# libertininick/imagescry

Hardware: AMD Instinct MI355X
Metric: queries/s cosine top-10 over N x D bank (higher is better)
Workload: dtype f16; 1 GPU; cosine top-10: 1024 fp16 queries x 10000000 x 768 fp16 bank (BASELINE config 4 bank; row-sharded 1 way); bank_rows=10000000, dim=768, queries=1024, k=10, rows_per_gpu=10000000, parallelism=row-shard1

## Files before the change

### imagescry_amd/_lib.py

```python

from __future__ import annotations

import ctypes
import math
import os
from ctypes import POINTER, c_char_p, c_float, c_int, c_int32, c_int64, c_size_t, c_void_p
from pathlib import Path

import torch

LIB_NAME = "libimagescry_hip.so"
LIB_PATH = Path(os.environ.get("ISC_LIB") or Path(__file__).resolve().parent / LIB_NAME)

ISC_U8, ISC_F16, ISC_F32 = 0, 1, 2
ISC_ACT_NONE, ISC_ACT_RELU, ISC_ACT_GELU, ISC_ACT_SILU, ISC_ACT_SIGMOID = 0, 1, 2, 3, 4
ISC_ACT_RESIDUAL_AFTER = 0x100
ISC_TOPK_MAX_K = 120
ISC_SEARCH_MAX_D = 8192
ISC_SEARCH_PASS_QUERIES = 1024
ISC_ABI_VERSION = 4
ISC_BUILD_ABLATION = 1
ISC_GEMM_A_PACKED, ISC_GEMM_W_PACKED, ISC_GEMM_OUT_PACKED, ISC_GEMM_TILE_256, ISC_GEMM_TILE_128 = 1, 2, 4, 8, 16
ISC_KERNEL_DOTS_FILTER, ISC_KERNEL_CONV, ISC_KERNEL_GEMM_F16 = 0, 1, 2

ISC_OK = 0
ISC_ERR_INVALID_ARG = -1
ISC_ERR_UNSUPPORTED = -2
ISC_ERR_WORKSPACE = -3
ISC_ERR_LAUNCH = -4
ISC_ERR_NO_DEVICE = -5
ISC_ERR_ALIGNMENT = -6


class HipLibraryError(RuntimeError):
    """The HIP library is missing, failed to load, or a kernel launch failed."""


SIGNATURES: dict[str, tuple[object, list[object]]] = {
    "isc_abi_version": (c_int, []),
    "isc_build_flags": (c_int, []),
    "isc_strerror": (c_char_p, [c_int]),
    "isc_device_info": (c_int, [POINTER(c_int), POINTER(c_int), c_char_p, c_int]),
    "isc_timing_enable": (c_int, [c_int]),
    "isc_timing_read": (c_int, [c_int, POINTER(ctypes.c_double), POINTER(c_int)]),
    "isc_channel_stats_workspace_bytes": (c_int, [c_int, c_int, c_int, c_int, c_int, POINTER(c_size_t)]),
    "isc_channel_stats": (
        c_int,
        [c_void_p, c_int, c_int, c_int, c_int, c_int, c_void_p, c_void_p, c_void_p, c_size_t, c_void_p],
    ),
    "isc_normalize_clip": (
        c_int,
        [c_void_p, c_int, c_int, c_int, c_int, c_int, c_void_p, c_void_p, c_int, c_float, c_float, c_float, c_void_p,
         c_void_p],
    ),
    "isc_normalize_clip_nhwc4": (
        c_int,
        [c_void_p, c_int, c_int, c_int, c_int, c_int, c_void_p, c_void_p, c_int, c_float, c_float, c_float, c_void_p,
         c_void_p],
    ),
    "isc_resize_bilinear": (c_int, [c_void_p, c_int, c_int, c_int, c_int, c_int, c_int, c_void_p, c_void_p]),
    "isc_l2norm_channels": (c_int, [c_void_p, c_int, c_int, c_int, c_float, c_void_p, c_void_p]),
    "isc_bank_packed_bytes": (c_int, [c_int, c_int64, c_int, POINTER(c_size_t)]),
    "isc_bank_permutation": (c_int, [c_int64, POINTER(c_int64), POINTER(c_int64)]),
    "isc_bank_pack": (
        c_int,
        [c_void_p, c_int, c_int64, c_int, c_int64, c_int64, c_int64, c_int, c_float, c_void_p, c_int, c_void_p,
         c_void_p],
    ),
    "isc_bank_unpack": (c_int, [c_void_p, c_int, c_int, c_int64, c_int64, c_int64, c_void_p, c_int64, c_void_p]),
    "isc_bank_append": (
        c_int,
        [c_void_p, c_int, c_int64, c_int, c_int64, c_int64, c_int64, c_int, c_float, c_void_p, c_int, c_void_p,
         c_void_p, c_void_p, c_void_p, c_void_p],
    ),
    "isc_bank_repack": (
        c_int,
        [c_void_p, c_int64, c_void_p, c_int64, c_int, c_int, c_int64, c_int64, c_void_p, c_void_p, c_void_p, c_void_p],
    ),
    "isc_nchw_to_nhwc": (c_int, [c_void_p, c_int, c_int, c_int, c_int, c_int, c_void_p, c_void_p]),
    "isc_conv2d_nhwc": (
        c_int,
        [c_void_p, c_int, c_int, c_int, c_int, c_void_p, c_int, c_int, c_int, c_int, c_int, c_void_p, c_void_p, c_int,
         c_void_p, c_void_p],
    ),
    "isc_conv2d_nhwc_dual": (
        c_int,
        [c_void_p, c_int, c_int, c_int, c_int, c_void_p, c_int, c_int, c_int, c_int, c_void_p, c_int, c_void_p, c_void_p,
         c_int, c_void_p, c_void_p],
    ),
    "isc_conv2d_nhwc_gated": (
        c_int,
        [c_void_p, c_int, c_int, c_int, c_int, c_void_p, c_void_p, c_int, c_int, c_int, c_int, c_int, c_void_p,
         c_void_p, c_int, c_void_p, c_void_p],
    ),
    "isc_dwconv2d_nhwc": (
        c_int,
        [c_void_p, c_int, c_int, c_int, c_int, c_void_p, c_int, c_int, c_int, c_void_p, c_int, c_void_p, c_void_p],
    ),
    "isc_dwconv2d_nhwc_pool": (
        c_int,
        [c_void_p, c_int, c_int, c_int, c_int, c_void_p, c_int, c_int, c_int, c_void_p, c_int, c_void_p, c_void_p,
         c_void_p, c_void_p],
    ),
    "isc_se_gate": (
        c_int,
        [c_void_p, c_int, c_int, c_void_p, c_int, c_void_p, c_int, c_void_p, c_int, c_void_p, c_void_p, c_void_p],
    ),
    "isc_linear_centered": (
        c_int, [c_void_p, c_int64, c_int, c_void_p, c_void_p, c_int, c_void_p, c_void_p, c_void_p]
    ),
    "isc_feature_sums_workspace_bytes": (c_int, [c_int64, c_int, POINTER(c_size_t)]),
    "isc_feature_sums": (c_int, [c_void_p, c_int64, c_int, c_int64, c_void_p, c_void_p, c_size_t, c_void_p]),
    "isc_center_transpose": (c_int, [c_void_p, c_int64, c_int, c_int64, c_void_p, c_void_p, c_int, c_int64, c_void_p]),
    "isc_gram_rows": (c_int, [c_void_p, c_int, c_int64, c_void_p, c_void_p]),
    "isc_im2col_nchw": (
        c_int,
        [c_void_p, c_int, c_int, c_int, c_int, c_int, c_int, c_int, c_int, c_int, c_void_p, c_void_p],
    ),
    "isc_maxpool_nhwc": (c_int, [c_void_p, c_int, c_int, c_int, c_int, c_int, c_int, c_int, c_void_p, c_void_p]),
    "isc_global_avgpool_nhwc": (c_int, [c_void_p, c_int, c_int, c_int, c_int, c_void_p, c_void_p]),
    "isc_pool_linear_l2norm": (
        c_int, [c_void_p, c_int, c_int, c_int, c_int, c_void_p, c_void_p, c_int, c_int, c_float, c_void_p, c_void_p]
    ),
    "isc_gemm_f16": (
        c_int,
        [c_void_p, c_int64, c_int, c_void_p, c_int, c_void_p, c_void_p, c_int, c_void_p, c_int, c_int, c_void_p],
    ),
    "isc_layernorm": (
        c_int,
        [c_void_p, c_int64, c_int, c_int64, c_void_p, c_void_p, c_float, c_void_p, c_int, c_int64, c_int, c_void_p],
    ),
    "isc_attention_f16": (c_int, [c_void_p, c_int, c_int, c_int, c_int, c_void_p, c_int, c_void_p]),
    "isc_patchify_f16": (c_int, [c_void_p, c_int, c_int, c_int, c_int, c_int, c_void_p, c_int, c_void_p]),
    "isc_vit_assemble": (c_int, [c_void_p, c_void_p, c_void_p, c_int, c_int, c_int, c_void_p, c_void_p]),
    "isc_vit_pos_resample": (c_int, [c_void_p, c_int, c_int, c_int, c_int, c_void_p, c_void_p]),
    "isc_vit_tokens_out": (
        c_int, [c_void_p, c_int, c_int, c_int, c_void_p, c_void_p, c_float, c_int, c_float, c_void_p, c_void_p]
    ),
    "isc_cosine_topk_workspace_bytes": (c_int, [c_int, c_int64, c_int, c_int, c_int, POINTER(c_size_t)]),
    "isc_cosine_topk": (
        c_int,
        [c_void_p, c_int, c_int64, c_int, c_void_p, c_int, c_int, c_int64, c_int, c_int64, c_void_p, c_void_p, c_void_p,
         c_void_p, c_void_p, c_size_t, c_void_p],
    ),
    "isc_bank_shadow_bytes": (c_int, [c_int64, c_int, POINTER(c_size_t)]),
    "isc_bank_quantize": (c_int, [c_void_p, c_int64, c_int, c_void_p, c_size_t, c_void_p]),
    "isc_cosine_topk_uses_shadow": (c_int, [c_int, c_int64, c_int, c_int, c_int, POINTER(c_int)]),
    "isc_cosine_topk_shadow": (
        c_int,
        [c_void_p, c_int, c_int64, c_int, c_void_p, c_int, c_int, c_int64, c_int, c_int64, c_void_p, c_void_p, c_void_p,
         c_void_p, c_void_p, c_size_t, c_void_p, c_void_p],
    ),
    "isc_cosine_topk_exhaustive_workspace_bytes": (c_int, [c_int, c_int64, c_int, c_int, c_int, POINTER(c_size_t)]),
    "isc_cosine_topk_exhaustive": (
        c_int,
        [c_void_p, c_int, c_int64, c_int, c_void_p, c_int, c_int, c_int64, c_int, c_int64, c_void_p, c_void_p,
         c_void_p, c_size_t, c_void_p],
    ),
    "isc_cosine_range_workspace_bytes": (c_int, [c_int, c_int64, c_int, c_int, c_int64, POINTER(c_size_t)]),
    "isc_cosine_range": (
        c_int,
        [c_void_p, c_int, c_int64, c_int, c_void_p, c_int, c_int, c_int64, c_void_p, c_int64, c_void_p, c_int64,
         c_void_p, c_void_p, c_void_p, c_void_p, c_void_p, c_void_p, c_size_t, c_void_p],
    ),
    "isc_row_mask_words": (c_int, [c_int64, POINTER(c_size_t)]),
    "isc_row_mask_pack": (c_int, [c_void_p, c_int64, c_void_p, c_void_p, c_void_p]),
    "isc_cosine_topk_masked": (
        c_int,
        [c_void_p, c_int, c_int64, c_int, c_void_p, c_int, c_int, c_int64, c_int, c_int64, c_void_p, c_void_p, c_void_p,
         c_void_p, c_void_p, c_size_t, c_void_p, c_void_p],
    ),
    "isc_cosine_topk_exhaustive_masked": (
        c_int,
        [c_void_p, c_int, c_int64, c_int, c_void_p, c_int, c_int, c_int64, c_int, c_int64, c_void_p, c_void_p,
         c_void_p, c_size_t, c_void_p, c_void_p],
    ),
    "isc_cosine_range_masked": (
        c_int,
        [c_void_p, c_int, c_int64, c_int, c_void_p, c_int, c_int, c_int64, c_void_p, c_int64, c_void_p, c_int64,
         c_void_p, c_void_p, c_void_p, c_void_p, c_void_p, c_void_p, c_size_t, c_void_p, c_void_p],
    ),
    "isc_row_groups_pack": (c_int, [c_void_p, c_int64, c_void_p, c_void_p]),
    "isc_cosine_topk_grouped": (
        c_int,
        [c_void_p, c_int, c_int64, c_int, c_void_p, c_int, c_int, c_int64, c_int, c_int64, c_void_p, c_void_p, c_void_p,
         c_void_p, c_void_p, c_size_t, c_void_p, c_void_p, c_void_p, c_void_p],
    ),
    "isc_cosine_topk_exhaustive_grouped": (
        c_int,
        [c_void_p, c_int, c_int64, c_int, c_void_p, c_int, c_int, c_int64, c_int, c_int64, c_void_p, c_void_p,
         c_void_p, c_size_t, c_void_p, c_void_p, c_void_p, c_void_p],
    ),
    "isc_cosine_range_grouped": (
        c_int,
        [c_void_p, c_int, c_int64, c_int, c_void_p, c_int, c_int, c_int64, c_void_p, c_int64, c_void_p, c_int64,
         c_void_p, c_void_p, c_void_p, c_void_p, c_void_p, c_void_p, c_size_t, c_void_p, c_void_p, c_void_p, c_void_p],
    ),
    "isc_topk_merge": (
        c_int, [c_void_p, c_void_p, c_int, c_int, c_int, c_int, c_int64, c_int64, c_void_p, c_void_p, c_void_p]
    ),
    "isc_cosine_topk_collapse_workspace_bytes": (c_int, [c_int, c_int64, c_int, c_int, c_int, c_int, POINTER(c_size_t)]),
    "isc_cosine_topk_collapse": (
        c_int,
        [c_void_p, c_int, c_int64, c_int, c_void_p, c_int, c_int, c_int64, c_int, c_int64, c_void_p, c_void_p, c_void_p,
         c_void_p, c_void_p, c_size_t, c_void_p, c_void_p, c_void_p, c_int, c_void_p, c_void_p],
    ),
    "isc_cosine_topk_exhaustive_collapse_workspace_bytes": (
        c_int, [c_int, c_int64, c_int, c_int, c_int, POINTER(c_size_t)]
    ),
    "isc_cosine_topk_exhaustive_collapse": (
        c_int,
        [c_void_p, c_int, c_int64, c_int, c_void_p, c_int, c_int, c_int64, c_int, c_int64, c_void_p, c_void_p,
         c_void_p, c_size_t, c_void_p, c_void_p, c_void_p, c_void_p, c_void_p],
    ),
    "isc_topk_merge_groups": (
        c_int,
        [c_void_p, c_void_p, c_void_p, c_int, c_int, c_int, c_int, c_int64, c_int64, c_int64, c_void_p, c_void_p,
         c_void_p, c_void_p],
    ),
}

_lib: ctypes.CDLL | None = None


def load() -> ctypes.CDLL:
    global _lib
    if _lib is not None:
        return _lib
    if not LIB_PATH.exists():
        raise HipLibraryError(
            f"{LIB_PATH} not found: build it with `python -m imagescry_amd.build` (hipcc, gfx950). "
            "imagescry_amd has no CPU fallback."
        )
    try:
        lib = ctypes.CDLL(str(LIB_PATH))
    except OSError as exc:
        raise HipLibraryError(f"could not load {LIB_PATH}: {exc}") from exc
    missing = [name for name in SIGNATURES if not hasattr(lib, name)]
    if missing:
        raise HipLibraryError(f"{LIB_PATH} does not export {missing}; rebuild it with `python -m imagescry_amd.build`")
    for name, (restype, argtypes) in SIGNATURES.items():
        fn = getattr(lib, name)
        fn.restype = restype
        fn.argtypes = argtypes
    if lib.isc_abi_version() != ISC_ABI_VERSION:
        raise HipLibraryError(
            f"ABI version mismatch: library reports {lib.isc_abi_version()}, binding expects {ISC_ABI_VERSION}; "
            "rebuild it with `python -m imagescry_amd.build`"
        )
    if lib.isc_build_flags() & ISC_BUILD_ABLATION and os.environ.get("ISC_ALLOW_ABLATION") != "1":
        raise HipLibraryError(
            f"{LIB_PATH} is an ablation build (-DISC_ABLATION: timing variants that return wrong results); it is only "
            "loaded with ISC_ALLOW_ABLATION=1 (scripts/), never by the product"
        )
    _lib = lib
    return lib


def strerror(status: int) -> str:
    return load().isc_strerror(status).decode()


def check(status: int, what: str) -> None:
    if status == ISC_OK:
        return
    msg = f"{what}: {strerror(status)} (status {status})"
    if status in (ISC_ERR_INVALID_ARG, ISC_ERR_UNSUPPORTED, ISC_ERR_ALIGNMENT):
        raise ValueError(msg)
    raise HipLibraryError(msg)


def require_device(t: torch.Tensor, name: str) -> None:
    if t.device.type != "cuda":
        raise HipLibraryError(
            f"{name} is on {t.device}; imagescry_amd runs on MI355X (HIP) devices only and has no CPU fallback"
        )


def ptr(t: torch.Tensor | None) -> int | None:
    return None if t is None else t.data_ptr()


def stream_handle(device: torch.device) -> int:
    return torch.cuda.current_stream(device).cuda_stream


def dtype_code(dtype: torch.dtype) -> int:
    if dtype == torch.uint8:
        return ISC_U8
    if dtype == torch.float16:
        return ISC_F16
    if dtype == torch.float32:
        return ISC_F32
    raise TypeError(f"unsupported dtype {dtype}")


INF = math.inf


def timing_enable(enable: bool) -> None:
    check(load().isc_timing_enable(int(enable)), "isc_timing_enable")


def timing_read(kernel_id: int) -> tuple[float, int]:
    total = ctypes.c_double()
    n = c_int()
    check(load().isc_timing_read(kernel_id, total, n), "isc_timing_read")
    return total.value, n.value
```

### imagescry_amd/csrc/bank_layout.h

```cpp
#pragma once

#include <hip/hip_runtime.h>
#include <stdint.h>

#define ISC_TILE_ROWS 256
#define ISC_KSTEP_BYTES 128
#define ISC_TILE_KSTEP_BYTES (ISC_TILE_ROWS * ISC_KSTEP_BYTES)

__host__ __device__ inline int isc_ksteps(int d, int esz) { return (d * esz + ISC_KSTEP_BYTES - 1) / ISC_KSTEP_BYTES; }

__host__ __device__ inline int64_t isc_packed_offset(int64_t row, int kstep, int ks) {
    return (((row >> 8) * ks + kstep) * ISC_TILE_ROWS + (row & 255)) * (int64_t)ISC_KSTEP_BYTES;
}

template <typename T>
__device__ __forceinline__ T isc_packed_load(const void* bank, int64_t row, int e, int ks) {
    const int byte = e * (int)sizeof(T);
    const unsigned char* p = static_cast<const unsigned char*>(bank) + isc_packed_offset(row, byte >> 7, ks) + (byte & 127);
    return *reinterpret_cast<const T*>(p);
}

struct IscShadowRec {
    float scale, inv_scale, resid, qnorm;
};
#define ISC_SHADOW_KSTEP_DIMS 128
__host__ __device__ inline int isc_shadow_ksteps(int d) { return (d + ISC_SHADOW_KSTEP_DIMS - 1) / ISC_SHADOW_KSTEP_DIMS; }
__host__ __device__ inline size_t isc_shadow_data_bytes(int64_t n, int d) {
    return (size_t)((n + ISC_TILE_ROWS - 1) / ISC_TILE_ROWS) * isc_shadow_ksteps(d) * ISC_TILE_KSTEP_BYTES;
}
__host__ __device__ inline size_t isc_shadow_bytes(int64_t n, int d) {
    const size_t rec = (size_t)((n + ISC_TILE_ROWS - 1) / ISC_TILE_ROWS) * sizeof(IscShadowRec);
    return isc_shadow_data_bytes(n, d) + (rec + 255) / 256 * 256;
}

struct IscPerm {
    int64_t n;
    int64_t mul;
    int64_t mul_inv;
};
__host__ __device__ inline int64_t isc_perm_orig(const IscPerm& pm, int64_t packed_pos) {
    return (int64_t)(((unsigned long long)pm.mul * (unsigned long long)packed_pos) % (unsigned long long)pm.n);
}
__host__ __device__ inline int64_t isc_perm_pos(const IscPerm& pm, int64_t orig_row) {
    return (int64_t)(((unsigned long long)pm.mul_inv * (unsigned long long)orig_row) % (unsigned long long)pm.n);
}
IscPerm isc_make_perm(int64_t n);
```

### imagescry_amd/csrc/bank_pack.hip

```cpp
#include "bank_layout.h"
#include "isc_common.h"

namespace {

template <typename TIN, typename TOUT>
__device__ __forceinline__ void isc_pack_row(const TIN* __restrict__ p, int d, int64_t row, int normalize, float eps,
                                             unsigned char* __restrict__ packed, int ks,
                                             unsigned* __restrict__ norm_bound, int lane) {
    float denom = 1.f;
    if (normalize) {
        float acc = 0.f;
        for (int i = lane; i < d; i += 64) {
            const float v = (float)p[i];
            acc += v * v;
        }
        denom = fmaxf(sqrtf(isc_wave_sum(acc)), eps);
    }
    constexpr int PER_CHUNK = 16 / (int)sizeof(TOUT);
    constexpr int IN_VECS = PER_CHUNK * (int)sizeof(TIN) / 16;
    const int chunks = ks * 8;
    const bool vec_ok = IN_VECS > 0 && ((reinterpret_cast<uintptr_t>(p) & 15) == 0);
    float stored_sq = 0.f;
    for (int c = lane; c < chunks; c += 64) {
        TOUT v[PER_CHUNK];
        float f[PER_CHUNK];
        const int e0 = c * PER_CHUNK;
        if (vec_ok && e0 + PER_CHUNK <= d) {
            TIN raw[PER_CHUNK];
#pragma unroll
            for (int u = 0; u < (IN_VECS > 0 ? IN_VECS : 1); ++u)
                reinterpret_cast<uint4*>(raw)[u] = reinterpret_cast<const uint4*>(p + e0)[u];
#pragma unroll
            for (int j = 0; j < PER_CHUNK; ++j) f[j] = (float)raw[j];
        } else {
#pragma unroll
            for (int j = 0; j < PER_CHUNK; ++j) f[j] = e0 + j < d ? (float)p[e0 + j] : 0.f;
        }
#pragma unroll
        for (int j = 0; j < PER_CHUNK; ++j) {
            if (normalize && e0 + j < d) f[j] = __fdiv_rn(f[j], denom);
            v[j] = (TOUT)f[j];
            const float s = (float)v[j];
            stored_sq = fmaf(s, s, stored_sq);
        }
        unsigned char* dst = packed + isc_packed_offset(row, c >> 3, ks) + (c & 7) * 16;
        *reinterpret_cast<uint4*>(dst) = *reinterpret_cast<const uint4*>(v);
    }
    if (norm_bound) {
        stored_sq = isc_wave_sum(stored_sq);
        const float nb = sqrtf(stored_sq) * (1.f + 1e-3f);
        if (lane == 0) {
            const unsigned mine = nb == nb ? __float_as_uint(nb) : 0x7f800000u;
            if (mine > __hip_atomic_load(norm_bound, __ATOMIC_RELAXED, __HIP_MEMORY_SCOPE_AGENT)) atomicMax(norm_bound, mine);
        }
    }
}

template <typename TIN, typename TOUT>
__global__ __launch_bounds__(256) void k_bank_pack(const TIN* __restrict__ x, int64_t n_rows, int d, int64_t ldx,
                                                   int64_t first_row, IscPerm pm, int normalize, float eps,
                                                   unsigned char* __restrict__ packed, int ks,
                                                   unsigned* __restrict__ norm_bound) {
    const int64_t r = (int64_t)blockIdx.x * 4 + (threadIdx.x >> 6);
    if (r >= n_rows) return;
    isc_pack_row<TIN, TOUT>(x + r * ldx, d, isc_perm_pos(pm, first_row + r), normalize, eps, packed, ks, norm_bound,
                            threadIdx.x & 63);
}

template <typename TIN, typename TOUT>
__global__ __launch_bounds__(256) void k_bank_append(const TIN* __restrict__ x, int64_t n_rows, int d, int64_t ldx,
                                                     int64_t first_row, IscPerm pm, int normalize, float eps,
                                                     unsigned char* __restrict__ packed, int ks,
                                                     unsigned* __restrict__ norm_bound, uint32_t* __restrict__ fill_mask,
                                                     const int32_t* __restrict__ codes,
                                                     int32_t* __restrict__ packed_codes) {
    const int64_t r = (int64_t)blockIdx.x * 4 + (threadIdx.x >> 6);
    if (r >= n_rows) return;
    const int lane = threadIdx.x & 63;
    const int64_t row = isc_perm_pos(pm, first_row + r);
    isc_pack_row<TIN, TOUT>(x + r * ldx, d, row, normalize, eps, packed, ks, norm_bound, lane);
    if (lane == 0) {
        atomicOr(fill_mask + (row >> 5), 1u << (row & 31));
        if (packed_codes) {
            const int32_t c = codes[r];
            packed_codes[row] = c < 0 ? -2 : c;
        }
    }
}

__global__ __launch_bounds__(256) void k_bank_repack(const unsigned char* __restrict__ src, IscPerm spm,
                                                     unsigned char* __restrict__ dst, IscPerm dpm, int ks,
                                                     int64_t first_row, int64_t n_rows,
                                                     const int32_t* __restrict__ src_codes,
                                                     int32_t* __restrict__ dst_codes, uint32_t* __restrict__ dst_fill) {
    const int64_t r = (int64_t)blockIdx.x * 4 + (threadIdx.x >> 6);
    if (r >= n_rows) return;
    const int lane = threadIdx.x & 63;
    const int64_t from = isc_perm_pos(spm, first_row + r), to = isc_perm_pos(dpm, first_row + r);
    for (int c = lane; c < ks * 8; c += 64)
        *reinterpret_cast<uint4*>(dst + isc_packed_offset(to, c >> 3, ks) + (c & 7) * 16) =
            *reinterpret_cast<const uint4*>(src + isc_packed_offset(from, c >> 3, ks) + (c & 7) * 16);
    if (lane == 0) {
        atomicOr(dst_fill + (to >> 5), 1u << (to & 31));
        if (dst_codes) dst_codes[to] = src_codes[from];
    }
}

template <typename T>
__global__ __launch_bounds__(256) void k_bank_unpack(const unsigned char* __restrict__ packed, int d, int ks,
                                                     IscPerm pm, int64_t first_row, int64_t n_rows,
                                                     T* __restrict__ y, int64_t ldy) {
    const int64_t r = (int64_t)blockIdx.x * 4 + (threadIdx.x >> 6);
    if (r >= n_rows) return;
    const int lane = threadIdx.x & 63;
    const int64_t row = isc_perm_pos(pm, first_row + r);
    for (int e = lane; e < d; e += 64) y[r * ldy + e] = isc_packed_load<T>(packed, row, e, ks);
}

__global__ __launch_bounds__(256) void k_row_mask_pack(const uint8_t* __restrict__ allow, IscPerm pm,
                                                       uint32_t* __restrict__ packed_mask,
                                                       unsigned long long* __restrict__ allowed_count) {
    const int64_t p = (int64_t)blockIdx.x * 256 + threadIdx.x;
    const int lane = threadIdx.x & 63;
    const bool ok = p < pm.n && allow[isc_perm_orig(pm, p)] != 0;
    const unsigned long long bits = __ballot(ok);
    if (lane == 0) packed_mask[p >> 5] = (uint32_t)bits;
    if (lane == 32) packed_mask[p >> 5] = (uint32_t)(bits >> 32);
    if (allowed_count && lane == 0 && bits != 0ull) atomicAdd(allowed_count, (unsigned long long)__popcll(bits));
}

__global__ __launch_bounds__(256) void k_row_groups_pack(const int32_t* __restrict__ codes, IscPerm pm,
                                                         int32_t* __restrict__ packed_codes) {
    const int64_t p = (int64_t)blockIdx.x * 256 + threadIdx.x;
    const int32_t c = p < pm.n ? codes[isc_perm_orig(pm, p)] : -2;
    packed_codes[p] = c < 0 ? -2 : c;
}

__global__ __launch_bounds__(256) void k_bank_quantize(const unsigned char* __restrict__ bank, int ks, int ks8,
                                                       unsigned char* __restrict__ shadow,
                                                       IscShadowRec* __restrict__ recs) {
    __shared__ float mx_sh[4];
    __shared__ double sum_sh[2][4];
    const int64_t tile = blockIdx.x;
    const int tid = threadIdx.x, lane = tid & 63, wave = tid >> 6;
    const unsigned char* src = bank + tile * ks * (int64_t)ISC_TILE_KSTEP_BYTES;
    float mx = 0.f;
    int bad = 0;
    for (int i = tid; i < ks * (ISC_TILE_KSTEP_BYTES / 16); i += 256) {
        const uint4 raw = *reinterpret_cast<const uint4*>(src + (size_t)i * 16);
        const _Float16* h = reinterpret_cast<const _Float16*>(&raw);
#pragma unroll
        for (int j = 0; j < 8; ++j) {
            const float v = fabsf((float)h[j]);
            bad |= !(v <= 65504.f) ? 1 : 0;
            mx = fmaxf(mx, v);
        }
    }
#pragma unroll
    for (int off = 1; off < 64; off <<= 1) mx = fmaxf(mx, __shfl_xor(mx, off, 64));
    if (lane == 0) mx_sh[wave] = mx;
    bad = __syncthreads_or(bad);
    mx = fmaxf(fmaxf(mx_sh[0], mx_sh[1]), fmaxf(mx_sh[2], mx_sh[3]));
    const float c = mx > 0.f ? 127.f / mx : 1.f;
    const int row0 = tid >> 3, c8 = tid & 7;
    double rs[8], qs[8];
#pragma unroll
    for (int i = 0; i < 8; ++i) rs[i] = qs[i] = 0.0;
    unsigned char* dst = shadow + tile * ks8 * (int64_t)ISC_TILE_KSTEP_BYTES;
    for (int s8 = 0; s8 < ks8; ++s8) {
        const int s = 2 * s8 + (c8 >> 2);
#pragma unroll
        for (int i = 0; i < 8; ++i) {
            const int row = row0 + 32 * i;
            _Float16 h[16];
            if (s < ks) {
                const uint4* p = reinterpret_cast<const uint4*>(src + ((size_t)s * ISC_TILE_ROWS + row) * ISC_KSTEP_BYTES +
                                                                (c8 & 3) * 32);
                reinterpret_cast<uint4*>(h)[0] = p[0];
                reinterpret_cast<uint4*>(h)[1] = p[1];
            } else {
#pragma unroll
                for (int j = 0; j < 16; ++j) h[j] = (_Float16)0.f;
            }
            signed char out[16];
#pragma unroll
            for (int j = 0; j < 16; ++j) {
                const float v = (float)h[j];
                float x = bad ? 0.f : rintf(v * c);
                x = fminf(fmaxf(x, -127.f), 127.f);
                const double r = bad ? 0.0 : (double)v * (double)c - (double)x;
                rs[i] = fma(r, r, rs[i]);
                qs[i] = fma((double)x, (double)x, qs[i]);
                out[j] = (signed char)(int)x;
            }
            *reinterpret_cast<uint4*>(dst + ((size_t)s8 * ISC_TILE_ROWS + row) * ISC_KSTEP_BYTES + c8 * 16) =
                *reinterpret_cast<const uint4*>(out);
        }
    }
    double rmax = 0.0, qmax = 0.0;
#pragma unroll
    for (int i = 0; i < 8; ++i) {
#pragma unroll
        for (int off = 1; off < 8; off <<= 1) {
            rs[i] += __shfl_xor(rs[i], off, 64);
            qs[i] += __shfl_xor(qs[i], off, 64);
        }
        rmax = fmax(rmax, rs[i]);
        qmax = fmax(qmax, qs[i]);
    }
#pragma unroll
    for (int off = 8; off < 64; off <<= 1) {
        rmax = fmax(rmax, __shfl_xor(rmax, off, 64));
        qmax = fmax(qmax, __shfl_xor(qmax, off, 64));
    }
    if (lane == 0) {
        sum_sh[0][wave] = rmax;
        sum_sh[1][wave] = qmax;
    }
    __syncthreads();
    if (tid == 0) {
        rmax = fmax(fmax(sum_sh[0][0], sum_sh[0][1]), fmax(sum_sh[0][2], sum_sh[0][3]));
        qmax = fmax(fmax(sum_sh[1][0], sum_sh[1][1]), fmax(sum_sh[1][2], sum_sh[1][3]));
        IscShadowRec rec;
        rec.scale = mx > 0.f ? mx / 127.f : 1.f;
        rec.inv_scale = c;
        rec.resid = (float)sqrt(rmax) * (1.f + 1e-6f);
        rec.qnorm = bad ? INFINITY : (float)sqrt(qmax) * (1.f + 1e-6f);
        recs[tile] = rec;
    }
}

int check_dtype(int dtype) { return dtype == ISC_F16 || dtype == ISC_F32; }

int64_t gcd64(int64_t a, int64_t b) {
    while (b) {
        const int64_t t = a % b;
        a = b;
        b = t;
    }
    return a;
}

int64_t mod_inverse(int64_t a, int64_t n) {
    int64_t t = 0, nt = 1, r = n, nr = a % n;
    while (nr) {
        const int64_t q = r / nr;
        int64_t tmp = t - q * nt;
        t = nt;
        nt = tmp;
        tmp = r - q * nr;
        r = nr;
        nr = tmp;
    }
    return t < 0 ? t + n : t;
}

}

IscPerm isc_make_perm(int64_t n) {
    IscPerm pm;
    pm.n = n;
    if (n <= 2) {
        pm.mul = pm.mul_inv = 1;
        return pm;
    }
    int64_t m = (int64_t)((double)n * 0.6180339887498949);
    if (m < 1) m = 1;
    while (gcd64(m, n) != 1) ++m;
    pm.mul = m % n;
    pm.mul_inv = mod_inverse(pm.mul, n);
    return pm;
}

extern "C" int isc_bank_permutation(int64_t N, int64_t* mul, int64_t* mul_inv) {
    ISC_REQUIRE(N > 0 && N <= 0x7fffffff && mul && mul_inv);
    const IscPerm pm = isc_make_perm(N);
    *mul = pm.mul;
    *mul_inv = pm.mul_inv;
    return ISC_OK;
}

extern "C" int isc_bank_packed_bytes(int dtype, int64_t N, int D, size_t* bytes) {
    ISC_REQUIRE(bytes && check_dtype(dtype) && N > 0 && D > 0);
    const int esz = dtype == ISC_F16 ? 2 : 4;
    const int64_t tiles = isc_ceil_div<int64_t>(N, ISC_TILE_ROWS);
    *bytes = (size_t)tiles * isc_ksteps(D, esz) * ISC_TILE_KSTEP_BYTES;
    return ISC_OK;
}

extern "C" int isc_bank_pack(const void* rows, int in_dtype, int64_t n_rows, int D, int64_t ldx, int64_t first_row,
                             int64_t n_total, int normalize, float eps, void* packed, int dtype, float* norm_bound,
                             void* stream) {
    ISC_REQUIRE(rows && packed && check_dtype(in_dtype) && check_dtype(dtype));
    ISC_REQUIRE(n_rows > 0 && D > 0 && ldx >= D && first_row >= 0);
    ISC_REQUIRE(n_total >= first_row + n_rows && n_total <= 0x7fffffff);
    if (!isc_aligned(packed, 16)) return ISC_ERR_ALIGNMENT;
    const int64_t blocks = isc_ceil_div<int64_t>(n_rows, 4);
    if (blocks > 0x7fffffff) return ISC_ERR_UNSUPPORTED;
    const int ks = isc_ksteps(D, dtype == ISC_F16 ? 2 : 4);
    unsigned char* out = static_cast<unsigned char*>(packed);
    hipStream_t s = isc_stream(stream);
    const IscPerm pm = isc_make_perm(n_total);
    const dim3 grid((unsigned)blocks), block(256);
#define ISC_PACK(TIN, TOUT)                                                                                         \
    hipLaunchKernelGGL((k_bank_pack<TIN, TOUT>), grid, block, 0, s, static_cast<const TIN*>(rows), n_rows, D, ldx, \
                       first_row, pm, normalize, eps, out, ks, reinterpret_cast<unsigned*>(norm_bound))
    if (in_dtype == ISC_F32 && dtype == ISC_F16) ISC_PACK(float, _Float16);
    else if (in_dtype == ISC_F32 && dtype == ISC_F32) ISC_PACK(float, float);
    else if (in_dtype == ISC_F16 && dtype == ISC_F16) ISC_PACK(_Float16, _Float16);
    else ISC_PACK(_Float16, float);
#undef ISC_PACK
    return isc_launch_status();
}

extern "C" int isc_bank_append(const void* rows, int in_dtype, int64_t n_rows, int D, int64_t ldx, int64_t first_row,
                               int64_t capacity, int normalize, float eps, void* packed, int dtype, float* norm_bound,
                               uint32_t* fill_mask, const int32_t* codes, int32_t* packed_codes, void* stream) {
    ISC_REQUIRE(rows && packed && fill_mask && check_dtype(in_dtype) && check_dtype(dtype));
    ISC_REQUIRE(n_rows > 0 && D > 0 && ldx >= D && first_row >= 0);
    ISC_REQUIRE(capacity >= first_row + n_rows && capacity <= 0x7ffffffe);
    ISC_REQUIRE((codes == nullptr) == (packed_codes == nullptr));
    if (!isc_aligned(packed, 16) || !isc_aligned(fill_mask, 4) || !isc_aligned(codes, 4) || !isc_aligned(packed_codes, 16))
        return ISC_ERR_ALIGNMENT;
    const int64_t blocks = isc_ceil_div<int64_t>(n_rows, 4);
    if (blocks > 0x7fffffff) return ISC_ERR_UNSUPPORTED;
    const int ks = isc_ksteps(D, dtype == ISC_F16 ? 2 : 4);
    unsigned char* out = static_cast<unsigned char*>(packed);
    hipStream_t s = isc_stream(stream);
    const IscPerm pm = isc_make_perm(capacity);
    const dim3 grid((unsigned)blocks), block(256);
#define ISC_APPEND(TIN, TOUT)                                                                                         \
    hipLaunchKernelGGL((k_bank_append<TIN, TOUT>), grid, block, 0, s, static_cast<const TIN*>(rows), n_rows, D, ldx, \
                       first_row, pm, normalize, eps, out, ks, reinterpret_cast<unsigned*>(norm_bound), fill_mask,    \
                       codes, packed_codes)
    if (in_dtype == ISC_F32 && dtype == ISC_F16) ISC_APPEND(float, _Float16);
    else if (in_dtype == ISC_F32 && dtype == ISC_F32) ISC_APPEND(float, float);
    else if (in_dtype == ISC_F16 && dtype == ISC_F16) ISC_APPEND(_Float16, _Float16);
    else ISC_APPEND(_Float16, float);
#undef ISC_APPEND
    return isc_launch_status();
}

extern "C" int isc_bank_repack(const void* src_packed, int64_t src_capacity, void* dst_packed, int64_t dst_capacity,
                               int dtype, int D, int64_t first_row, int64_t n_rows, const int32_t* src_codes,
                               int32_t* dst_codes, uint32_t* dst_fill_mask, void* stream) {
    ISC_REQUIRE(src_packed && dst_packed && dst_fill_mask && src_packed != dst_packed && check_dtype(dtype));
    ISC_REQUIRE(n_rows > 0 && D > 0 && first_row >= 0);
    ISC_REQUIRE(src_capacity >= first_row + n_rows && dst_capacity >= first_row + n_rows);
    ISC_REQUIRE(src_capacity <= 0x7ffffffe && dst_capacity <= 0x7ffffffe);
    ISC_REQUIRE((src_codes == nullptr) == (dst_codes == nullptr));
    if (!isc_aligned(src_packed, 16) || !isc_aligned(dst_packed, 16) || !isc_aligned(dst_fill_mask, 4) ||
        !isc_aligned(src_codes, 4) || !isc_aligned(dst_codes, 16))
        return ISC_ERR_ALIGNMENT;
    const int64_t blocks = isc_ceil_div<int64_t>(n_rows, 4);
    if (blocks > 0x7fffffff) return ISC_ERR_UNSUPPORTED;
    hipLaunchKernelGGL(k_bank_repack, dim3((unsigned)blocks), dim3(256), 0, isc_stream(stream),
                       static_cast<const unsigned char*>(src_packed), isc_make_perm(src_capacity),
                       static_cast<unsigned char*>(dst_packed), isc_make_perm(dst_capacity),
                       isc_ksteps(D, dtype == ISC_F16 ? 2 : 4), first_row, n_rows, src_codes, dst_codes, dst_fill_mask);
    return isc_launch_status();
}

extern "C" int isc_bank_unpack(const void* packed, int dtype, int D, int64_t n_total, int64_t first_row,
                               int64_t n_rows, void* rows, int64_t ldy, void* stream) {
    ISC_REQUIRE(packed && rows && check_dtype(dtype) && D > 0 && n_rows > 0 && first_row >= 0 && ldy >= D);
    ISC_REQUIRE(n_total >= first_row + n_rows && n_total <= 0x7fffffff);
    const int64_t blocks = isc_ceil_div<int64_t>(n_rows, 4);
    if (blocks > 0x7fffffff) return ISC_ERR_UNSUPPORTED;
    const unsigned char* in = static_cast<const unsigned char*>(packed);
    const IscPerm pm = isc_make_perm(n_total);
    if (dtype == ISC_F16)
        hipLaunchKernelGGL(k_bank_unpack<_Float16>, dim3((unsigned)blocks), dim3(256), 0, isc_stream(stream), in, D,
                           isc_ksteps(D, 2), pm, first_row, n_rows, static_cast<_Float16*>(rows), ldy);
    else
        hipLaunchKernelGGL(k_bank_unpack<float>, dim3((unsigned)blocks), dim3(256), 0, isc_stream(stream), in, D,
                           isc_ksteps(D, 4), pm, first_row, n_rows, static_cast<float*>(rows), ldy);
    return isc_launch_status();
}

extern "C" int isc_row_mask_words(int64_t N, size_t* words) {
    ISC_REQUIRE(words && N > 0 && N <= 0x7ffffffe);
    *words = (size_t)isc_ceil_div<int64_t>(N, ISC_TILE_ROWS) * (ISC_TILE_ROWS / 32);
    return ISC_OK;
}

extern "C" int isc_row_mask_pack(const uint8_t* allow, int64_t N, uint32_t* packed_mask, int64_t* allowed_count,
                                 void* stream) {
    ISC_REQUIRE(allow && packed_mask && N > 0 && N <= 0x7ffffffe);
    if (!isc_aligned(packed_mask, 4) || !isc_aligned(allowed_count, 8)) return ISC_ERR_ALIGNMENT;
    const int64_t tiles = isc_ceil_div<int64_t>(N, ISC_TILE_ROWS);
    hipLaunchKernelGGL(k_row_mask_pack, dim3((unsigned)tiles), dim3(256), 0, isc_stream(stream), allow, isc_make_perm(N),
                       packed_mask, reinterpret_cast<unsigned long long*>(allowed_count));
    return isc_launch_status();
}

extern "C" int isc_row_groups_pack(const int32_t* codes, int64_t N, int32_t* packed_codes, void* stream) {
    ISC_REQUIRE(codes && packed_codes && N > 0 && N <= 0x7ffffffe);
    if (!isc_aligned(codes, 4) || !isc_aligned(packed_codes, 16)) return ISC_ERR_ALIGNMENT;
    const int64_t tiles = isc_ceil_div<int64_t>(N, ISC_TILE_ROWS);
    hipLaunchKernelGGL(k_row_groups_pack, dim3((unsigned)tiles), dim3(256), 0, isc_stream(stream), codes,
                       isc_make_perm(N), packed_codes);
    return isc_launch_status();
}

extern "C" int isc_bank_shadow_bytes(int64_t N, int D, size_t* bytes) {
    ISC_REQUIRE(bytes && N > 0 && N <= 0x7ffffffe && D > 0);
    *bytes = isc_shadow_bytes(N, D);
    return ISC_OK;
}

extern "C" int isc_bank_quantize(const void* packed, int64_t N, int D, void* shadow, size_t shadow_bytes, void* stream) {
    ISC_REQUIRE(packed && shadow && N > 0 && N <= 0x7ffffffe && D > 0);
    if (!isc_aligned(packed, 16) || !isc_aligned(shadow, 256)) return ISC_ERR_ALIGNMENT;
    if (shadow_bytes < isc_shadow_bytes(N, D)) return ISC_ERR_WORKSPACE;
    const int64_t tiles = isc_ceil_div<int64_t>(N, ISC_TILE_ROWS);
    unsigned char* out = static_cast<unsigned char*>(shadow);
    hipLaunchKernelGGL(k_bank_quantize, dim3((unsigned)tiles), dim3(256), 0, isc_stream(stream),
                       static_cast<const unsigned char*>(packed), isc_ksteps(D, 2), isc_shadow_ksteps(D), out,
                       reinterpret_cast<IscShadowRec*>(out + isc_shadow_data_bytes(N, D)));
    return isc_launch_status();
}
```

### imagescry_amd/csrc/cosine_topk.hip

```cpp
#include <math.h>
#include <stdlib.h>

#include <type_traits>

#include "bank_layout.h"
#include "isc_common.h"
#include "search_common.h"

namespace {

typedef _Float16 half8 __attribute__((ext_vector_type(8)));
typedef float f32x4 __attribute__((ext_vector_type(4)));
typedef unsigned u32x4 __attribute__((ext_vector_type(4)));
typedef int i32x4 __attribute__((ext_vector_type(4)));

constexpr int TM = 256;
constexpr int NTHREADS = 512;
constexpr int CAP = 32;
constexpr int TARGET_WGS = 256;
constexpr int QCAP = 8192;
constexpr int SLACK = 6;
constexpr int SMALL_Q = 128;
constexpr int QBATCH = ISC_SEARCH_PASS_QUERIES;
constexpr int MAX_LEVELS = 12;
constexpr int SEL_THREADS = 512;
constexpr int SURV_CAP = 2048;
constexpr int TAIL_LCAP = 256;
constexpr int TAIL_COUNT_OFF = 64 * TAIL_LCAP * 8;
constexpr int TAIL_LBOUND_OFF = 140 * 1024;

struct Cand {
    float s;
    int32_t row;
};

struct Level {
    int64_t r0, r1;
    int ntiles, tiles_per_chunk, nchunks;
    int sample;
};

struct Plan {
    int tnq;
    int segs_per_chunk;
    int kp;
    int nslots;
    int qb;
    int qtiles;
    int qpad;
    int max_seg;
    int nlevels;
    int64_t budget;
    Level levels[MAX_LEVELS];
};

int plan_kp(int k) { return (int)isc_align_up((size_t)k + SLACK, 16); }

#ifdef ISC_ABLATION
int forced_tile() {
    static const int v = [] {
        const char* e = getenv("ISC_FORCE_TILE");
        return e ? atoi(e) : 0;
    }();
    return v;
}
#else
constexpr int forced_tile() { return 0; }
#endif

#ifdef ISC_ABLATION
__device__ int g_abl_thr_inf = 0;
int first_ratio() {
    static const int v = getenv("ISC_FIRST_RATIO") ? atoi(getenv("ISC_FIRST_RATIO")) : 16;
    return v;
}
int sample_tiles_cap() {
    static const int v = getenv("ISC_SAMPLE_TILES") ? atoi(getenv("ISC_SAMPLE_TILES")) : 0;
    return v;
}
#else
constexpr int first_ratio() { return 16; }
constexpr int sample_tiles_cap() { return 0; }
#endif

constexpr int COLLAPSE_MIN_KP = 32;
constexpr int COLLAPSE_ROWS_CAP = 64;
constexpr int COLLAPSE_GROUPS = 4096;

Plan make_plan(int64_t n, int q, int k, int group_rows = 0) {
    Plan p;
    p.qb = q < QBATCH ? q : QBATCH;
    p.tnq = p.qb <= 64 ? 64 : p.qb <= SMALL_Q ? 128 : 256;
    if (forced_tile() == 64 || forced_tile() == 128 || forced_tile() == 256) p.tnq = forced_tile();
    p.segs_per_chunk = (8 / (p.tnq / 64)) * 4;
    p.kp = plan_kp(k);
    if (group_rows > 0 && p.kp < COLLAPSE_MIN_KP) p.kp = COLLAPSE_MIN_KP;
    p.qtiles = isc_ceil_div(p.qb, p.tnq);
    p.qpad = p.qtiles * p.tnq;
    p.nslots = group_rows > 0 ? 0 : p.kp <= 16 ? 32 : p.kp <= 32 ? 64 : p.kp <= 64 ? 128 : 0;
    int wgs = TARGET_WGS / p.qtiles;
    if (wgs < 1) wgs = 1;
    const int64_t ntiles_all = isc_ceil_div<int64_t>(n, TM);

    p.nlevels = 0;
    p.max_seg = 0;
    p.budget = 0;
    auto add = [&](int64_t r0, int64_t r1, int sample) {
        Level& l = p.levels[p.nlevels++];
        l.r0 = r0;
        l.r1 = r1;
        l.sample = sample;
        l.ntiles = (int)isc_ceil_div<int64_t>(r1 - r0, TM);
        int want = sample ? l.ntiles : wgs;
        if (want > l.ntiles) want = l.ntiles;
        l.tiles_per_chunk = isc_ceil_div(l.ntiles, want);
        l.nchunks = isc_ceil_div(l.ntiles, l.tiles_per_chunk);
        if (p.segs_per_chunk * l.nchunks > p.max_seg) p.max_seg = p.segs_per_chunk * l.nchunks;
    };
    int64_t stiles = p.nslots ? (int64_t)(QCAP * 7 / 10) / (p.kp * 27 / 20) : 16;
    if (stiles > wgs) stiles = wgs;
    if (sample_tiles_cap() > 0 && stiles > sample_tiles_cap()) stiles = sample_tiles_cap();
    if (stiles < 1) stiles = 1;
    if (stiles > ntiles_all) stiles = ntiles_all;
    int64_t seen = stiles * TM < n ? stiles * TM : n;
    add(0, seen, 1);
    while (seen < n) {
        const int64_t nseg = (int64_t)p.segs_per_chunk * wgs;
        int64_t budget = (int64_t)((double)QCAP * p.kp / (p.kp + 8.0 * sqrt((double)p.kp)));
        if (group_rows > 0) budget = (int64_t)((double)COLLAPSE_GROUPS * p.kp / (p.kp + 8.0 * sqrt((double)p.kp)));
        if (nseg * CAP / 8 < budget) budget = nseg * CAP / 8;
        p.budget = budget;
        const int64_t unit = (int64_t)p.kp * (group_rows > COLLAPSE_ROWS_CAP ? COLLAPSE_ROWS_CAP : group_rows > 0 ? group_rows : 1);
        int64_t ratio = 1 + budget / unit;
        if (p.tnq == 256 && p.qtiles == 1 && p.nlevels == 1 && ratio > first_ratio()) ratio = first_ratio();
        if (ratio < 3) ratio = 3;
        int64_t r1 = seen * ratio;
        if (r1 > n || p.nlevels == MAX_LEVELS - 1) r1 = n;
        add(seen, r1, 0);
        seen = r1;
    }
    const int redo_chunks = (int)(wgs < ntiles_all ? wgs : ntiles_all);
    if (p.segs_per_chunk * redo_chunks > p.max_seg) p.max_seg = p.segs_per_chunk * redo_chunks;
    return p;
}

struct Workspace {
    float* tau;
    float* carry_s;
    int32_t* carry_r;
    int32_t* carry_n;
    int32_t* qflag;
    Cand* seg_ent;
    int32_t* qcount;
    Cand* qlist;
    unsigned char* qpacked;
    int32_t* r_count;
    int32_t* r_list;
    float* tau2;
    int32_t* qcount2;
    int32_t* qflag2;
    unsigned char* qpacked2;
    IscExactWs exact;
    unsigned char* qpacked8;
    float4* qrec8;
    size_t bytes;
};

Workspace carve(const Plan& p, int ks, int64_t n, int k, void* base) {
    Workspace w;
    size_t off = 0;
    auto take = [&](size_t bytes) {
        void* ptr = base ? static_cast<char*>(base) + off : nullptr;
        off += isc_align_up(bytes, 256);
        return ptr;
    };
    w.tau = static_cast<float*>(take((size_t)p.qpad * 4));
    w.carry_s = static_cast<float*>(take((size_t)p.qpad * p.kp * 4));
    w.carry_r = static_cast<int32_t*>(take((size_t)p.qpad * p.kp * 4));
    w.carry_n = static_cast<int32_t*>(take((size_t)p.qpad * 4));
    w.qflag = static_cast<int32_t*>(take((size_t)p.qpad * 4));
    w.seg_ent = static_cast<Cand*>(take((size_t)p.max_seg * p.qpad * CAP * sizeof(Cand)));
    w.qcount = static_cast<int32_t*>(take((size_t)p.qpad * 4));
    w.qlist = static_cast<Cand*>(take((size_t)p.qpad * QCAP * sizeof(Cand)));
    w.qpacked = static_cast<unsigned char*>(take((size_t)p.qpad * ks * ISC_KSTEP_BYTES));
    w.r_count = static_cast<int32_t*>(take(4));
    w.r_list = static_cast<int32_t*>(take((size_t)p.qpad * 4));
    w.tau2 = static_cast<float*>(take((size_t)p.qpad * 4));
    w.qcount2 = static_cast<int32_t*>(take((size_t)p.qpad * 4));
    w.qflag2 = static_cast<int32_t*>(take((size_t)p.qpad * 4));
    w.qpacked2 = static_cast<unsigned char*>(take((size_t)p.qpad * ks * ISC_KSTEP_BYTES));
    const size_t ex = isc_exact_ws_bytes(n, p.qb, k);
    w.exact = isc_exact_ws_carve(take(ex), n, p.qb, k);
    const int ks8 = (ks + 1) / 2;
    w.qpacked8 = static_cast<unsigned char*>(take((size_t)p.qpad * ks8 * ISC_KSTEP_BYTES));
    w.qrec8 = static_cast<float4*>(take((size_t)p.qpad * sizeof(float4)));
    w.bytes = off;
    return w;
}

template <typename T, typename TQ>
__global__ __launch_bounds__(256) void k_prep(const TQ* __restrict__ queries, int64_t ldq, int q, int d, int ks, int qpad,
                                              int tnq, unsigned char* __restrict__ packed, float* __restrict__ tau,
                                              int32_t* __restrict__ carry_n, int32_t* __restrict__ qcount,
                                              int32_t* __restrict__ qflag, int32_t* __restrict__ redo_count,
                                              int32_t* __restrict__ exact_done, int32_t* __restrict__ r_count,
                                              float* __restrict__ tau2, int32_t* __restrict__ qcount2,
                                              int32_t* __restrict__ qflag2, int32_t* __restrict__ status,
                                              int zero_status) {
    constexpr int PER = 16 / (int)sizeof(T);
    const int total = qpad * ks * 8;
    const int i = blockIdx.x * 256 + threadIdx.x;
    if (i < qpad) {
        tau[i] = i < q ? -INFINITY : INFINITY;
        carry_n[i] = 0;
        qcount[i] = 0;
        qflag[i] = 0;
        tau2[i] = INFINITY;
        qcount2[i] = 0;
        qflag2[i] = 0;
    }
    if (i == 0) {
        *redo_count = 0;
        *exact_done = 0;
        *r_count = 0;
    }
    if (zero_status && i < 4) status[i] = 0;
    if (i >= total) return;
    const int c = i & 7;
    const int row = (i >> 3) % tnq;
    const int blk = (i >> 3) / tnq;
    const int kstep = blk % ks;
    const int qrow = (blk / ks) * tnq + row;
    T v[PER];
#pragma unroll
    for (int j = 0; j < PER; ++j) {
        const int e = (kstep * 8 + c) * PER + j;
        v[j] = (qrow < q && e < d) ? (T)queries[(int64_t)qrow * ldq + e] : (T)0.f;
    }
    *reinterpret_cast<uint4*>(packed + (size_t)i * 16) = *reinterpret_cast<const uint4*>(v);
}

template <typename TQ>
__global__ __launch_bounds__(256) void k_prep_i8(const TQ* __restrict__ queries, int64_t ldq, int q, int d, int ks8,
                                                 int tnq, unsigned char* __restrict__ packed8,
                                                 float4* __restrict__ qrec) {
    const int lane = threadIdx.x & 63;
    const int qrow = blockIdx.x * 4 + (threadIdx.x >> 6);
    const TQ* src = queries + (int64_t)qrow * ldq;
    float mx = 0.f;
    int bad = 0;
    if (qrow < q) {
        for (int e = lane; e < d; e += 64) {
            const float v = fabsf((float)(_Float16)src[e]);
            bad |= !(v <= 65504.f) ? 1 : 0;
            mx = fmaxf(mx, v);
        }
    }
#pragma unroll
    for (int off = 1; off < 64; off <<= 1) {
        mx = fmaxf(mx, __shfl_xor(mx, off, 64));
        bad |= __shfl_xor(bad, off, 64);
    }
    const bool live = qrow < q && !bad && mx > 0.f;
    const float c = live ? 127.f / mx : 0.f;
    double rs = 0.0, qs = 0.0;
    unsigned char* dst = packed8 + ((size_t)(qrow / tnq) * ks8 * tnq + (qrow % tnq)) * ISC_KSTEP_BYTES;
    for (int ch = lane; ch < ks8 * 8; ch += 64) {
        signed char out[16];
#pragma unroll
        for (int j = 0; j < 16; ++j) {
            const int e = ch * 16 + j;
            const float v = (live && e < d) ? (float)(_Float16)src[e] : 0.f;
            const float x = fminf(fmaxf(rintf(v * c), -127.f), 127.f);
            const double r = (double)v * (double)c - (double)x;
            rs = fma(r, r, rs);
            qs = fma((double)x, (double)x, qs);
            out[j] = (signed char)(int)x;
        }
        *reinterpret_cast<uint4*>(dst + (size_t)(ch >> 3) * tnq * ISC_KSTEP_BYTES + (ch & 7) * 16) =
            *reinterpret_cast<const uint4*>(out);
    }
    rs = isc_wave_sum(rs);
    qs = isc_wave_sum(qs);
    if (lane == 0)
        qrec[qrow] = make_float4(live ? c : __uint_as_float(0x7fc00000u), (float)sqrt(qs) * (1.f + 1e-6f),
                                 (float)sqrt(rs) * (1.f + 1e-6f), 0.f);
}

template <typename T>
struct Mma;

template <>
struct Mma<_Float16> {
    typedef f32x4 Acc;
    static __device__ __forceinline__ void half(const u32x4& a, const u32x4 (&b)[4], f32x4 (&acc)[4]) {
#pragma unroll
        for (int n = 0; n < 4; ++n)
            acc[n] = __builtin_amdgcn_mfma_f32_16x16x32_f16(__builtin_bit_cast(half8, a),
                                                            __builtin_bit_cast(half8, b[n]), acc[n], 0, 0, 0);
    }
    static __device__ __forceinline__ void row(const u32x4& a0, const u32x4& a1, const u32x4 (&b)[2][4],
                                               f32x4 (&acc)[4]) {
        half(a0, b[0], acc);
        half(a1, b[1], acc);
    }
    template <int N0, int N1>
    static __device__ __forceinline__ void part(const u32x4& a, const u32x4 (&b)[4], f32x4 (&acc)[4]) {
#pragma unroll
        for (int n = N0; n < N1; ++n)
            acc[n] = __builtin_amdgcn_mfma_f32_16x16x32_f16(__builtin_bit_cast(half8, a),
                                                            __builtin_bit_cast(half8, b[n]), acc[n], 0, 0, 0);
    }
};

template <>
struct Mma<float> {
    typedef f32x4 Acc;
    static __device__ __forceinline__ void half(const u32x4& a, const u32x4 (&b)[4], f32x4 (&acc)[4]) {
#pragma unroll
        for (int j = 0; j < 4; ++j)
#pragma unroll
            for (int n = 0; n < 4; ++n)
                acc[n] = __builtin_amdgcn_mfma_f32_16x16x4f32(__uint_as_float(a[j]), __uint_as_float(b[n][j]), acc[n],
                                                              0, 0, 0);
    }
    static __device__ __forceinline__ void row(const u32x4& a0, const u32x4& a1, const u32x4 (&b)[2][4],
                                               f32x4 (&acc)[4]) {
        half(a0, b[0], acc);
        half(a1, b[1], acc);
    }
    template <int N0, int N1>
    static __device__ __forceinline__ void part(const u32x4& a, const u32x4 (&b)[4], f32x4 (&acc)[4]) {
#pragma unroll
        for (int j = 0; j < 4; ++j)
#pragma unroll
            for (int n = N0; n < N1; ++n)
                acc[n] = __builtin_amdgcn_mfma_f32_16x16x4f32(__uint_as_float(a[j]), __uint_as_float(b[n][j]), acc[n],
                                                              0, 0, 0);
    }
};

template <>
struct Mma<signed char> {
    typedef i32x4 Acc;
    template <int N0, int N1>
    static __device__ __forceinline__ void part(const u32x4& a, const u32x4 (&b)[4], i32x4 (&acc)[4]) {
#pragma unroll
        for (int n = N0; n < N1; ++n)
            acc[n] = __builtin_amdgcn_mfma_i32_16x16x64_i8(__builtin_bit_cast(i32x4, a), __builtin_bit_cast(i32x4, b[n]),
                                                           acc[n], 0, 0, 0);
    }
};

struct IscShadowArgs {
    const IscShadowRec* recs;
    const float4* qrec;
};

#define ISC_DS_READ(dst_, addr_, off_) \
    asm volatile("ds_read_b128 %0, %1 offset:%2" : "=v"(dst_) : "v"(addr_), "i"(off_))

__device__ __forceinline__ void glds16(const unsigned char* gsrc, unsigned char* lds_wave_base) {
    __builtin_amdgcn_global_load_lds((const __attribute__((address_space(1))) void*)gsrc,
                                     (__attribute__((address_space(3))) void*)lds_wave_base, 16, 0, 0);
}
template <bool NT>
__device__ __forceinline__ void glds16_bank(const unsigned char* gsrc, unsigned char* lds_wave_base) {
    if constexpr (NT)
        __builtin_amdgcn_global_load_lds((const __attribute__((address_space(1))) void*)gsrc,
                                         (__attribute__((address_space(3))) void*)lds_wave_base, 16, 0, 2);
    else
        glds16(gsrc, lds_wave_base);
}

template <int N>
__device__ __forceinline__ void wait_vmcnt() {
    static_assert(N >= 0 && N <= 63, "vmcnt range");
    asm volatile("s_waitcnt vmcnt(%0)" ::"i"(N) : "memory");
}

constexpr int A_TILE_BYTES = TM * 128;

#ifndef ISC_ASYM_MBLO
#define ISC_ASYM_MBLO 6
#endif
#ifndef ISC_ASYM_SPLIT_MBLO
#define ISC_ASYM_SPLIT_MBLO 8
#endif
#ifndef ISC_HM_RING
#define ISC_HM_RING 4
#endif
#ifndef ISC_HM_DMA0
#define ISC_HM_DMA0 1
#endif
#ifndef ISC_HM_B1U
#define ISC_HM_B1U 2
#endif

template <typename T, int TNQ, int DBG, bool SAMPLE, typename... RowMask>
__global__ __launch_bounds__(NTHREADS) void k_dots_filter(const unsigned char* __restrict__ bank, int64_t r0,
                                                          int64_t r1, int tiles_per_chunk, int ntiles,
                                                          const unsigned char* __restrict__ qpacked, int ksteps,
                                                          const float* __restrict__ tau, int qpad,
                                                          Cand* __restrict__ seg_ent, int32_t* __restrict__ qcount,
                                                          Cand* __restrict__ qlist, int kp, int nslots,
                                                          int32_t* __restrict__ qflag, int32_t* __restrict__ status,
                                                          const int32_t* __restrict__ active, RowMask... row_mask) {
    constexpr bool I8 = std::is_same<T, signed char>::value;
    typedef typename Mma<T>::Acc Acc;
    constexpr bool MASK = sizeof...(RowMask) > 0 && !I8;
    constexpr bool GROUP = isc_grouped<RowMask...>();
    static_assert(!I8 || (TNQ == 256 && DBG == 12 && !SAMPLE && sizeof...(RowMask) == 1), "the int8 filter is one kernel");
    constexpr bool REDO = DBG == 20 || DBG == 32 || DBG == 33;
    constexpr int MODE = DBG == 20 ? 0 : DBG == 32 ? 12 : DBG == 33 ? 13 : DBG;
    if constexpr (REDO) {
        if (*active <= (int)blockIdx.y * TNQ) return;
    }
    constexpr int WN = TNQ / 64;
    constexpr int WM = 8 / WN;
    constexpr int MB = TM / WM / 16;
    constexpr bool NOBREAD = (MODE == 41 || MODE == 43) && TNQ == 256;
    constexpr bool NOBDMA = MODE == 41 && TNQ == 256;
    constexpr bool HM = MODE == 12 && TNQ == 256 && !SAMPLE;
    constexpr bool NOSPLIT_FORM = MODE == 12 || MODE == 22 || MODE == 41 || MODE == 43 || MODE == 48;
    constexpr int ASYM_LO = NOSPLIT_FORM ? ISC_ASYM_MBLO : MODE == 0 ? ISC_ASYM_SPLIT_MBLO : 8;
    constexpr bool ASYM = TNQ == 256 && !SAMPLE && ASYM_LO != 8;
    constexpr int MBLO = ASYM ? ASYM_LO : MB;
    constexpr int MBHI = ASYM ? 2 * MB - MBLO : MB;
    constexpr int MBMAX = MBHI > MBLO ? MBHI : MBLO;
    constexpr int B_TILE_BYTES = TNQ * 128;
    constexpr int NA = 4;
    constexpr int NB = B_TILE_BYTES / 8192;
    constexpr int A_ST = TNQ == 64 ? 4 : 3;
    constexpr int B_ST = TNQ == 256 ? 2 : TNQ == 128 ? 3 : 4;
    constexpr int DA = A_ST - 1;
    constexpr int DB = B_ST - 1;
    constexpr int LDS_BYTES = A_ST * A_TILE_BYTES + B_ST * B_TILE_BYTES;
    static_assert(LDS_BYTES == (TNQ == 128 ? 147456 : 163840), "the two rings fill the CU's LDS (TNQ = 128: 144 KiB of it)");
    static_assert(TNQ == 256 || DA == DB, "the HBM-bound shapes stage query and bank steps at one prefetch distance");
    __shared__ __attribute__((aligned(16))) unsigned char lds[LDS_BYTES];

    const int tid = threadIdx.x;
    const int lane = tid & 63;
    const int wave = __builtin_amdgcn_readfirstlane(tid >> 6);
    const int wm = wave / WN;
    const int wn = wave % WN;
    const int chunk = blockIdx.x;
    const int qt = blockIdx.y;
    const int q0 = qt * TNQ;

    const int tile_begin = chunk * tiles_per_chunk;
    const int tile_end = min(ntiles, tile_begin + tiles_per_chunk);
    const int my_tiles = tile_end - tile_begin;
    const int total_steps = my_tiles * ksteps;

    const int frow = lane & 15;
    const int fg = lane >> 4;

    float thr[4];
    int cnt[4];
#pragma unroll
    for (int n = 0; n < 4; ++n) {
        thr[n] = tau[q0 + wn * 64 + n * 16 + frow];
        if ((MODE != 0 && MODE < 11) || (MODE >= 15 && MODE != 48)) thr[n] = fabsf(thr[n]) + 3.0e38f;
#ifdef ISC_ABLATION
        if (!SAMPLE && g_abl_thr_inf) thr[n] = fabsf(thr[n]) + 3.0e38f;
#endif
        cnt[n] = 0;
    }
    [[maybe_unused]] float qn8[4], eq8[4];
    if constexpr (I8) {
        const IscShadowArgs& sa = (row_mask, ...);
#pragma unroll
        for (int n = 0; n < 4; ++n) {
            const float4 qr = sa.qrec[q0 + wn * 64 + n * 16 + frow];
            thr[n] *= qr.x;
            qn8[n] = qr.y;
            eq8[n] = qr.z;
        }
    }

    const int srow = tid >> 3;
    const int spc = tid & 7;
    const int slot_src = srow * 128 + ((spc ^ ((srow >> 1) & 7)) << 4);
    const unsigned char* a_stream = bank + ((r0 >> 8) + tile_begin) * (int64_t)ksteps * A_TILE_BYTES + slot_src;
    const unsigned char* b_stream = qpacked + (int64_t)qt * ksteps * B_TILE_BYTES + slot_src;

    unsigned char* const lds_a = lds;
    unsigned char* const lds_b = lds + A_ST * A_TILE_BYTES;
    const unsigned lds_a_addr = (unsigned)(size_t)(__attribute__((address_space(3))) unsigned char*)lds;
    const unsigned lds_b_addr = lds_a_addr + A_ST * A_TILE_BYTES;
    const int wave_dst = wave * 1024;

    constexpr bool SPLIT = TNQ == 256 && !NOSPLIT_FORM;
    constexpr bool NT = (TNQ == 256 && MODE == 0) || MODE == 13;
    auto issue_a = [&](int step) {
        const unsigned char* src = a_stream + (int64_t)step * A_TILE_BYTES;
        unsigned char* dst = lds_a + (step % A_ST) * A_TILE_BYTES + wave_dst;
        if constexpr (SPLIT) {
            if (wm == 0) {
#pragma unroll
                for (int i = 0; i < 2 * NA; ++i) glds16_bank<NT>(src + 4096 * i, dst + 4096 * i);
            }
        } else {
#pragma unroll
            for (int i = 0; i < NA; ++i) glds16_bank<NT>(src + 8192 * i, dst + 8192 * i);
        }
    };
    auto issue_b = [&](int step) {
        const unsigned char* src = b_stream + (int64_t)(step % ksteps) * B_TILE_BYTES;
        unsigned char* dst = lds_b + (step % B_ST) * B_TILE_BYTES + wave_dst;
        if constexpr (SPLIT) {
            if (wm == 0) {
#pragma unroll
                for (int i = 0; i < 2 * NB; ++i) glds16(src + 4096 * i, dst + 4096 * i);
            }
        } else {
#pragma unroll
            for (int i = 0; i < NB; ++i) glds16(src + 8192 * i, dst + 8192 * i);
        }
    };
    auto issue_iter = [&](int it) {
        if ((MODE == 2 || MODE == 7) && it >= 0) return;
        const int sb = it + DB, sa = it + DA;
        if (!NOBDMA && sb >= 0 && sb < total_steps) issue_b(sb);
        if (sa >= 0 && sa < total_steps) issue_a(sa);
    };
    auto retire_for = [&](int next) {
        if (MODE == 2 || MODE == 7) {
            wait_vmcnt<0>();
            return;
        }
        if (MODE == 15) return;
        if (TNQ == 256) {
            if constexpr (SPLIT) {
                if (wm == 0) {
                    if (next + 1 < total_steps) wait_vmcnt<2 * NA>();
                    else wait_vmcnt<0>();
                }
            } else {
                if (next + 1 < total_steps) wait_vmcnt<NA>();
                else wait_vmcnt<0>();
            }
        } else {
            const int ahead = min(DA - 1, total_steps - 1 - next);
            if (ahead >= 2) wait_vmcnt<2 * (NA + NB)>();
            else if (ahead == 1) wait_vmcnt<NA + NB>();
            else wait_vmcnt<0>();
        }
    };

    const int fsw = (lane >> 1) & 7;
    int foff[2];
#pragma unroll
    for (int kk = 0; kk < 2; ++kk) foff[kk] = frow * 128 + (((kk * 4 + fg) ^ fsw) << 4);
    const int wave_row0 = ASYM ? (wm == 0 ? 0 : MBLO * 16) : wm * (TM / WM);
    const int a_wave_off = wave_row0 * 128;
    const int b_wave_off = wn * 64 * 128;

    Acc acc[MBMAX][4];
#pragma unroll
    for (int m = 0; m < MBMAX; ++m)
#pragma unroll
        for (int n = 0; n < 4; ++n) acc[m][n] = Acc{0, 0, 0, 0};

    constexpr int MASK_WORDS = (16 + MBMAX * 16 + 31) / 32;
    auto load_mask = [&](auto mbe_c, auto sub_c, int64_t gtile, uint32_t (&w)[MASK_WORDS]) {
        constexpr int MBE = decltype(mbe_c)::value, SUB = decltype(sub_c)::value, NW = (SUB + MBE * 16 + 31) / 32;
        typedef const __attribute__((address_space(4))) uint32_t ConstWord;
        ConstWord* src = (ConstWord*)(isc_row_mask_ptr(row_mask...) + gtile * (TM / 32) + (wave_row0 >> 5));
#pragma unroll
        for (int i = 0; i < NW; ++i) w[i] = src[i];
    };
    auto apply_mask = [&](auto mbe_c, auto sub_c, const uint32_t (&w)[MASK_WORDS]) {
        constexpr int MBE = decltype(mbe_c)::value, SUB = decltype(sub_c)::value;
#pragma unroll
        for (int m = 0; m < MBE; ++m) {
            const uint32_t bits = w[(SUB + 16 * m) >> 5] >> ((SUB + 16 * m) & 31);
            if ((bits & 0xffffu) == 0xffffu) continue;
            const uint32_t nib = bits >> (fg * 4);
#pragma unroll
            for (int r = 0; r < 4; ++r)
                if (!((nib >> r) & 1u)) {
#pragma unroll
                    for (int n = 0; n < 4; ++n) acc[m][n][r] = -INFINITY;
                }
        }
    };
    [[maybe_unused]] bool use_mask = true;
    if constexpr (GROUP) use_mask = isc_row_mask_ptr(row_mask...) != nullptr;
    [[maybe_unused]] uint32_t sample_mask[MASK_WORDS];
    if constexpr (MASK && SAMPLE) {
        if (use_mask)
            load_mask(std::integral_constant<int, MB>{}, std::integral_constant<int, 0>{}, (r0 >> 8) + tile_begin,
                      sample_mask);
    }

    constexpr bool DEFER = GROUP && TNQ == 256 && !SAMPLE;
    constexpr bool LATE = GROUP && TNQ == 256 && SAMPLE;
    [[maybe_unused]] int qcode[4];
    if constexpr (GROUP) {
        const IscGroups& gr = (row_mask, ...);
#pragma unroll
        for (int n = 0; n < 4; ++n) {
            const int col = q0 + wn * 64 + n * 16 + frow;
            if constexpr (REDO) {
                const int c = col < *active ? gr.query_group[gr.slot_query[col]] : -1;
                qcode[n] = c < 0 ? -1 : c;
            } else {
                qcode[n] = isc_query_code(gr, col);
            }
        }
    }
    auto load_codes = [&](auto mbe_c, int64_t gtile, i32x4 (&c)[MBMAX]) {
        constexpr int MBE = decltype(mbe_c)::value;
        const int32_t* src = isc_row_group_ptr(row_mask...) + gtile * TM + wave_row0 + fg * 4;
#pragma unroll
        for (int m = 0; m < MBE; ++m) c[m] = *reinterpret_cast<const i32x4*>(src + 16 * m);
    };
    auto apply_codes = [&](auto mbe_c, const i32x4 (&c)[MBMAX]) {
        constexpr int MBE = decltype(mbe_c)::value;
#pragma unroll
        for (int m = 0; m < MBE; ++m)
#pragma unroll
            for (int r = 0; r < 4; ++r)
#pragma unroll
                for (int n = 0; n < 4; ++n)
                    if (c[m][r] == qcode[n]) acc[m][n][r] = -INFINITY;
    };
    [[maybe_unused]] i32x4 sample_codes[MBMAX];
    if constexpr (GROUP && SAMPLE && !LATE)
        load_codes(std::integral_constant<int, MB>{}, (r0 >> 8) + tile_begin, sample_codes);

    const int seg = (chunk * WM + wm) * 4 + fg;
    Cand* my_ent = seg_ent + ((size_t)seg * qpad + q0 + wn * 64 + frow) * CAP;

    if constexpr (TNQ == 256 && NOSPLIT_FORM) {
#ifdef ISC_ABLATION
        if (!((nslots >> 18) & 1))
#endif
            if (__builtin_amdgcn_readfirstlane(tid) >= 256) __builtin_amdgcn_s_setprio(1);
    }
    for (int it = -DA; it < 0; ++it) issue_iter(it);
    retire_for(0);
    __builtin_amdgcn_s_barrier();

    unsigned long long st_compute = 0, st_vmwait = 0, st_barrier = 0, st_prev = 0;
    auto stamp = [&]() -> unsigned long long {
        unsigned long long t;
        __builtin_amdgcn_sched_barrier(0);
        asm volatile("s_memtime %0\n\ts_waitcnt lgkmcnt(0)" : "=s"(t)::"memory");
        __builtin_amdgcn_sched_barrier(0);
        return t;
    };
    auto main_loop = [&](auto stagger_tag) {
    constexpr bool STAGGER = decltype(stagger_tag)::value;
    using MBE_C = std::integral_constant<int, STAGGER ? MBHI : MBLO>;
    using SUB_C = std::integral_constant<int, (TNQ == 256 && STAGGER) ? ((ASYM ? MBLO : MB) * 16) & 31 : 0>;
    int kt = 0, tile = 0;
    [[maybe_unused]] uint32_t tile_mask[MASK_WORDS];
    [[maybe_unused]] i32x4 tile_codes[MBMAX];
    [[maybe_unused]] float tile_ct = 0.f, tile_et = 0.f, tile_nt = 0.f;
    if constexpr (MODE == 22) st_prev = stamp();
    for (int step = 0; step < total_steps; ++step) {
        if constexpr (MASK && !SAMPLE) {
            if (kt == 0 && use_mask) load_mask(MBE_C{}, SUB_C{}, (r0 >> 8) + tile_begin + tile, tile_mask);
        }
        if constexpr (GROUP && !SAMPLE && !DEFER) {
            if (kt == 0) load_codes(MBE_C{}, (r0 >> 8) + tile_begin + tile, tile_codes);
        }
        if constexpr (I8) {
            if (kt == 0) {
                typedef const __attribute__((address_space(4))) float ConstFloat;
                ConstFloat* src = (ConstFloat*)((row_mask, ...).recs + ((r0 >> 8) + tile_begin + tile));
                tile_ct = src[1];
                tile_et = src[2];
                tile_nt = src[3];
            }
        }
        if constexpr (HM) {
            constexpr int MBW = STAGGER ? MBHI : MBLO;
            constexpr int NU = 2 * MBW;
            static_assert(MBW >= 4, "the second half's query fragments are fetched under four units of the first");
            const int sb = step + DB, sa = step + DA;
            const bool do_b = sb < total_steps;
            const bool do_a = sa < total_steps;
            const unsigned char* bsrc = b_stream + (int64_t)(sb % ksteps) * B_TILE_BYTES;
            unsigned char* bdst = lds_b + (sb % B_ST) * B_TILE_BYTES + wave_dst;
            const unsigned char* asrc = a_stream + (int64_t)sa * A_TILE_BYTES;
            unsigned char* adst = lds_a + (sa % A_ST) * A_TILE_BYTES + wave_dst;
            const unsigned a_addr = lds_a_addr + (unsigned)((step % A_ST) * A_TILE_BYTES + a_wave_off);
            const unsigned b_addr = lds_b_addr + (unsigned)((step % B_ST) * B_TILE_BYTES + b_wave_off);
            const unsigned a_addr0 = a_addr + foff[0], a_addr1 = a_addr + foff[1];
            const unsigned b_addr0 = b_addr + foff[0], b_addr1 = b_addr + foff[1];
            constexpr int RING = ISC_HM_RING;
            u32x4 b0[4], b1[4], ar[RING];
            ISC_DS_READ(b0[0], b_addr0, 0);
            ISC_DS_READ(b0[1], b_addr0, 2048);
            ISC_DS_READ(b0[2], b_addr0, 4096);
            ISC_DS_READ(b0[3], b_addr0, 6144);
            auto read_unit = [&](auto uc) {
                constexpr int u = decltype(uc)::value, m = u % MBW, kk = u / MBW;
                auto& frag = ar;
                const unsigned addr = kk == 0 ? a_addr0 : a_addr1;
                ISC_DS_READ(frag[u % RING], addr, m * 2048);
            };
            read_unit(std::integral_constant<int, 0>{});
            read_unit(std::integral_constant<int, 1>{});
            read_unit(std::integral_constant<int, 2>{});
            if constexpr (RING > 4) read_unit(std::integral_constant<int, 3>{});
            if constexpr (RING > 5) read_unit(std::integral_constant<int, 4>{});
            static_assert(RING >= 4 && RING <= 6, "prologue reads");
            constexpr int B1U = ISC_HM_B1U < MBW - 4 ? ISC_HM_B1U : MBW - 4;
            constexpr int DMA0 = ISC_HM_DMA0;
            auto reads_of = [](int v) constexpr { return (v >= B1U && v < B1U + 4 ? 1 : 0) + (v + RING - 1 < NU ? 1 : 0); };
            auto issued_through = [reads_of](int u) constexpr {
                int c = 4 + RING - 1;
                for (int v = 0; v <= u; ++v) c += reads_of(v);
                return c;
            };
            auto pos_a = [issued_through](int w) constexpr {
                if (w < RING - 1) return 4 + w;
                return issued_through(w - (RING - 1)) - 1;
            };
            auto pos_b1_last = [issued_through]() constexpr {
                return issued_through(B1U + 2);
            };
            auto newer_than = [=](int w, int u) constexpr {
                int need = pos_a(w);
                if (w >= MBW && pos_b1_last() > need) need = pos_b1_last();
                return issued_through(u) - 1 - need;
            };
            auto overhead = [&](auto uc, auto wc) {
                constexpr int u = decltype(uc)::value, w = decltype(wc)::value;
                if constexpr (u >= B1U && u < B1U + 4) {
                    auto& q1 = b1;
                    const unsigned addr = b_addr1;
                    ISC_DS_READ(q1[u - B1U], addr, (u - B1U) * 2048);
                }
                if constexpr (u + RING - 1 < NU) read_unit(std::integral_constant<int, u + RING - 1>{});
#pragma unroll
                for (int j = 0; j < 8; ++j) {
                    if (DMA0 + j * (NU - 1 - DMA0) / 8 != u) continue;
                    if (j < 4) {
                        if (do_b) glds16(bsrc + 8192 * j, bdst + 8192 * j);
                    } else {
                        if (do_a) glds16_bank<NT>(asrc + 8192 * (j - 4), adst + 8192 * (j - 4));
                    }
                }
                if constexpr (w < NU) {
                    auto& frag = ar;
                    auto& q0 = b0;
                    auto& q1 = b1;
                    if constexpr (w == 0)
                        asm volatile("s_waitcnt lgkmcnt(%5)"
                                     : "+v"(frag[0]), "+v"(q0[0]), "+v"(q0[1]), "+v"(q0[2]), "+v"(q0[3])
                                     : "i"(newer_than(0, u)));
                    else if constexpr (w == MBW)
                        asm volatile("s_waitcnt lgkmcnt(%5)"
                                     : "+v"(frag[w % RING]), "+v"(q1[0]), "+v"(q1[1]), "+v"(q1[2]), "+v"(q1[3])
                                     : "i"(newer_than(w, u)));
                    else
                        asm volatile("s_waitcnt lgkmcnt(%1)" : "+v"(frag[w % RING]) : "i"(newer_than(w, u)));
                    __builtin_amdgcn_sched_barrier(0);
                }
            };
            if constexpr (STAGGER) {
                asm volatile("s_waitcnt lgkmcnt(%5)" : "+v"(ar[0]), "+v"(b0[0]), "+v"(b0[1]), "+v"(b0[2]), "+v"(b0[3]) : "i"(RING - 2));
                __builtin_amdgcn_sched_barrier(0);
                auto units = [&](auto self, auto uc) {
                    constexpr int u = decltype(uc)::value, m = u % MBW, kk = u / MBW;
                    if constexpr (kk == 0) Mma<T>::template part<0, 2>(ar[u % RING], b0, acc[m]);
                    else Mma<T>::template part<0, 2>(ar[u % RING], b1, acc[m]);
                    overhead(uc, std::integral_constant<int, u + 1>{});
                    if constexpr (kk == 0) Mma<T>::template part<2, 4>(ar[u % RING], b0, acc[m]);
                    else Mma<T>::template part<2, 4>(ar[u % RING], b1, acc[m]);
                    if constexpr (u + 1 < NU) self(self, std::integral_constant<int, u + 1>{});
                };
                units(units, std::integral_constant<int, 0>{});
            } else {
                auto units = [&](auto self, auto uc) {
                    constexpr int u = decltype(uc)::value, m = u % MBW, kk = u / MBW;
                    overhead(uc, uc);
                    if constexpr (kk == 0) Mma<T>::template part<0, 4>(ar[u % RING], b0, acc[m]);
                    else Mma<T>::template part<0, 4>(ar[u % RING], b1, acc[m]);
                    if constexpr (u + 1 < NU) self(self, std::integral_constant<int, u + 1>{});
                };
                units(units, std::integral_constant<int, 0>{});
            }
        } else if constexpr (TNQ == 256 && MODE != 7 && MODE != 17) {
            constexpr int MBW = STAGGER ? MBHI : MBLO;
            static_assert(MBW >= 3 && MBW <= MBMAX, "row blocks per wave");
            const int sb = step + DB, sa = step + DA;
            const bool do_b = MODE != 2 && !NOBDMA && sb < total_steps;
            const bool do_a = MODE != 2 && sa < total_steps;
            const unsigned char* bsrc = b_stream + (int64_t)(sb % ksteps) * B_TILE_BYTES;
            unsigned char* bdst = lds_b + (sb % B_ST) * B_TILE_BYTES + wave_dst;
            const unsigned char* asrc = a_stream + (int64_t)sa * A_TILE_BYTES;
            unsigned char* adst = lds_a + (sa % A_ST) * A_TILE_BYTES + wave_dst;
            const unsigned a_addr = lds_a_addr + (unsigned)((step % A_ST) * A_TILE_BYTES + a_wave_off);
            const unsigned b_addr = lds_b_addr + (unsigned)((step % B_ST) * B_TILE_BYTES + b_wave_off);
            const unsigned a_addr0 = a_addr + foff[0], a_addr1 = a_addr + foff[1];
            const unsigned b_addr0 = b_addr + foff[0], b_addr1 = b_addr + foff[1];
            u32x4 b0[4], b1[4], ar[3][2];
            constexpr int NBR = NOBREAD ? 0 : 4;
            if constexpr (NOBREAD) {
#pragma unroll
                for (int i = 0; i < 4; ++i) b0[i] = b1[i] = u32x4{(unsigned)step, 1u, 2u, (unsigned)lane};
                ISC_DS_READ(ar[0][0], a_addr0, 0);
                ISC_DS_READ(ar[0][1], a_addr1, 0);
            } else {
            ISC_DS_READ(b0[0], b_addr0, 0);
            ISC_DS_READ(b0[1], b_addr0, 2048);
            ISC_DS_READ(b0[2], b_addr0, 4096);
            ISC_DS_READ(b0[3], b_addr0, 6144);
            ISC_DS_READ(ar[0][0], a_addr0, 0);
            ISC_DS_READ(b1[0], b_addr1, 0);
            ISC_DS_READ(b1[1], b_addr1, 2048);
            ISC_DS_READ(b1[2], b_addr1, 4096);
            ISC_DS_READ(b1[3], b_addr1, 6144);
            ISC_DS_READ(ar[0][1], a_addr1, 0);
            }
            ISC_DS_READ(ar[1][0], a_addr0, 2048);
            ISC_DS_READ(ar[1][1], a_addr1, 2048);
            auto dma_piece = [&](auto jc) {
                constexpr int j = decltype(jc)::value;
                if constexpr (SPLIT) {
                    if constexpr (!STAGGER) {
                        if constexpr (j < 4) {
                            if (do_b) {
                                glds16(bsrc + 4096 * (2 * j), bdst + 4096 * (2 * j));
                                glds16(bsrc + 4096 * (2 * j + 1), bdst + 4096 * (2 * j + 1));
                            }
                        } else if (do_a) {
                            glds16_bank<NT>(asrc + 4096 * (2 * (j - 4)), adst + 4096 * (2 * (j - 4)));
                            glds16_bank<NT>(asrc + 4096 * (2 * (j - 4) + 1), adst + 4096 * (2 * (j - 4) + 1));
                        }
                    }
                } else if constexpr (j < 4) {
                    if (do_b) glds16(bsrc + 8192 * j, bdst + 8192 * j);
                } else {
                    if (do_a) glds16_bank<NT>(asrc + 8192 * (j - 4), adst + 8192 * (j - 4));
                }
            };
            auto dma_at = [&](auto mc) {
                constexpr int m = decltype(mc)::value;
                constexpr int extra = MBW < 8 ? 8 - MBW : 0;
                if constexpr (m < extra) {
                    dma_piece(std::integral_constant<int, 2 * m>{});
                    dma_piece(std::integral_constant<int, 2 * m + 1>{});
                } else if constexpr (m + extra < 8) {
                    dma_piece(std::integral_constant<int, m + extra>{});
                }
            };
#define ISC_MFMA_HALF(a_, b_, m_)                                                                         \
    if constexpr (MODE != 3) Mma<T>::half(a_, b_, acc[m_]);                                                 \
    else acc[m_][0][0] += __uint_as_float((a_)[0] ^ (b_)[1][1] ^ (b_)[2][2]);
            if constexpr (STAGGER) {
                asm volatile("s_waitcnt lgkmcnt(%5)" : "+v"(b0[0]), "+v"(b0[1]), "+v"(b0[2]), "+v"(b0[3]), "+v"(ar[0][0]) : "i"(NBR + 3));
                __builtin_amdgcn_sched_barrier(0);
                ISC_MFMA_HALF(ar[0][0], b0, 0)
                ISC_DS_READ(ar[2][0], a_addr0, 4096);
                ISC_DS_READ(ar[2][1], a_addr1, 4096);
                dma_at(std::integral_constant<int, 0>{});
                asm volatile("s_waitcnt lgkmcnt(2)"
                             : "+v"(b1[0]), "+v"(b1[1]), "+v"(b1[2]), "+v"(b1[3]), "+v"(ar[0][1]), "+v"(ar[1][0]),
                               "+v"(ar[1][1]));
                __builtin_amdgcn_sched_barrier(0);
                ISC_MFMA_HALF(ar[0][1], b1, 0)
                auto blocks = [&](auto self, auto mc) {
                    constexpr int m = decltype(mc)::value;
                    constexpr int cur = m % 3, nxt = (m + 1) % 3, nn = (m + 2) % 3;
                    ISC_MFMA_HALF(ar[cur][0], b0, m)
                    if constexpr (m + 2 < MBW) {
                        ISC_DS_READ(ar[nn][0], a_addr0, (m + 2) * 2048);
                        ISC_DS_READ(ar[nn][1], a_addr1, (m + 2) * 2048);
                    }
                    dma_at(mc);
                    if constexpr (m + 1 < MBW) {
                        asm volatile("s_waitcnt lgkmcnt(%3)"
                                     : "+v"(ar[nxt][0]), "+v"(ar[nxt][1]), "+v"(ar[cur][1])
                                     : "i"(m + 2 < MBW ? 2 : 0));
                        __builtin_amdgcn_sched_barrier(0);
                    }
                    ISC_MFMA_HALF(ar[cur][1], b1, m)
                    if constexpr (m + 1 < MBW) self(self, std::integral_constant<int, m + 1>{});
                };
                blocks(blocks, std::integral_constant<int, 1>{});
            } else {
                ISC_DS_READ(ar[2][0], a_addr0, 4096);
                ISC_DS_READ(ar[2][1], a_addr1, 4096);
                asm volatile("s_waitcnt lgkmcnt(%5)" : "+v"(b0[0]), "+v"(b0[1]), "+v"(b0[2]), "+v"(b0[3]), "+v"(ar[0][0]) : "i"(NBR + 5));
                __builtin_amdgcn_sched_barrier(0);
                dma_at(std::integral_constant<int, 0>{});
                ISC_MFMA_HALF(ar[0][0], b0, 0)
                asm volatile("s_waitcnt lgkmcnt(4)" : "+v"(b1[0]), "+v"(b1[1]), "+v"(b1[2]), "+v"(b1[3]), "+v"(ar[0][1]));
                __builtin_amdgcn_sched_barrier(0);
                ISC_MFMA_HALF(ar[0][1], b1, 0)
                auto blocks = [&](auto self, auto mc) {
                    constexpr int m = decltype(mc)::value;
                    constexpr int cur = m % 3, nn = (m + 2) % 3;
                    if constexpr (m + 2 < MBW) {
                        ISC_DS_READ(ar[nn][0], a_addr0, (m + 2) * 2048);
                        ISC_DS_READ(ar[nn][1], a_addr1, (m + 2) * 2048);
                    }
                    asm volatile("s_waitcnt lgkmcnt(%2)"
                                 : "+v"(ar[cur][0]), "+v"(ar[cur][1])
                                 : "i"(m + 2 < MBW ? 4 : m + 1 < MBW ? 2 : 0));
                    __builtin_amdgcn_sched_barrier(0);
                    dma_at(mc);
                    ISC_MFMA_HALF(ar[cur][0], b0, m)
                    ISC_MFMA_HALF(ar[cur][1], b1, m)
                    if constexpr (m + 1 < MBW) self(self, std::integral_constant<int, m + 1>{});
                };
                blocks(blocks, std::integral_constant<int, 1>{});
            }
#undef ISC_MFMA_HALF
        } else {
        issue_iter(step);

        {
            const unsigned a_addr = lds_a_addr + (unsigned)((step % A_ST) * A_TILE_BYTES + a_wave_off);
            const unsigned b_addr = lds_b_addr + (unsigned)((step % B_ST) * B_TILE_BYTES + b_wave_off);
            const unsigned a_addr0 = a_addr + foff[0], a_addr1 = a_addr + foff[1];
            const unsigned b_addr0 = b_addr + foff[0], b_addr1 = b_addr + foff[1];
            u32x4 bq[2][4], ar[2][2];
            if constexpr (MODE == 7 || MODE == 17) {
#pragma unroll
                for (int i = 0; i < 8; ++i) bq[i >> 2][i & 3] = u32x4{(unsigned)step, 1u, 2u, (unsigned)lane};
                ar[0][0] = ar[0][1] = ar[1][0] = ar[1][1] = u32x4{(unsigned)lane, 3u, (unsigned)step, 5u};
#pragma unroll
                for (int m = 0; m < MB; ++m) Mma<T>::row(ar[m & 1][0], ar[m & 1][1], bq, acc[m]);
            } else {
            ISC_DS_READ(bq[0][0], b_addr0, 0);
            ISC_DS_READ(bq[0][1], b_addr0, 2048);
            ISC_DS_READ(bq[0][2], b_addr0, 4096);
            ISC_DS_READ(bq[0][3], b_addr0, 6144);
            ISC_DS_READ(bq[1][0], b_addr1, 0);
            ISC_DS_READ(bq[1][1], b_addr1, 2048);
            ISC_DS_READ(bq[1][2], b_addr1, 4096);
            ISC_DS_READ(bq[1][3], b_addr1, 6144);
            ISC_DS_READ(ar[0][0], a_addr0, 0);
            ISC_DS_READ(ar[0][1], a_addr1, 0);
#define ISC_ROW_STEP(m_, cur_, nxt_)                                                                                 \
    if constexpr ((m_) < MB) {                                                                                       \
        if constexpr ((m_) + 1 < MB) {                                                                               \
            ISC_DS_READ(ar[nxt_][0], a_addr0, ((m_) + 1) * 2048);                                                    \
            ISC_DS_READ(ar[nxt_][1], a_addr1, ((m_) + 1) * 2048);                                                    \
        }                                                                                                            \
        if constexpr ((m_) == 0)                                                                                     \
            asm volatile("s_waitcnt lgkmcnt(2)"                                                                      \
                         : "+v"(bq[0][0]), "+v"(bq[0][1]), "+v"(bq[0][2]), "+v"(bq[0][3]), "+v"(bq[1][0]),           \
                           "+v"(bq[1][1]), "+v"(bq[1][2]), "+v"(bq[1][3]), "+v"(ar[0][0]), "+v"(ar[0][1]));          \
        else if constexpr ((m_) + 1 < MB)                                                                            \
            asm volatile("s_waitcnt lgkmcnt(2)" : "+v"(ar[cur_][0]), "+v"(ar[cur_][1]));                            \
        else                                                                                                         \
            asm volatile("s_waitcnt lgkmcnt(0)" : "+v"(ar[cur_][0]), "+v"(ar[cur_][1]));                            \
        __builtin_amdgcn_sched_barrier(0);                                                                           \
        if constexpr (MODE != 3)                                                                                      \
            Mma<T>::row(ar[cur_][0], ar[cur_][1], bq, acc[m_]);                                                      \
        else                                                                                                         \
            acc[m_][0][0] += __uint_as_float(ar[cur_][0][0] ^ ar[cur_][1][1] ^ bq[0][1][0] ^ bq[1][2][1]);           \
    }
            ISC_ROW_STEP(0, 0, 1)
            ISC_ROW_STEP(1, 1, 0)
            ISC_ROW_STEP(2, 0, 1)
            ISC_ROW_STEP(3, 1, 0)
            ISC_ROW_STEP(4, 0, 1)
            ISC_ROW_STEP(5, 1, 0)
            ISC_ROW_STEP(6, 0, 1)
            ISC_ROW_STEP(7, 1, 0)
#undef ISC_ROW_STEP
            }
        }

        }

        if constexpr (!SAMPLE) {
        if (++kt == ksteps) {
            kt = 0;
            constexpr int MBE = STAGGER ? MBHI : MBLO;
            const int64_t trow0 = r0 + (int64_t)(tile_begin + tile) * TM + wave_row0 + fg * 4;
            if constexpr (MASK) {
                if (use_mask) apply_mask(MBE_C{}, SUB_C{}, tile_mask);
            }
            if constexpr (GROUP && !DEFER) apply_codes(MBE_C{}, tile_codes);
            if constexpr (I8) {
                int thr_i[4];
#pragma unroll
                for (int n = 0; n < 4; ++n) {
                    const float t = thr[n] * tile_ct;
                    const float mg = fmaf(qn8[n], tile_et, eq8[n] * (tile_nt + tile_et));
                    const float lo = (t - mg) - (fabsf(t) + mg) * 9.5367431640625e-7f - 1e-30f;
                    thr_i[n] = !(lo <= 2.0e9f) ? INT32_MAX : lo < -2.0e9f ? INT32_MIN : (int)floorf(lo);
                    if (!(tile_nt < INFINITY)) thr_i[n] = thr[n] < INFINITY ? INT32_MIN : INT32_MAX;
                }
                if (r0 + (int64_t)(tile_begin + tile + 1) * TM > r1) {
#pragma unroll
                    for (int m = 0; m < MBE; ++m)
#pragma unroll
                        for (int r = 0; r < 4; ++r)
                            if (trow0 + m * 16 + r >= r1) {
#pragma unroll
                                for (int n = 0; n < 4; ++n) acc[m][n][r] = INT32_MIN;
                            }
                }
#pragma unroll
                for (int n = 0; n < 4; ++n) {
                    int bm[MBE];
                    int mx = INT32_MIN;
#pragma unroll
                    for (int m = 0; m < MBE; ++m) {
                        bm[m] = max(max(acc[m][n][0], acc[m][n][1]), max(acc[m][n][2], acc[m][n][3]));
                        mx = max(mx, bm[m]);
                    }
                    if (__ballot(mx > thr_i[n]) != 0ull) {
#pragma unroll
                        for (int m = 0; m < MBE; ++m) {
                            if (__ballot(bm[m] > thr_i[n]) == 0ull) continue;
#pragma unroll
                            for (int r = 0; r < 4; ++r) {
                                if (acc[m][n][r] > thr_i[n]) {
                                    const int pos = cnt[n]++;
                                    if (pos < CAP)
                                        my_ent[n * 16 * CAP + pos] = Cand{(float)acc[m][n][r], (int32_t)(trow0 + m * 16 + r)};
                                }
                            }
                        }
                    }
                }
            } else {
            if (r0 + (int64_t)(tile_begin + tile + 1) * TM > r1) {
#pragma unroll
                for (int m = 0; m < MBE; ++m)
#pragma unroll
                    for (int r = 0; r < 4; ++r)
                        if (trow0 + m * 16 + r >= r1) {
#pragma unroll
                            for (int n = 0; n < 4; ++n) acc[m][n][r] = -INFINITY;
                        }
            }
#pragma unroll
            for (int n = 0; n < 4; ++n) {
                float bm[MBE];
                float mx = -INFINITY;
#pragma unroll
                for (int m = 0; m < MBE; ++m) {
                    bm[m] = fmaxf(fmaxf(acc[m][n][0], acc[m][n][1]), fmaxf(acc[m][n][2], acc[m][n][3]));
                    mx = fmaxf(mx, bm[m]);
                }
                if (__ballot(mx > thr[n]) != 0ull) {
#pragma unroll
                    for (int m = 0; m < MBE; ++m) {
                        if (__ballot(bm[m] > thr[n]) == 0ull) continue;
#pragma unroll
                        for (int r = 0; r < 4; ++r) {
                            const float s = acc[m][n][r];
                            if (s > thr[n]) {
                                const int pos = cnt[n]++;
                                if (pos < CAP) my_ent[n * 16 * CAP + pos] = Cand{s, (int32_t)(trow0 + m * 16 + r)};
                            }
                        }
                    }
                }
            }
            }
#pragma unroll
            for (int m = 0; m < MBE; ++m)
#pragma unroll
                for (int n = 0; n < 4; ++n) acc[m][n] = Acc{0, 0, 0, 0};
            ++tile;
        }
        }

        if constexpr (MODE == 22) {
            const unsigned long long tb = stamp();
            retire_for(step + 1);
            const unsigned long long tc = stamp();
            __builtin_amdgcn_s_barrier();
            const unsigned long long td = stamp();
            st_compute += tb - st_prev;
            st_vmwait += tc - tb;
            st_barrier += td - tc;
            st_prev = td;
        } else {
        retire_for(step + 1);
        __builtin_amdgcn_s_barrier();
        }
    }
    if constexpr (MODE == 22) {
        if (lane == 0) {
            unsigned long long* dbg = reinterpret_cast<unsigned long long*>(seg_ent) +
                                      ((size_t)(blockIdx.y * gridDim.x + blockIdx.x) * 8 + wave) * 4;
            dbg[0] = st_compute;
            dbg[1] = st_vmwait;
            dbg[2] = st_barrier;
            dbg[3] = (unsigned long long)total_steps;
        }
    }
    };
    if (TNQ == 256 && MODE != 11 && __builtin_amdgcn_readfirstlane(wm) == 1) main_loop(std::true_type{});
    else main_loop(std::false_type{});

#ifdef ISC_ABLATION
    const int abl = nslots >> 16;
    nslots &= 0xffff;
    if (abl & 1) return;
#endif
    if constexpr (SAMPLE) {
        const int64_t trow0 = r0 + (int64_t)tile_begin * TM + wm * (TM / WM) + fg * 4;
        if constexpr (MASK) {
            if (use_mask) apply_mask(std::integral_constant<int, MB>{}, std::integral_constant<int, 0>{}, sample_mask);
        }
        if constexpr (LATE) load_codes(std::integral_constant<int, MB>{}, (r0 >> 8) + tile_begin, sample_codes);
        if constexpr (GROUP) apply_codes(std::integral_constant<int, MB>{}, sample_codes);
#pragma unroll
        for (int m = 0; m < MB; ++m)
#pragma unroll
            for (int r = 0; r < 4; ++r)
                if (trow0 + m * 16 + r >= r1) {
#pragma unroll
                    for (int n = 0; n < 4; ++n) acc[m][n][r] = -INFINITY;
                }
        if (nslots > 0) {
            float* smax = reinterpret_cast<float*>(lds);
            const int sstride = nslots + 4;
            float* lbound = reinterpret_cast<float*>(lds + TAIL_LBOUND_OFF);
            const int gsz = TM / nslots;
            const int per_lane = MB * 4 / gsz;
#pragma unroll
            for (int n = 0; n < 4; ++n) {
                float* dst = smax + (size_t)(wn * 64 + n * 16 + frow) * sstride + (wm * 4 + fg) * per_lane;
                float cur = -INFINITY;
#pragma unroll
                for (int e = 0; e < MB * 4; ++e) {
                    cur = fmaxf(cur, acc[e >> 2][n][e & 3]);
                    if (((e + 1) & (gsz - 1)) == 0) {
                        dst[e / gsz] = cur;
                        cur = -INFINITY;
                    }
                }
            }
            __syncthreads();
            for (int id = tid; id < TNQ * nslots; id += NTHREADS) {
                const int qc = id / nslots, sl = id - qc * nslots;
                const float4* row4 = reinterpret_cast<const float4*>(smax + (size_t)qc * sstride);
                const float v = smax[(size_t)qc * sstride + sl];
                int rank = 0;
#pragma unroll 2
                for (int j4 = 0; j4 < nslots / 4; ++j4) {
                    const float4 x = row4[j4];
                    const int j = j4 * 4;
                    rank += (x.x > v || (x.x == v && j + 0 < sl)) ? 1 : 0;
                    rank += (x.y > v || (x.y == v && j + 1 < sl)) ? 1 : 0;
                    rank += (x.z > v || (x.z == v && j + 2 < sl)) ? 1 : 0;
                    rank += (x.w > v || (x.w == v && j + 3 < sl)) ? 1 : 0;
                }
                if (rank == kp - 1) lbound[qc] = v;
            }
            __syncthreads();
#pragma unroll
            for (int n = 0; n < 4; ++n) {
                const float lb = lbound[wn * 64 + n * 16 + frow];
                const unsigned u = __float_as_uint(lb);
                const float below = lb == 0.f ? __uint_as_float(0x80000001u)
                                              : __uint_as_float(lb > 0.f ? u - 1u : u + 1u);
                if (thr[n] != INFINITY) thr[n] = lb == -INFINITY ? -INFINITY : below;
            }
        }
    }

#ifdef ISC_ABLATION
    if (abl & 2) return;
#endif
    {
        const int PASSES = (SAMPLE && TNQ == 256 && kp <= 16) ? 1 : WN;
        const int QPP = TNQ / PASSES;
        const int LCAP = 64 * TAIL_LCAP / QPP;
        const int TPQ = NTHREADS / QPP;
        Cand* lists = reinterpret_cast<Cand*>(lds);
        int* lcount = reinterpret_cast<int*>(lds + TAIL_COUNT_OFF);
        const int64_t trow0 = r0 + (int64_t)tile_begin * TM + wm * (TM / WM) + fg * 4;
#pragma unroll 1
        for (int pass = 0; pass < PASSES; ++pass) {
            __syncthreads();
            if (tid < QPP) lcount[tid] = 0;
            __syncthreads();
            if (PASSES == 1 || wn == pass) {
#pragma unroll
                for (int n = 0; n < 4; ++n) {
                    const int qc = (PASSES == 1 ? wn * 64 : 0) + n * 16 + frow;
                    if constexpr (SAMPLE) {
                        int mine = 0;
#pragma unroll
                        for (int m = 0; m < MB; ++m)
#pragma unroll
                            for (int r = 0; r < 4; ++r) mine += acc[m][n][r] > thr[n] ? 1 : 0;
                        int pos = mine > 0 ? atomicAdd(&lcount[qc], mine) : 0;
#pragma unroll
                        for (int m = 0; m < MB; ++m)
#pragma unroll
                            for (int r = 0; r < 4; ++r) {
                                const float sc = acc[m][n][r];
                                if (sc > thr[n]) {
                                    if (pos < LCAP) lists[qc * LCAP + pos] = Cand{sc, (int32_t)(trow0 + m * 16 + r)};
                                    ++pos;
                                }
                            }
                    } else {
                        const int c = min(cnt[n], CAP);
                        if (cnt[n] > CAP) {
                            atomicAdd(&status[0], 1);
                            qflag[q0 + wn * 64 + qc] = 1;
                        }
                        const Cand* src = my_ent + (size_t)n * 16 * CAP;
                        for (int i = 0; i < c; i += 4) {
                            Cand e[4];
#pragma unroll
                            for (int j = 0; j < 4; ++j) e[j] = src[min(i + j, c - 1)];
#pragma unroll
                            for (int j = 0; j < 4; ++j) {
                                if constexpr (DEFER) {
                                    if (i + j < c && isc_row_group_ptr(row_mask...)[e[j].row] == qcode[n]) continue;
                                }
                                if (i + j < c) {
                                    const int pos = atomicAdd(&lcount[qc], 1);
                                    if (pos < LCAP) lists[qc * LCAP + pos] = e[j];
                                }
                            }
                        }
                    }
                }
            }
            __syncthreads();
            {
                const int qc = tid / TPQ, sub = tid % TPQ;
                const int q = q0 + pass * 64 + qc;
                const int c_all = lcount[qc];
                const int c = min(c_all, LCAP);
                int off = 0;
                if (sub == 0 && c > 0) off = atomicAdd(&qcount[q], c);
                off = __shfl(off, lane & ~(TPQ - 1), 64);
                if (sub == 0 && (c_all > LCAP || off + c > QCAP)) {
                    atomicAdd(&status[0], 1);
                    qflag[q] = 1;
                }
                Cand* dst = qlist + (size_t)q * QCAP + off;
                for (int i = sub; i < c; i += TPQ)
                    if (off + i < QCAP) dst[i] = lists[qc * LCAP + i];
            }
        }
    }
}

constexpr int SEL_PER = QCAP / SEL_THREADS;
constexpr int SEL_SPEC_MANY = 4;
struct SelShared {
    unsigned long long surv[SURV_CAP];
    unsigned long long topk[ISC_TOPK_MAX_K + 8];
    unsigned long long wlim[SEL_THREADS];
    unsigned long long lim;
    int ns;
};

__device__ int wg_select_keys(SelShared& sh, const unsigned long long (&key)[SEL_PER + 1], int kp) {
    const int tid = threadIdx.x;
    const int lane = tid & 63;
    const int wave = tid >> 6;
    if (tid == 0) sh.ns = 0;
    unsigned long long lmax = 0ull;
#pragma unroll
    for (int j = 0; j <= SEL_PER; ++j) lmax = key[j] > lmax ? key[j] : lmax;

    if (kp <= 32) {
        int rank = 0;
        for (int j = 0; j < 64; ++j) {
            const unsigned long long o = isc_bcast_key(lmax, j);
            rank += (o > lmax || (o == lmax && j < lane)) ? 1 : 0;
        }
        const unsigned long long mine = (rank == kp - 1) ? lmax : 0ull;
        const unsigned long long lw = isc_wave_max_key(mine);
        if (lane == 0) sh.wlim[wave] = lw;
        __syncthreads();
        unsigned long long lim = sh.wlim[0];
#pragma unroll
        for (int w = 1; w < SEL_THREADS / 64; ++w) lim = sh.wlim[w] > lim ? sh.wlim[w] : lim;
        if (tid == 0) sh.lim = lim;
    } else {
        sh.wlim[tid] = lmax;
        __syncthreads();
        int rank = 0;
        for (int j = 0; j < SEL_THREADS; ++j) {
            const unsigned long long o = sh.wlim[j];
            rank += (o > lmax || (o == lmax && j < tid)) ? 1 : 0;
        }
        if (rank == kp - 1) sh.lim = lmax;
    }
    __syncthreads();
    const unsigned long long lim = sh.lim;

    int mine_n = 0;
#pragma unroll
    for (int j = 0; j <= SEL_PER; ++j) mine_n += (key[j] != 0ull && key[j] >= lim) ? 1 : 0;
    if (mine_n > 0) {
        int pos = atomicAdd(&sh.ns, mine_n);
#pragma unroll
        for (int j = 0; j <= SEL_PER; ++j)
            if (key[j] != 0ull && key[j] >= lim) {
                if (pos < SURV_CAP) sh.surv[pos] = key[j];
                ++pos;
            }
    }
    __syncthreads();
    const int ns = sh.ns;
    if (ns > SURV_CAP) return -1;

    for (int e = tid; e < ns; e += SEL_THREADS) {
        const unsigned long long mine = sh.surv[e];
        int rank = 0;
#pragma unroll 8
        for (int j = 0; j < ns; ++j) rank += sh.surv[j] > mine ? 1 : 0;
        if (rank < kp) sh.topk[rank] = mine;
    }
    __syncthreads();
    return min(kp, ns);
}

template <int SPEC>
__device__ int wg_select(SelShared& sh, int q, int kp, const int32_t* __restrict__ qcount,
                         const Cand* __restrict__ qlist, const float* __restrict__ carry_s,
                         const int32_t* __restrict__ carry_r, const int32_t* __restrict__ carry_n) {
    const int tid = threadIdx.x;
    const Cand* src = qlist + (size_t)q * QCAP;
    const int from_list = min(qcount[q], QCAP);
    const int carried = min(carry_n[q], kp);

    unsigned long long key[SEL_PER + 1];
    {
        const unsigned long long* raw = reinterpret_cast<const unsigned long long*>(src);
#pragma unroll
        for (int j = 0; j < SPEC; ++j) key[j] = raw[tid + SEL_THREADS * j];
        if constexpr (SPEC < SEL_PER) {
            if (from_list > SPEC * SEL_THREADS) {
#pragma unroll
                for (int j = SPEC; j < SEL_PER; ++j) key[j] = raw[tid + SEL_THREADS * j];
            } else {
#pragma unroll
                for (int j = SPEC; j < SEL_PER; ++j) key[j] = 0ull;
            }
        }
        const int ci = min(tid, kp - 1);
        const float cs = carry_s[(size_t)q * kp + ci];
        const int cr = carry_r[(size_t)q * kp + ci];
#pragma unroll
        for (int j = 0; j < SEL_PER; ++j) {
            const Cand e{__uint_as_float((unsigned)key[j]), (int)(unsigned)(key[j] >> 32)};
            key[j] = tid + SEL_THREADS * j < from_list ? isc_make_key(e.s, e.row) : 0ull;
        }
        key[SEL_PER] = tid < carried ? isc_make_key(cs, cr) : 0ull;
    }
    return wg_select_keys(sh, key, kp);
}

template <int SPEC>
__global__ __launch_bounds__(SEL_THREADS, 4) void k_select(int32_t* __restrict__ qcount, const Cand* __restrict__ qlist,
                                                        int kp, float* __restrict__ tau, float* __restrict__ carry_s,
                                                        int32_t* __restrict__ carry_r, int32_t* __restrict__ carry_n,
                                                        int32_t* __restrict__ qflag) {
    __shared__ SelShared sh;
    const int q = blockIdx.x;
    const int n = wg_select<SPEC>(sh, q, kp, qcount, qlist, carry_s, carry_r, carry_n);
    const int tid = threadIdx.x;
    if (n < 0) {
        if (tid == 0) {
            qflag[q] = 1;
            tau[q] = INFINITY;
            carry_n[q] = 0;
            qcount[q] = 0;
        }
        return;
    }
    if (tid < n) {
        const unsigned long long key = sh.topk[tid];
        const float sc = isc_key_score(key);
        carry_s[(size_t)q * kp + tid] = sc;
        carry_r[(size_t)q * kp + tid] = isc_key_row(key);
        if (tid == kp - 1) tau[q] = sc;
    }
    if (tid == 0) {
        carry_n[q] = n;
        qcount[q] = 0;
    }
}

__global__ __launch_bounds__(SEL_THREADS, 2) void k_rescore(const unsigned char* __restrict__ bank, int ks,
                                                            const unsigned char* __restrict__ qpacked, int tnq,
                                                            const float* __restrict__ tau, int32_t* __restrict__ qcount,
                                                            Cand* __restrict__ qlist, int64_t nrows) {
    __shared__ float score[QCAP];
    __shared__ int kept;
    const int q = blockIdx.x;
    const int tid = threadIdx.x, lane = tid & 63, wave = tid >> 6;
    constexpr int NW = SEL_THREADS / 64;
    const int n = min(qcount[q], QCAP);
    Cand* list = qlist + (size_t)q * QCAP;
    const unsigned char* qrow_base = qpacked + ((size_t)(q / tnq) * ks * tnq + (q % tnq)) * ISC_KSTEP_BYTES;
    const int nch = ks * 8;
    float qv[2][8];
#pragma unroll
    for (int h = 0; h < 2; ++h) {
        const int ch = lane + 64 * h;
        uint4 raw = make_uint4(0u, 0u, 0u, 0u);
        if (ch < nch) raw = *reinterpret_cast<const uint4*>(qrow_base + (size_t)(ch >> 3) * tnq * ISC_KSTEP_BYTES + (ch & 7) * 16);
        const _Float16* hv = reinterpret_cast<const _Float16*>(&raw);
#pragma unroll
        for (int j = 0; j < 8; ++j) qv[h][j] = (float)hv[j];
    }
    if (tid == 0) kept = 0;
    for (int c0 = wave; c0 < n; c0 += 4 * NW) {
        float acc[4];
#pragma unroll
        for (int u = 0; u < 4; ++u) {
            const int c = c0 + u * NW;
            int row = c < n ? list[c].row : 0;
            if ((unsigned)row >= (unsigned)nrows) row = 0;
            acc[u] = 0.f;
#pragma unroll
            for (int h = 0; h < 2; ++h) {
                const int ch = lane + 64 * h;
                if (ch < nch) {
                    const uint4 raw = *reinterpret_cast<const uint4*>(bank + isc_packed_offset(row, ch >> 3, ks) + (ch & 7) * 16);
                    const _Float16* hv = reinterpret_cast<const _Float16*>(&raw);
#pragma unroll
                    for (int j = 0; j < 8; ++j) acc[u] = fmaf((float)hv[j], qv[h][j], acc[u]);
                }
            }
        }
#pragma unroll
        for (int u = 0; u < 4; ++u) {
            const float tot = isc_wave_sum(acc[u]);
            if (lane == 0 && c0 + u * NW < n) score[c0 + u * NW] = tot;
        }
    }
    __syncthreads();
    const float t = tau[q];
    int rows[SEL_PER];
#pragma unroll
    for (int j = 0; j < SEL_PER; ++j) rows[j] = tid + SEL_THREADS * j < n ? list[tid + SEL_THREADS * j].row : 0;
    __syncthreads();
#pragma unroll
    for (int j = 0; j < SEL_PER; ++j) {
        const int i = tid + SEL_THREADS * j;
        if (i < n && score[i] > t) list[atomicAdd(&kept, 1)] = Cand{score[i], rows[j]};
    }
    __syncthreads();
    if (tid == 0) qcount[q] = kept;
}

template <typename T, typename RowOf, typename Store>
__device__ void exact_dots(const unsigned char* __restrict__ bank, int ks, const unsigned char* qrow_base, int tnq,
                           int nc, int64_t nrows, RowOf row_of, Store store) {
    const int lane = threadIdx.x & 63, wave = threadIdx.x >> 6;
    const int sub = lane >> 3, ch = lane & 7;
    constexpr int NW = SEL_THREADS / 64;
    for (int c0 = wave; c0 < nc; c0 += 4 * NW) {
        int row[4];
        double acc[4];
#pragma unroll
        for (int u = 0; u < 4; ++u) {
            const int c = c0 + u * NW;
            row[u] = c < nc ? row_of(c) : -1;
            if ((unsigned)row[u] >= (unsigned)nrows) row[u] = -1;
            acc[u] = 0.0;
        }
        for (int s0 = 0; s0 < ks; s0 += 8) {
            const int s = s0 + sub;
            if (s < ks) {
                double a[4][8], b[8];
#pragma unroll
                for (int u = 0; u < 4; ++u)
                    Chunk16<T>::load(bank + isc_packed_offset(row[u] < 0 ? 0 : row[u], s, ks) + ch * 16, a[u]);
                Chunk16<T>::load(qrow_base + (size_t)s * tnq * ISC_KSTEP_BYTES + ch * 16, b);
#pragma unroll
                for (int u = 0; u < 4; ++u)
#pragma unroll
                    for (int j = 0; j < Chunk16<T>::N; ++j) acc[u] = fma(a[u][j], b[j], acc[u]);
            }
        }
#pragma unroll
        for (int u = 0; u < 4; ++u) {
            const double tot = isc_wave_sum(acc[u]);
            if (lane == 0 && c0 + u * NW < nc) store(c0 + u * NW, row[u] < 0 ? 0.0 : tot);
        }
    }
}

struct RedoLists {
    int32_t* r_count;
    int32_t* r_list;
    float* tau2;
    unsigned char* qpacked2;
    int32_t* x_count;
    int32_t* x_list;
};

template <typename T, int SPEC, bool MASK>
__global__ __launch_bounds__(SEL_THREADS, 4) void k_final(
    const unsigned char* __restrict__ bank, int ks, const unsigned char* __restrict__ qpacked, int tnq, int kp, int k,
    IscPerm pm, int64_t index_base, const float* __restrict__ norm_bound, const int32_t* __restrict__ qcount,
    const Cand* __restrict__ qlist, const float* __restrict__ carry_s, const int32_t* __restrict__ carry_r,
    const int32_t* __restrict__ carry_n, const int32_t* __restrict__ qflag, float* __restrict__ out_s,
    int64_t* __restrict__ out_i, RedoLists rl, int32_t* __restrict__ status) {
    __shared__ SelShared sh;
    __shared__ double exact_dot[ISC_TOPK_MAX_K + 8];
    __shared__ float fsc[ISC_TOPK_MAX_K + 8];
    __shared__ int orig[ISC_TOPK_MAX_K + 8];
    __shared__ double qnorm_sh;
    __shared__ float kth_sh;
    __shared__ int slot_sh;
    const int q = blockIdx.x;
    const int tid = threadIdx.x;
    const int n = wg_select<SPEC>(sh, q, kp, qcount, qlist, carry_s, carry_r, carry_n);
    bool redo = n < 0 || qflag[q] != 0;
    const int nc = n < 0 ? 0 : n;

    const unsigned char* qrow_base = qpacked + ((size_t)(q / tnq) * ks * tnq + (q % tnq)) * ISC_KSTEP_BYTES;
    if (tid < 64) {
        const double nn = wave_query_norm<T>(qrow_base, ks, tnq);
        if (tid == 0) qnorm_sh = sqrt(nn);
    }
    exact_dots<T>(bank, ks, qrow_base, tnq, nc, pm.n, [&](int c) { return isc_key_row(sh.topk[c]); },
                  [&](int c, double dot) { exact_dot[c] = dot; });
    __syncthreads();
    const double qnorm = qnorm_sh;
    const double denom = fmax(qnorm, 1e-12);
    const double bmax = norm_bound ? (double)*norm_bound : 1.001;

    if ((qnorm == 0.0 || !(qnorm <= 1.7e308)) && bmax <= 1.7e308) {
        if constexpr (MASK) {
            if (tid == 0) {
                rl.x_list[atomicAdd(rl.x_count, 1)] = q;
                atomicAdd(&status[3], 1);
            }
        } else if (tid < k) {
            out_s[(size_t)q * k + tid] = qnorm == 0.0 ? 0.f : __uint_as_float(0x7fc00000u);
            out_i[(size_t)q * k + tid] = (int64_t)tid + index_base;
        }
        return;
    }

    if (tid < nc) {
        const int row = isc_key_row(sh.topk[tid]);
        fsc[tid] = (float)(exact_dot[tid] / denom);
        orig[tid] = (unsigned)row < (unsigned)pm.n ? (int)isc_perm_orig(pm, row) : 0x7ffffffe;
        if ((unsigned)row >= (unsigned)pm.n) redo = true;
    }
    if (tid == 0) kth_sh = __uint_as_float(0x7fc00000u);
    __syncthreads();
    const double eps = (double)(ks * (ISC_KSTEP_BYTES / (int)sizeof(T))) * (1.0 / 8388608.0) * qnorm * bmax;
    const bool filter_trusted = qnorm >= 1e-30 && qnorm * bmax <= 1e37;
    if (tid < nc) {
        const unsigned long long mykey = isc_make_key(fsc[tid], orig[tid]);
        int rank = 0;
        for (int j = 0; j < nc; ++j) rank += isc_make_key(fsc[j], orig[j]) > mykey ? 1 : 0;
        if (rank < k) {
            out_s[(size_t)q * k + rank] = fsc[tid];
            out_i[(size_t)q * k + rank] = (int64_t)orig[tid] + index_base;
        }
        if (rank == k - 1) kth_sh = fsc[tid];
        if (eps > 0.0) {
            const float ratio = (float)(fabs((double)isc_key_score(sh.topk[tid]) - exact_dot[tid]) / eps);
            if (ratio == ratio) atomicMax(reinterpret_cast<unsigned*>(&status[2]), __float_as_uint(ratio));
        }
    }
    if (MASK && tid >= nc && tid < k) {
        out_s[(size_t)q * k + tid] = __uint_as_float(0x7fc00000u);
        out_i[(size_t)q * k + tid] = INT64_MAX;
    }
    redo = __syncthreads_or(redo ? 1 : 0) != 0;
    if (tid == 0) {
        slot_sh = -1;
        if (!filter_trusted) redo = true;
        if (!redo && (int64_t)nc < pm.n) {
            if (nc < kp) {
                if constexpr (!MASK) redo = true;
            } else {
                const float t = isc_key_score(sh.topk[kp - 1]);
                const float bound = (float)(((double)t + eps) / denom);
                redo = !(bound < kth_sh);
            }
        }
        if (redo) {
            atomicAdd(&status[1], 1);
            const float kth = kth_sh;
            double t2 = (double)__uint_as_float(0x7fc00000u);
            if (filter_trusted && kth == kth && fabsf(kth) <= 3.0e38f) {
                const float kth_dn = nextafterf(kth, -INFINITY);
                const double ed = (double)kth_dn * denom;
                t2 = ed - eps - fabs(ed) * 1e-12;
            }
            if (t2 == t2 && fabs(t2) <= 3.0e38) {
                float tf = (float)t2;
                if ((double)tf >= t2) tf = nextafterf(tf, -INFINITY);
                const int slot = atomicAdd(rl.r_count, 1);
                rl.r_list[slot] = q;
                rl.tau2[slot] = tf;
                slot_sh = slot;
            } else {
                const int slot = atomicAdd(rl.x_count, 1);
                rl.x_list[slot] = q;
                atomicAdd(&status[3], 1);
            }
        }
    }
    __syncthreads();
    const int slot = slot_sh;
    if (slot >= 0) {
        unsigned char* dst = rl.qpacked2 + ((size_t)(slot / tnq) * ks * tnq + (slot % tnq)) * ISC_KSTEP_BYTES;
        for (int i = tid; i < ks * 8; i += SEL_THREADS) {
            const size_t off = (size_t)(i >> 3) * tnq * ISC_KSTEP_BYTES + (i & 7) * 16;
            *reinterpret_cast<uint4*>(dst + off) = *reinterpret_cast<const uint4*>(qrow_base + off);
        }
    }
}

template <typename T>
__global__ __launch_bounds__(SEL_THREADS, 4) void k_final2(
    const unsigned char* __restrict__ bank, int ks, const unsigned char* __restrict__ qpacked2, int tnq, int k, IscPerm pm,
    int64_t index_base, const int32_t* __restrict__ r_count, const int32_t* __restrict__ r_list,
    const int32_t* __restrict__ qcount2, const int32_t* __restrict__ qflag2, Cand* __restrict__ qlist,
    float* __restrict__ out_s, int64_t* __restrict__ out_i, int32_t* __restrict__ x_count, int32_t* __restrict__ x_list,
    int32_t* __restrict__ status) {
    const int slot = blockIdx.x;
    if (slot >= *r_count) return;
    __shared__ SelShared sh;
    __shared__ double qnorm_sh;
    const int tid = threadIdx.x;
    const int q = r_list[slot];
    const int cnt_all = qcount2[slot];
    const int cnt = min(cnt_all, QCAP);
    bool lost = qflag2[slot] != 0 || cnt_all > QCAP || cnt < k;
    const unsigned char* qrow_base = qpacked2 + ((size_t)(slot / tnq) * ks * tnq + (slot % tnq)) * ISC_KSTEP_BYTES;
    if (tid < 64) {
        const double nn = wave_query_norm<T>(qrow_base, ks, tnq);
        if (tid == 0) qnorm_sh = sqrt(nn);
    }
    __syncthreads();
    const double denom = fmax(qnorm_sh, 1e-12);
    Cand* list = qlist + (size_t)slot * QCAP;
    unsigned long long* keys = reinterpret_cast<unsigned long long*>(list);
    int n = -1;
    if (!lost) {
        exact_dots<T>(bank, ks, qrow_base, tnq, cnt, pm.n, [&](int c) { return list[c].row; },
                      [&](int c, double dot) {
                          const int row = list[c].row;
                          keys[c] = (unsigned)row < (unsigned)pm.n
                                        ? isc_make_key((float)(dot / denom), (int)isc_perm_orig(pm, row))
                                        : 0ull;
                      });
        __syncthreads();
        unsigned long long key[SEL_PER + 1];
        const volatile unsigned long long* vkeys = keys;
#pragma unroll
        for (int j = 0; j < SEL_PER; ++j) key[j] = tid + SEL_THREADS * j < cnt ? vkeys[tid + SEL_THREADS * j] : 0ull;
        key[SEL_PER] = 0ull;
        n = wg_select_keys(sh, key, k);
    }
    if (n < k) {
        if (tid == 0) {
            const int xs = atomicAdd(x_count, 1);
            x_list[xs] = q;
            atomicAdd(&status[3], 1);
        }
        return;
    }
    if (tid < k) {
        const unsigned long long key = sh.topk[tid];
        out_s[(size_t)q * k + tid] = isc_key_score(key);
        out_i[(size_t)q * k + tid] = (int64_t)isc_key_row(key) + index_base;
    }
}

#ifdef ISC_ABLATION
int debug_mode() {
    static const int mode = [] {
        const char* e = getenv("ISC_DEBUG_MODE");
        return e ? atoi(e) : 0;
    }();
    return mode;
}
#else
constexpr int debug_mode() { return 0; }
#endif

#ifdef ISC_ABLATION
bool no_nt() {
    static const bool v = getenv("ISC_NO_NT") != nullptr;
    return v;
}
#else
constexpr bool no_nt() { return false; }
#endif

#ifdef ISC_ABLATION
int seg_tiles() {
    static const int v = [] {
        const char* e = getenv("ISC_SEG_TILES");
        return e ? atoi(e) : 128;
    }();
    return v;
}
#else
constexpr int seg_tiles() { return 128; }
#endif

struct FilterIO {
    const unsigned char* qpacked;
    const float* tau;
    int32_t* qcount;
    int32_t* qflag;
    const int32_t* active;
};

template <typename T, int TNQ, typename... RowMask>
void launch_filter(const Level& l, const Plan& p, const Workspace& w, const FilterIO& io, const unsigned char* bank,
                   int ksteps, int32_t* status, hipStream_t stream, RowMask... rm) {
#define ISC_LAUNCH_FILTER(DBG_, SAMPLE_)                                                                              \
    hipLaunchKernelGGL((k_dots_filter<T, TNQ, DBG_, SAMPLE_, RowMask...>), dim3(l.nchunks, p.qtiles), dim3(NTHREADS), \
                       0, stream, bank, l.r0, l.r1, l.tiles_per_chunk, l.ntiles, io.qpacked, ksteps, io.tau, p.qpad,   \
                       w.seg_ent, io.qcount, w.qlist, p.kp, nslots_arg, io.qflag, status, io.active, rm...)
    int nslots_arg = p.nslots;
    if constexpr (TNQ == 128) {
        if (l.sample) ISC_LAUNCH_FILTER(13, true);
        else if (io.active) ISC_LAUNCH_FILTER(33, false);
        else ISC_LAUNCH_FILTER(13, false);
    } else {
    if (l.sample) {
#ifdef ISC_ABLATION
        static const int abl = [] {
            const char* e = getenv("ISC_SAMPLE_ABL");
            return e ? atoi(e) : 0;
        }();
        Plan pa = p;
        pa.nslots |= abl << 16;
        hipLaunchKernelGGL((k_dots_filter<T, TNQ, 12, true, RowMask...>), dim3(l.nchunks, p.qtiles), dim3(NTHREADS), 0,
                           stream, bank, l.r0, l.r1, l.tiles_per_chunk, l.ntiles, io.qpacked, ksteps, io.tau, p.qpad,
                           w.seg_ent, io.qcount, w.qlist, p.kp, pa.nslots, io.qflag, status, io.active, rm...);
#else
        if constexpr (TNQ == 64) {
            if (p.qtiles == 1) ISC_LAUNCH_FILTER(13, true);
            else ISC_LAUNCH_FILTER(12, true);
        } else {
            ISC_LAUNCH_FILTER(12, true);
        }
#endif
        return;
    }
    if (io.active) {
        if (TNQ == 256 && p.qtiles > 1) ISC_LAUNCH_FILTER(32, false);
        else if constexpr (TNQ == 256) ISC_LAUNCH_FILTER(20, false);
        else if (p.qtiles == 1) ISC_LAUNCH_FILTER(33, false);
        else ISC_LAUNCH_FILTER(32, false);
        return;
    }
    int mode = debug_mode();
#ifdef ISC_ABLATION
    static const bool force_split = getenv("ISC_FORCE_SPLIT") != nullptr;
    static const int prio = getenv("ISC_NO_STATIC_PRIO") ? 1 : 0;
    nslots_arg |= prio << 18;
    static const int fabl = getenv("ISC_FILTER_ABL") ? atoi(getenv("ISC_FILTER_ABL")) : 0;
    nslots_arg |= (fabl & 3) << 16;
    if (mode == 0 && TNQ == 256 && p.qtiles > 1 && !force_split) mode = 12;
#else
    if (mode == 0 && TNQ == 256 && p.qtiles > 1) mode = 12;
#endif
    switch (mode) {
#ifdef ISC_ABLATION
        case 2: ISC_LAUNCH_FILTER(2, false); break;
        case 3: ISC_LAUNCH_FILTER(3, false); break;
        case 7: ISC_LAUNCH_FILTER(7, false); break;
        case 11: ISC_LAUNCH_FILTER(11, false); break;
        case 15: ISC_LAUNCH_FILTER(15, false); break;
        case 17: ISC_LAUNCH_FILTER(17, false); break;
        case 22: ISC_LAUNCH_FILTER(22, false); break;
        case 41: ISC_LAUNCH_FILTER(41, false); break;
        case 43: ISC_LAUNCH_FILTER(43, false); break;
        case 48: ISC_LAUNCH_FILTER(48, false); break;
#endif
        case 12: ISC_LAUNCH_FILTER(12, false); break;
        default:
            if constexpr (TNQ == 256) {
                ISC_LAUNCH_FILTER(0, false);
            } else {
                if (p.qtiles == 1 && !no_nt()) ISC_LAUNCH_FILTER(13, false);
                else ISC_LAUNCH_FILTER(12, false);
            }
            break;
    }
    }
#undef ISC_LAUNCH_FILTER
}

template <typename F>
void for_each_segment(const Level& l, const Plan& p, F&& launch) {
    int nseg = 1;
    if (!l.sample && p.qtiles > 1) nseg = isc_ceil_div(l.tiles_per_chunk, seg_tiles());
    const int64_t seg_rows = isc_ceil_div<int64_t>(isc_ceil_div<int64_t>(l.r1 - l.r0, nseg), TM) * TM;
    for (int sg = 0; sg < nseg; ++sg) {
        Level ls = l;
        ls.r0 = l.r0 + sg * seg_rows;
        ls.r1 = ls.r0 + seg_rows < l.r1 ? ls.r0 + seg_rows : l.r1;
        if (ls.r0 >= ls.r1) break;
        ls.ntiles = (int)isc_ceil_div<int64_t>(ls.r1 - ls.r0, TM);
        const int want = l.nchunks < ls.ntiles ? l.nchunks : ls.ntiles;
        ls.tiles_per_chunk = isc_ceil_div(ls.ntiles, want);
        ls.nchunks = isc_ceil_div(ls.ntiles, ls.tiles_per_chunk);
        launch(ls);
    }
}

__host__ inline const uint32_t* pass_filter(const uint32_t* m, int, int, const int32_t*) { return m; }
__host__ inline IscGroups pass_filter(IscGroups g, int q0, int q, const int32_t* slots) {
    g.query_group += q0;
    g.nq = q;
    g.slot_query = slots;
    return g;
}

constexpr int I8_INFLATION = 16;
bool plan_uses_i8(const Plan& p, int d) {
    if (p.tnq != 256 || p.qtiles <= 1 || p.nlevels < 3) return false;
    if ((int64_t)isc_shadow_ksteps(d) * ISC_SHADOW_KSTEP_DIMS * 127 * 127 >= (1 << 24)) return false;
    const Level& l = p.levels[p.nlevels - 1];
    return (double)p.kp * (double)(l.r1 - l.r0) / (double)l.r0 * I8_INFLATION <= (double)p.budget;
}

template <typename T, typename TQ, typename... RowMask>
int run(const void* bank, int64_t n, int d, const void* queries, int q_total, int64_t ldq, int k, int64_t index_base,
        const float* norm_bound, float* out_s, int64_t* out_i, int32_t* status, void* ws_base, hipStream_t stream,
        const void* shadow, RowMask... rm) {
    constexpr bool MASK = sizeof...(RowMask) > 0;
    const Plan p = make_plan(n, q_total, k);
    const bool use_i8 = std::is_same<T, _Float16>::value && !MASK && shadow != nullptr && plan_uses_i8(p, d);
#ifdef ISC_ABLATION
    static const bool thr_inf_set = [] {
        const int v = getenv("ISC_THR_INF") != nullptr;
        return hipMemcpyToSymbol(HIP_SYMBOL(g_abl_thr_inf), &v, sizeof(int)) == hipSuccess;
    }();
    (void)thr_inf_set;
#endif
    const int ksteps = isc_ksteps(d, (int)sizeof(T));
    const Workspace w = carve(p, ksteps, n, k, ws_base);
    const unsigned char* bank_bytes = static_cast<const unsigned char*>(bank);
    const IscPerm pm = isc_make_perm(n);
    for (int q0 = 0; q0 < q_total; q0 += p.qb) {
        const int q = q_total - q0 < p.qb ? q_total - q0 : p.qb;
        const TQ* qptr = static_cast<const TQ*>(queries) + (int64_t)q0 * ldq;
        float* os = out_s + (size_t)q0 * k;
        int64_t* oi = out_i + (size_t)q0 * k;
        const bool spec_all = q <= SMALL_Q;
        hipLaunchKernelGGL((k_prep<T, TQ>), dim3(isc_ceil_div(p.qpad * ksteps * 8, 256)), dim3(256), 0, stream, qptr, ldq, q,
                           d, ksteps, p.qpad, p.tnq, w.qpacked, w.tau, w.carry_n, w.qcount, w.qflag,
                           w.exact.redo_count, w.exact.done, w.r_count, w.tau2, w.qcount2, w.qflag2, status,
                           q0 == 0 ? 1 : 0);
        const int ks8 = isc_shadow_ksteps(d);
        if (use_i8)
            hipLaunchKernelGGL((k_prep_i8<TQ>), dim3(p.qpad / 4), dim3(256), 0, stream, qptr, ldq, q, d, ks8, p.tnq,
                               w.qpacked8, w.qrec8);
        const FilterIO io{w.qpacked, w.tau, w.qcount, w.qflag, nullptr};
        for (int li = 0; li < p.nlevels; ++li) {
            const Level& l = p.levels[li];
            if (use_i8 && li == p.nlevels - 1) {
                const unsigned char* sh = static_cast<const unsigned char*>(shadow);
                const IscShadowArgs sa{reinterpret_cast<const IscShadowRec*>(sh + isc_shadow_data_bytes(n, d)), w.qrec8};
                for_each_segment(l, p, [&](const Level& ls) {
                    isc_timing_begin(ISC_KERNEL_DOTS_FILTER, stream);
                    hipLaunchKernelGGL((k_dots_filter<signed char, 256, 12, false, IscShadowArgs>),
                                       dim3(ls.nchunks, p.qtiles), dim3(NTHREADS), 0, stream, sh, ls.r0, ls.r1,
                                       ls.tiles_per_chunk, ls.ntiles, w.qpacked8, ks8, w.tau, p.qpad, w.seg_ent, w.qcount,
                                       w.qlist, p.kp, p.nslots, w.qflag, status, (const int32_t*)nullptr, sa);
                    isc_timing_end(ISC_KERNEL_DOTS_FILTER, stream);
                });
                hipLaunchKernelGGL(k_rescore, dim3(q), dim3(SEL_THREADS), 0, stream, bank_bytes, ksteps, w.qpacked, p.tnq,
                                   w.tau, w.qcount, w.qlist, n);
                continue;
            }
            for_each_segment(l, p, [&](const Level& ls) {
                isc_timing_begin(ISC_KERNEL_DOTS_FILTER, stream);
                if (p.tnq == 256)
                    launch_filter<T, 256>(ls, p, w, io, bank_bytes, ksteps, status, stream,
                                          pass_filter(rm, q0, q, nullptr)...);
                else if (p.tnq == 128)
                    launch_filter<T, 128>(ls, p, w, io, bank_bytes, ksteps, status, stream,
                                          pass_filter(rm, q0, q, nullptr)...);
                else
                    launch_filter<T, 64>(ls, p, w, io, bank_bytes, ksteps, status, stream,
                                         pass_filter(rm, q0, q, nullptr)...);
                isc_timing_end(ISC_KERNEL_DOTS_FILTER, stream);
            });
            if (li + 1 < p.nlevels) {
                if (spec_all)
                    hipLaunchKernelGGL(k_select<SEL_PER>, dim3(q), dim3(SEL_THREADS), 0, stream, w.qcount, w.qlist, p.kp,
                                       w.tau, w.carry_s, w.carry_r, w.carry_n, w.qflag);
                else
                    hipLaunchKernelGGL(k_select<SEL_SPEC_MANY>, dim3(q), dim3(SEL_THREADS), 0, stream, w.qcount, w.qlist,
                                       p.kp, w.tau, w.carry_s, w.carry_r, w.carry_n, w.qflag);
            }
        }
        const RedoLists rl{w.r_count, w.r_list, w.tau2, w.qpacked2, w.exact.redo_count, w.exact.redo_list};
        if (spec_all)
            hipLaunchKernelGGL((k_final<T, SEL_PER, MASK>), dim3(q), dim3(SEL_THREADS), 0, stream, bank_bytes, ksteps, w.qpacked,
                               p.tnq, p.kp, k, pm, index_base, norm_bound, w.qcount, w.qlist, w.carry_s, w.carry_r,
                               w.carry_n, w.qflag, os, oi, rl, status);
        else
            hipLaunchKernelGGL((k_final<T, SEL_SPEC_MANY, MASK>), dim3(q), dim3(SEL_THREADS), 0, stream, bank_bytes, ksteps,
                               w.qpacked, p.tnq, p.kp, k, pm, index_base, norm_bound, w.qcount, w.qlist, w.carry_s,
                               w.carry_r, w.carry_n, w.qflag, os, oi, rl, status);
        {
            const FilterIO rio{w.qpacked2, w.tau2, w.qcount2, w.qflag2, w.r_count};
            Level all;
            all.r0 = 0;
            all.r1 = n;
            all.sample = 0;
            all.ntiles = (int)isc_ceil_div<int64_t>(n, TM);
            int wgs = TARGET_WGS / p.qtiles;
            if (wgs < 1) wgs = 1;
            const int want = wgs < all.ntiles ? wgs : all.ntiles;
            all.tiles_per_chunk = isc_ceil_div(all.ntiles, want);
            all.nchunks = isc_ceil_div(all.ntiles, all.tiles_per_chunk);
            for_each_segment(all, p, [&](const Level& ls) {
                if (p.tnq == 256)
                    launch_filter<T, 256>(ls, p, w, rio, bank_bytes, ksteps, status, stream,
                                          pass_filter(rm, q0, q, w.r_list)...);
                else if (p.tnq == 128)
                    launch_filter<T, 128>(ls, p, w, rio, bank_bytes, ksteps, status, stream,
                                          pass_filter(rm, q0, q, w.r_list)...);
                else
                    launch_filter<T, 64>(ls, p, w, rio, bank_bytes, ksteps, status, stream,
                                         pass_filter(rm, q0, q, w.r_list)...);
            });
            hipLaunchKernelGGL(k_final2<T>, dim3(q), dim3(SEL_THREADS), 0, stream, bank_bytes, ksteps, w.qpacked2, p.tnq, k,
                               pm, index_base, w.r_count, w.r_list, w.qcount2, w.qflag2, w.qlist, os, oi,
                               w.exact.redo_count, w.exact.redo_list, status);
        }
        int st;
        if constexpr (isc_grouped<RowMask...>())
            st = isc_exact_launch(sizeof(T) == 2 ? ISC_F16 : ISC_F32, bank, n, d, qptr, sizeof(TQ) == 2 ? ISC_F16 : ISC_F32,
                                  ldq, k, index_base, w.exact, os, oi, status, pass_filter(rm, q0, q, nullptr)..., stream);
        else
            st = isc_exact_launch(sizeof(T) == 2 ? ISC_F16 : ISC_F32, bank, n, d, qptr,
                                  sizeof(TQ) == 2 ? ISC_F16 : ISC_F32, ldq, k, index_base, w.exact, os, oi, status,
                                  isc_row_mask_ptr(rm...), stream);
        if (st != ISC_OK) return st;
    }
    return isc_launch_status();
}

int check_args(int dtype, int64_t n, int d, int q, int k) {
    if (dtype != ISC_F16 && dtype != ISC_F32) return ISC_ERR_INVALID_ARG;
    if (n <= 0 || d <= 0 || q <= 0 || k <= 0 || k > n) return ISC_ERR_INVALID_ARG;
    if (k > ISC_TOPK_MAX_K) return ISC_ERR_UNSUPPORTED;
    if (n > 0x7ffffffe) return ISC_ERR_UNSUPPORTED;
    if (d > ISC_SEARCH_MAX_D) return ISC_ERR_UNSUPPORTED;
    if (q > ISC_SEARCH_MAX_Q) return ISC_ERR_UNSUPPORTED;
    return ISC_OK;
}

}

extern "C" int isc_cosine_topk_workspace_bytes(int dtype, int64_t N, int D, int Q, int k, size_t* bytes) {
    ISC_REQUIRE(bytes);
    const int st = check_args(dtype, N, D, Q, k);
    if (st != ISC_OK) return st;
    *bytes = carve(make_plan(N, Q, k), isc_ksteps(D, dtype == ISC_F16 ? 2 : 4), N, k, nullptr).bytes;
    return ISC_OK;
}

namespace {

int topk(const void* bank, int dtype, int64_t N, int D, const void* queries, int q_dtype, int Q, int64_t ldq, int k,
         int64_t index_base, const float* norm_bound, float* out_scores, int64_t* out_indices, int32_t* status,
         void* workspace, size_t workspace_bytes, const uint32_t* row_mask, void* stream,
         const IscGroups* groups = nullptr, const void* shadow = nullptr) {
    ISC_REQUIRE(bank && queries && out_scores && out_indices && status);
    ISC_REQUIRE(q_dtype == ISC_F16 || q_dtype == ISC_F32);
    const int st = check_args(dtype, N, D, Q, k);
    if (st != ISC_OK) return st;
    ISC_REQUIRE(ldq >= D);
    if (!isc_aligned(bank, 16) || !isc_aligned(workspace, 256)) return ISC_ERR_ALIGNMENT;
    size_t need = 0;
    isc_cosine_topk_workspace_bytes(dtype, N, D, Q, k, &need);
    if (!workspace || workspace_bytes < need) return ISC_ERR_WORKSPACE;
#define ISC_RUN(T_, TQ_)                                                                                             \
    return groups   ? run<T_, TQ_>(bank, N, D, queries, Q, ldq, k, index_base, norm_bound, out_scores, out_indices,    \
                                   status, workspace, isc_stream(stream), nullptr, *groups)                                     \
           : row_mask ? run<T_, TQ_>(bank, N, D, queries, Q, ldq, k, index_base, norm_bound, out_scores, out_indices,    \
                                   status, workspace, isc_stream(stream), nullptr, row_mask)                                    \
                    : run<T_, TQ_>(bank, N, D, queries, Q, ldq, k, index_base, norm_bound, out_scores, out_indices,    \
                                   status, workspace, isc_stream(stream), shadow)
    if (dtype == ISC_F16) {
        if (q_dtype == ISC_F16) ISC_RUN(_Float16, _Float16);
        ISC_RUN(_Float16, float);
    }
    if (q_dtype == ISC_F16) ISC_RUN(float, _Float16);
    ISC_RUN(float, float);
#undef ISC_RUN
}

}

extern "C" int isc_cosine_topk(const void* bank, int dtype, int64_t N, int D, const void* queries, int q_dtype, int Q,
                               int64_t ldq, int k, int64_t index_base, const float* norm_bound, float* out_scores,
                               int64_t* out_indices, int32_t* status, void* workspace, size_t workspace_bytes,
                               void* stream) {
    return topk(bank, dtype, N, D, queries, q_dtype, Q, ldq, k, index_base, norm_bound, out_scores, out_indices, status,
                workspace, workspace_bytes, nullptr, stream);
}

extern "C" int isc_cosine_topk_shadow(const void* bank, int dtype, int64_t N, int D, const void* queries, int q_dtype,
                                      int Q, int64_t ldq, int k, int64_t index_base, const float* norm_bound,
                                      float* out_scores, int64_t* out_indices, int32_t* status, void* workspace,
                                      size_t workspace_bytes, const void* shadow, void* stream) {
    ISC_REQUIRE(dtype == ISC_F16 || shadow == nullptr);
    if (!isc_aligned(shadow, 256)) return ISC_ERR_ALIGNMENT;
    return topk(bank, dtype, N, D, queries, q_dtype, Q, ldq, k, index_base, norm_bound, out_scores, out_indices, status,
                workspace, workspace_bytes, nullptr, stream, nullptr, shadow);
}

extern "C" int isc_cosine_topk_uses_shadow(int dtype, int64_t N, int D, int Q, int k, int* uses) {
    ISC_REQUIRE(uses);
    const int st = check_args(dtype, N, D, Q, k);
    if (st != ISC_OK) return st;
    *uses = dtype == ISC_F16 && plan_uses_i8(make_plan(N, Q, k), D) ? 1 : 0;
    return ISC_OK;
}

extern "C" int isc_cosine_topk_masked(const void* bank, int dtype, int64_t N, int D, const void* queries, int q_dtype,
                                      int Q, int64_t ldq, int k, int64_t index_base, const float* norm_bound,
                                      float* out_scores, int64_t* out_indices, int32_t* status, void* workspace,
                                      size_t workspace_bytes, const uint32_t* row_mask, void* stream) {
    ISC_REQUIRE(row_mask);
    return topk(bank, dtype, N, D, queries, q_dtype, Q, ldq, k, index_base, norm_bound, out_scores, out_indices, status,
                workspace, workspace_bytes, row_mask, stream);
}

extern "C" int isc_cosine_topk_grouped(const void* bank, int dtype, int64_t N, int D, const void* queries, int q_dtype,
                                       int Q, int64_t ldq, int k, int64_t index_base, const float* norm_bound,
                                       float* out_scores, int64_t* out_indices, int32_t* status, void* workspace,
                                       size_t workspace_bytes, const uint32_t* row_mask, const int32_t* row_group,
                                       const int32_t* query_group, void* stream) {
    ISC_REQUIRE(row_group && query_group);
    if (!isc_aligned(row_group, 16) || !isc_aligned(query_group, 4) || !isc_aligned(row_mask, 4))
        return ISC_ERR_ALIGNMENT;
    const IscGroups g{row_mask, row_group, query_group, nullptr, Q};
    return topk(bank, dtype, N, D, queries, q_dtype, Q, ldq, k, index_base, norm_bound, out_scores, out_indices, status,
                workspace, workspace_bytes, row_mask, stream, &g);
}

namespace {

constexpr int GH = COLLAPSE_GROUPS;
constexpr int GH_PER = GH / SEL_THREADS;
constexpr int GH_EMPTY = INT32_MIN;
static_assert(GH % SEL_THREADS == 0 && GH_PER <= SEL_PER && GH == 4096, "hash slots per thread; 12-bit hash");

struct GroupHash {
    int code[GH];
    unsigned long long lead[GH];
    unsigned long long sib[GH];
    unsigned sib3[GH];
    unsigned long long tsib[ISC_TOPK_MAX_K + 8];
    unsigned tsib3[ISC_TOPK_MAX_K + 8];
    int tcode[ISC_TOPK_MAX_K + 8];
    int fail;
};

__device__ __forceinline__ int gh_insert(GroupHash& gh, int code) {
    unsigned h = ((unsigned)code * 2654435761u) >> 20;
    for (int probe = 0; probe < GH; ++probe) {
        const int old = atomicCAS(&gh.code[h], GH_EMPTY, code);
        if (old == GH_EMPTY || old == code) return (int)h;
        h = (h + 1) & (GH - 1);
    }
    return -1;
}

__device__ void gh_clear(GroupHash& gh) {
    for (int i = threadIdx.x; i < GH; i += SEL_THREADS) {
        gh.code[i] = GH_EMPTY;
        gh.lead[i] = 0ull;
        gh.sib[i] = 0ull;
        gh.sib3[i] = 0u;
    }
    if (threadIdx.x == 0) gh.fail = 0;
}

__device__ int gh_select(SelShared& sh, GroupHash& gh, int kp) {
    const int tid = threadIdx.x;
    unsigned long long lk[SEL_PER + 1];
#pragma unroll
    for (int j = 0; j <= SEL_PER; ++j) lk[j] = j < GH_PER ? gh.lead[tid + SEL_THREADS * j] : 0ull;
    const int n = wg_select_keys(sh, lk, kp);
    if (n <= 0) return n;
    const unsigned long long last = sh.topk[n - 1];
#pragma unroll
    for (int j = 0; j < GH_PER; ++j)
        if (lk[j] != 0ull && lk[j] >= last) {
            int lo = 0, hi = n - 1;
            while (lo < hi) {
                const int mid = (lo + hi) >> 1;
                if (sh.topk[mid] > lk[j]) lo = mid + 1;
                else hi = mid;
            }
            gh.tsib[lo] = gh.sib[tid + SEL_THREADS * j];
            gh.tsib3[lo] = gh.sib3[tid + SEL_THREADS * j];
            gh.tcode[lo] = gh.code[tid + SEL_THREADS * j];
        }
    __syncthreads();
    return n;
}

template <int SPEC>
__device__ int wg_select_groups(SelShared& sh, GroupHash& gh, int q, int kp, const int32_t* __restrict__ qcount,
                                const Cand* __restrict__ qlist, const float* __restrict__ carry_s,
                                const int32_t* __restrict__ carry_r, const unsigned long long* __restrict__ carry_sib,
                                const uint32_t* __restrict__ carry_sib3, const int32_t* __restrict__ carry_n,
                                const int32_t* __restrict__ row_group, int64_t nrows) {
    const int tid = threadIdx.x;
    const Cand* src = qlist + (size_t)q * QCAP;
    const int from_list = min(qcount[q], QCAP);
    const int carried = min(carry_n[q], kp);
    gh_clear(gh);
    constexpr int NK = SEL_PER + 2;
    unsigned long long key[NK];
    unsigned csib3 = 0u;
    {
        const unsigned long long* raw = reinterpret_cast<const unsigned long long*>(src);
#pragma unroll
        for (int j = 0; j < SPEC; ++j) key[j] = raw[tid + SEL_THREADS * j];
        if constexpr (SPEC < SEL_PER) {
            if (from_list > SPEC * SEL_THREADS) {
#pragma unroll
                for (int j = SPEC; j < SEL_PER; ++j) key[j] = raw[tid + SEL_THREADS * j];
            } else {
#pragma unroll
                for (int j = SPEC; j < SEL_PER; ++j) key[j] = 0ull;
            }
        }
        const int ci = min(tid, kp - 1);
        const float cs = carry_s[(size_t)q * kp + ci];
        const int cr = carry_r[(size_t)q * kp + ci];
        csib3 = tid < carried ? carry_sib3[(size_t)q * kp + ci] : 0u;
        key[SEL_PER + 1] = tid < carried ? carry_sib[(size_t)q * kp + ci] : 0ull;
#pragma unroll
        for (int j = 0; j < SEL_PER; ++j) {
            const Cand e{__uint_as_float((unsigned)key[j]), (int)(unsigned)(key[j] >> 32)};
            key[j] = tid + SEL_THREADS * j < from_list ? isc_make_key(e.s, e.row) : 0ull;
        }
        key[SEL_PER] = tid < carried ? isc_make_key(cs, cr) : 0ull;
    }
    __syncthreads();
    int slot[NK];
    bool fail = false;
#pragma unroll
    for (int j = 0; j < NK; ++j) {
        slot[j] = -1;
        if (key[j] != 0ull) {
            const int row = isc_key_row(key[j]);
            const int s = (unsigned)row < (unsigned)nrows ? gh_insert(gh, row_group[row]) : -1;
            if (s < 0) {
                fail = true;
            } else {
                slot[j] = s;
                atomicMax(&gh.lead[s], key[j]);
            }
        }
    }
    if (csib3 != 0u && slot[SEL_PER] >= 0) atomicMax(&gh.sib3[slot[SEL_PER]], csib3);
    if (fail) gh.fail = 1;
    __syncthreads();
#pragma unroll
    for (int j = 0; j < NK; ++j)
        if (slot[j] >= 0 && key[j] != gh.lead[slot[j]]) atomicMax(&gh.sib[slot[j]], key[j]);
    __syncthreads();
#pragma unroll
    for (int j = 0; j < NK; ++j)
        if (slot[j] >= 0 && key[j] != gh.lead[slot[j]] && key[j] != gh.sib[slot[j]])
            atomicMax(&gh.sib3[slot[j]], (unsigned)(key[j] >> 32));
    __syncthreads();
    if (gh.fail) return -1;
    return gh_select(sh, gh, kp);
}

template <int SPEC>
__global__ __launch_bounds__(SEL_THREADS) void k_select_groups(int32_t* __restrict__ qcount, const Cand* __restrict__ qlist,
                                                               int kp, float* __restrict__ tau, float* __restrict__ carry_s,
                                                               int32_t* __restrict__ carry_r,
                                                               unsigned long long* __restrict__ carry_sib,
                                                               uint32_t* __restrict__ carry_sib3,
                                                               int32_t* __restrict__ carry_n, int32_t* __restrict__ qflag,
                                                               const int32_t* __restrict__ row_group, int64_t nrows) {
    __shared__ SelShared sh;
    __shared__ GroupHash gh;
    const int q = blockIdx.x;
    const int n = wg_select_groups<SPEC>(sh, gh, q, kp, qcount, qlist, carry_s, carry_r, carry_sib, carry_sib3, carry_n,
                                         row_group, nrows);
    const int tid = threadIdx.x;
    if (n < 0) {
        if (tid == 0) {
            qflag[q] = 1;
            tau[q] = INFINITY;
            carry_n[q] = 0;
            qcount[q] = 0;
        }
        return;
    }
    if (tid < n) {
        const unsigned long long key = sh.topk[tid];
        const float sc = isc_key_score(key);
        carry_s[(size_t)q * kp + tid] = sc;
        carry_r[(size_t)q * kp + tid] = isc_key_row(key);
        carry_sib[(size_t)q * kp + tid] = gh.tsib[tid];
        carry_sib3[(size_t)q * kp + tid] = gh.tsib3[tid];
        if (tid == kp - 1) tau[q] = sc;
    }
    if (tid == 0) {
        carry_n[q] = n;
        qcount[q] = 0;
    }
}

template <typename T, int SPEC>
__global__ __launch_bounds__(SEL_THREADS) void k_final_groups(
    const unsigned char* __restrict__ bank, int ks, const unsigned char* __restrict__ qpacked, int tnq, int kp, int k,
    IscPerm pm, int64_t index_base, const float* __restrict__ norm_bound, const int32_t* __restrict__ qcount,
    const Cand* __restrict__ qlist, const float* __restrict__ carry_s, const int32_t* __restrict__ carry_r,
    const unsigned long long* __restrict__ carry_sib, const uint32_t* __restrict__ carry_sib3,
    const int32_t* __restrict__ carry_n, const int32_t* __restrict__ qflag, const int32_t* __restrict__ row_group,
    float* __restrict__ out_s, int64_t* __restrict__ out_i, int32_t* __restrict__ out_c, RedoLists rl,
    int32_t* __restrict__ status) {
    constexpr int MAXG = ISC_TOPK_MAX_K + 8;
    __shared__ SelShared sh;
    __shared__ GroupHash gh;
    __shared__ double exact_dot[2 * MAXG];
    __shared__ unsigned long long gkey[MAXG];
    __shared__ int rank_sh[MAXG];
    __shared__ double qnorm_sh;
    __shared__ float kth_sh;
    __shared__ int slot_sh;
    const int q = blockIdx.x;
    const int tid = threadIdx.x;
    const int n = wg_select_groups<SPEC>(sh, gh, q, kp, qcount, qlist, carry_s, carry_r, carry_sib, carry_sib3, carry_n,
                                         row_group, pm.n);
    bool redo = n < 0 || qflag[q] != 0;
    const int nc = n < 0 ? 0 : n;

    const unsigned char* qrow_base = qpacked + ((size_t)(q / tnq) * ks * tnq + (q % tnq)) * ISC_KSTEP_BYTES;
    if (tid < 64) {
        const double nn = wave_query_norm<T>(qrow_base, ks, tnq);
        if (tid == 0) qnorm_sh = sqrt(nn);
    }
    exact_dots<T>(bank, ks, qrow_base, tnq, 2 * nc, pm.n,
                  [&](int c) { return c < nc ? isc_key_row(sh.topk[c]) : gh.tsib[c - nc] ? isc_key_row(gh.tsib[c - nc]) : -1; },
                  [&](int c, double dot) { exact_dot[c < nc ? c : MAXG + c - nc] = dot; });
    __syncthreads();
    const double qnorm = qnorm_sh;
    const double denom = fmax(qnorm, 1e-12);
    const double bmax = norm_bound ? (double)*norm_bound : 1.001;

    if ((qnorm == 0.0 || !(qnorm <= 1.7e308)) && bmax <= 1.7e308) {
        if (tid == 0) {
            rl.x_list[atomicAdd(rl.x_count, 1)] = q;
            atomicAdd(&status[3], 1);
        }
        return;
    }

    if (tid < nc) {
        const int row = isc_key_row(sh.topk[tid]);
        if ((unsigned)row >= (unsigned)pm.n) redo = true;
        unsigned long long best =
            (unsigned)row < (unsigned)pm.n ? isc_make_key((float)(exact_dot[tid] / denom), (int)isc_perm_orig(pm, row)) : 0ull;
        const unsigned long long sib = gh.tsib[tid];
        if (sib != 0ull) {
            const int srow = isc_key_row(sib);
            if ((unsigned)srow < (unsigned)pm.n) {
                const unsigned long long sk =
                    isc_make_key((float)(exact_dot[MAXG + tid] / denom), (int)isc_perm_orig(pm, srow));
                best = sk > best ? sk : best;
            } else {
                redo = true;
            }
        }
        gkey[tid] = best;
    }
    if (tid == 0) kth_sh = __uint_as_float(0x7fc00000u);
    __syncthreads();
    const double eps = (double)(ks * (ISC_KSTEP_BYTES / (int)sizeof(T))) * (1.0 / 8388608.0) * qnorm * bmax;
    const bool filter_trusted = qnorm >= 1e-30 && qnorm * bmax <= 1e37;
    if (tid < nc) {
        const unsigned long long mykey = gkey[tid];
        int rank = 0;
        for (int j = 0; j < nc; ++j) rank += gkey[j] > mykey ? 1 : 0;
        rank_sh[tid] = rank;
        if (rank < k) {
            out_s[(size_t)q * k + rank] = isc_key_score(mykey);
            out_i[(size_t)q * k + rank] = (int64_t)isc_key_row(mykey) + index_base;
            out_c[(size_t)q * k + rank] = gh.tcode[tid];
        }
        if (rank == k - 1) kth_sh = isc_key_score(mykey);
        if (eps > 0.0) {
            const float ratio = (float)(fabs((double)isc_key_score(sh.topk[tid]) - exact_dot[tid]) / eps);
            if (ratio == ratio) atomicMax(reinterpret_cast<unsigned*>(&status[2]), __float_as_uint(ratio));
        }
    }
    if (tid >= nc && tid < k) {
        out_s[(size_t)q * k + tid] = __uint_as_float(0x7fc00000u);
        out_i[(size_t)q * k + tid] = INT64_MAX;
        out_c[(size_t)q * k + tid] = -1;
    }
    __syncthreads();
    if (tid < nc && gh.tsib3[tid] != 0u) {
        const float sf = isc_key_score((unsigned long long)gh.tsib3[tid] << 32);
        const float ub = (float)(((double)sf + eps) / denom);
        const float lim = rank_sh[tid] < k ? isc_key_score(gkey[tid]) : kth_sh;
        if (!(ub < lim)) redo = true;
    }
    redo = __syncthreads_or(redo ? 1 : 0) != 0;
    if (tid == 0) {
        slot_sh = -1;
        if (!filter_trusted) redo = true;
        if (!redo && nc >= kp) {
            const float t = isc_key_score(sh.topk[kp - 1]);
            const float bound = (float)(((double)t + eps) / denom);
            redo = !(bound < kth_sh);
        }
        if (redo) {
            atomicAdd(&status[1], 1);
            const float kth = kth_sh;
            double t2 = (double)__uint_as_float(0x7fc00000u);
            if (filter_trusted && kth == kth && fabsf(kth) <= 3.0e38f) {
                const float kth_dn = nextafterf(kth, -INFINITY);
                const double ed = (double)kth_dn * denom;
                t2 = ed - eps - fabs(ed) * 1e-12;
            }
            if (t2 == t2 && fabs(t2) <= 3.0e38) {
                float tf = (float)t2;
                if ((double)tf >= t2) tf = nextafterf(tf, -INFINITY);
                const int slot = atomicAdd(rl.r_count, 1);
                rl.r_list[slot] = q;
                rl.tau2[slot] = tf;
                slot_sh = slot;
            } else {
                const int slot = atomicAdd(rl.x_count, 1);
                rl.x_list[slot] = q;
                atomicAdd(&status[3], 1);
            }
        }
    }
    __syncthreads();
    const int slot = slot_sh;
    if (slot >= 0) {
        unsigned char* dst = rl.qpacked2 + ((size_t)(slot / tnq) * ks * tnq + (slot % tnq)) * ISC_KSTEP_BYTES;
        for (int i = tid; i < ks * 8; i += SEL_THREADS) {
            const size_t off = (size_t)(i >> 3) * tnq * ISC_KSTEP_BYTES + (i & 7) * 16;
            *reinterpret_cast<uint4*>(dst + off) = *reinterpret_cast<const uint4*>(qrow_base + off);
        }
    }
}

template <typename T>
__global__ __launch_bounds__(SEL_THREADS) void k_final2_groups(
    const unsigned char* __restrict__ bank, int ks, const unsigned char* __restrict__ qpacked2, int tnq, int k, IscPerm pm,
    int64_t index_base, const int32_t* __restrict__ r_count, const int32_t* __restrict__ r_list,
    const int32_t* __restrict__ qcount2, const int32_t* __restrict__ qflag2, const Cand* __restrict__ qlist,
    const int32_t* __restrict__ row_group, float* __restrict__ out_s, int64_t* __restrict__ out_i,
    int32_t* __restrict__ out_c, int32_t* __restrict__ x_count, int32_t* __restrict__ x_list,
    int32_t* __restrict__ status) {
    const int slot = blockIdx.x;
    if (slot >= *r_count) return;
    __shared__ SelShared sh;
    __shared__ GroupHash gh;
    __shared__ double qnorm_sh;
    const int tid = threadIdx.x;
    const int q = r_list[slot];
    const int cnt_all = qcount2[slot];
    const int cnt = min(cnt_all, QCAP);
    const bool lost = qflag2[slot] != 0 || cnt_all > QCAP || cnt < k;
    const unsigned char* qrow_base = qpacked2 + ((size_t)(slot / tnq) * ks * tnq + (slot % tnq)) * ISC_KSTEP_BYTES;
    gh_clear(gh);
    if (tid < 64) {
        const double nn = wave_query_norm<T>(qrow_base, ks, tnq);
        if (tid == 0) qnorm_sh = sqrt(nn);
    }
    __syncthreads();
    const double denom = fmax(qnorm_sh, 1e-12);
    const Cand* list = qlist + (size_t)slot * QCAP;
    int n = -1;
    if (!lost) {
        exact_dots<T>(bank, ks, qrow_base, tnq, cnt, pm.n, [&](int c) { return list[c].row; },
                      [&](int c, double dot) {
                          const int row = list[c].row;
                          if ((unsigned)row < (unsigned)pm.n) {
                              const int s = gh_insert(gh, row_group[row]);
                              if (s < 0) gh.fail = 1;
                              else atomicMax(&gh.lead[s], isc_make_key((float)(dot / denom), (int)isc_perm_orig(pm, row)));
                          }
                      });
        __syncthreads();
        if (!gh.fail) n = gh_select(sh, gh, k);
    }
    if (n < k) {
        if (tid == 0) {
            const int xs = atomicAdd(x_count, 1);
            x_list[xs] = q;
            atomicAdd(&status[3], 1);
        }
        return;
    }
    if (tid < k) {
        const unsigned long long key = sh.topk[tid];
        out_s[(size_t)q * k + tid] = isc_key_score(key);
        out_i[(size_t)q * k + tid] = (int64_t)isc_key_row(key) + index_base;
        out_c[(size_t)q * k + tid] = gh.tcode[tid];
    }
}

__global__ void k_fill_i32(int32_t* p, int n, int v) {
    const int i = blockIdx.x * blockDim.x + threadIdx.x;
    if (i < n) p[i] = v;
}

struct CollapseWs {
    unsigned long long* carry_sib;
    uint32_t* carry_sib3;
    int32_t* qnone;
    int32_t* part_code;
    size_t bytes;
};

CollapseWs carve_collapse(const Plan& p, int ks, int64_t n, int k, void* base) {
    CollapseWs c;
    size_t off = carve(p, ks, n, k, nullptr).bytes;
    auto take = [&](size_t bytes) {
        void* ptr = base ? static_cast<char*>(base) + off : nullptr;
        off += isc_align_up(bytes, 256);
        return ptr;
    };
    c.carry_sib = static_cast<unsigned long long*>(take((size_t)p.qpad * p.kp * 8));
    c.carry_sib3 = static_cast<uint32_t*>(take((size_t)p.qpad * p.kp * 4));
    c.qnone = static_cast<int32_t*>(take((size_t)p.qpad * 4));
    c.part_code = static_cast<int32_t*>(take(isc_exact_collapse_ws_bytes(n, p.qb, k) - isc_exact_ws_bytes(n, p.qb, k)));
    c.bytes = off;
    return c;
}

template <typename T, typename TQ>
int run_collapse(const void* bank, int64_t n, int d, const void* queries, int q_total, int64_t ldq, int k,
                 int64_t index_base, const float* norm_bound, float* out_s, int64_t* out_i, int32_t* out_c,
                 int32_t* status, void* ws_base, hipStream_t stream, const IscGroups& g, int group_rows) {
    const Plan p = make_plan(n, q_total, k, group_rows);
    const int ksteps = isc_ksteps(d, (int)sizeof(T));
    const Workspace w = carve(p, ksteps, n, k, ws_base);
    const CollapseWs cw = carve_collapse(p, ksteps, n, k, ws_base);
    const unsigned char* bank_bytes = static_cast<const unsigned char*>(bank);
    const IscPerm pm = isc_make_perm(n);
    if (!g.query_group)
        hipLaunchKernelGGL(k_fill_i32, dim3(isc_ceil_div(p.qpad, 256)), dim3(256), 0, stream, cw.qnone, p.qpad, -1);
    for (int q0 = 0; q0 < q_total; q0 += p.qb) {
        const int q = q_total - q0 < p.qb ? q_total - q0 : p.qb;
        const TQ* qptr = static_cast<const TQ*>(queries) + (int64_t)q0 * ldq;
        float* os = out_s + (size_t)q0 * k;
        int64_t* oi = out_i + (size_t)q0 * k;
        int32_t* oc = out_c + (size_t)q0 * k;
        const bool spec_all = q <= SMALL_Q;
        hipLaunchKernelGGL((k_prep<T, TQ>), dim3(isc_ceil_div(p.qpad * ksteps * 8, 256)), dim3(256), 0, stream, qptr, ldq, q,
                           d, ksteps, p.qpad, p.tnq, w.qpacked, w.tau, w.carry_n, w.qcount, w.qflag,
                           w.exact.redo_count, w.exact.done, w.r_count, w.tau2, w.qcount2, w.qflag2, status,
                           q0 == 0 ? 1 : 0);
        IscGroups gp = g;
        gp.query_group = g.query_group ? g.query_group + q0 : cw.qnone;
        gp.nq = q;
        gp.slot_query = nullptr;
        IscGroups gr = gp;
        gr.slot_query = w.r_list;
        const FilterIO io{w.qpacked, w.tau, w.qcount, w.qflag, nullptr};
        for (int li = 0; li < p.nlevels; ++li) {
            const Level& l = p.levels[li];
            for_each_segment(l, p, [&](const Level& ls) {
                isc_timing_begin(ISC_KERNEL_DOTS_FILTER, stream);
                if (p.tnq == 256) launch_filter<T, 256>(ls, p, w, io, bank_bytes, ksteps, status, stream, gp);
                else if (p.tnq == 128) launch_filter<T, 128>(ls, p, w, io, bank_bytes, ksteps, status, stream, gp);
                else launch_filter<T, 64>(ls, p, w, io, bank_bytes, ksteps, status, stream, gp);
                isc_timing_end(ISC_KERNEL_DOTS_FILTER, stream);
            });
            if (li + 1 < p.nlevels) {
                if (spec_all)
                    hipLaunchKernelGGL(k_select_groups<SEL_PER>, dim3(q), dim3(SEL_THREADS), 0, stream, w.qcount, w.qlist,
                                       p.kp, w.tau, w.carry_s, w.carry_r, cw.carry_sib, cw.carry_sib3, w.carry_n, w.qflag, g.row_group,
                                       n);
                else
                    hipLaunchKernelGGL(k_select_groups<SEL_SPEC_MANY>, dim3(q), dim3(SEL_THREADS), 0, stream, w.qcount,
                                       w.qlist, p.kp, w.tau, w.carry_s, w.carry_r, cw.carry_sib, cw.carry_sib3, w.carry_n,
                                       w.qflag, g.row_group, n);
            }
        }
        const RedoLists rl{w.r_count, w.r_list, w.tau2, w.qpacked2, w.exact.redo_count, w.exact.redo_list};
        if (spec_all)
            hipLaunchKernelGGL((k_final_groups<T, SEL_PER>), dim3(q), dim3(SEL_THREADS), 0, stream, bank_bytes, ksteps,
                               w.qpacked, p.tnq, p.kp, k, pm, index_base, norm_bound, w.qcount, w.qlist, w.carry_s,
                               w.carry_r, cw.carry_sib, cw.carry_sib3, w.carry_n, w.qflag, g.row_group, os, oi, oc, rl,
                               status);
        else
            hipLaunchKernelGGL((k_final_groups<T, SEL_SPEC_MANY>), dim3(q), dim3(SEL_THREADS), 0, stream, bank_bytes, ksteps,
                               w.qpacked, p.tnq, p.kp, k, pm, index_base, norm_bound, w.qcount, w.qlist, w.carry_s,
                               w.carry_r, cw.carry_sib, cw.carry_sib3, w.carry_n, w.qflag, g.row_group, os, oi, oc, rl,
                               status);
        {
            const FilterIO rio{w.qpacked2, w.tau2, w.qcount2, w.qflag2, w.r_count};
            Level all;
            all.r0 = 0;
            all.r1 = n;
            all.sample = 0;
            all.ntiles = (int)isc_ceil_div<int64_t>(n, TM);
            int wgs = TARGET_WGS / p.qtiles;
            if (wgs < 1) wgs = 1;
            const int want = wgs < all.ntiles ? wgs : all.ntiles;
            all.tiles_per_chunk = isc_ceil_div(all.ntiles, want);
            all.nchunks = isc_ceil_div(all.ntiles, all.tiles_per_chunk);
            for_each_segment(all, p, [&](const Level& ls) {
                if (p.tnq == 256) launch_filter<T, 256>(ls, p, w, rio, bank_bytes, ksteps, status, stream, gr);
                else if (p.tnq == 128) launch_filter<T, 128>(ls, p, w, rio, bank_bytes, ksteps, status, stream, gr);
                else launch_filter<T, 64>(ls, p, w, rio, bank_bytes, ksteps, status, stream, gr);
            });
            hipLaunchKernelGGL(k_final2_groups<T>, dim3(q), dim3(SEL_THREADS), 0, stream, bank_bytes, ksteps, w.qpacked2,
                               p.tnq, k, pm, index_base, w.r_count, w.r_list, w.qcount2, w.qflag2, w.qlist, g.row_group,
                               os, oi, oc, w.exact.redo_count, w.exact.redo_list, status);
        }
        const int st = isc_exact_collapse_launch(sizeof(T) == 2 ? ISC_F16 : ISC_F32, bank, n, d, qptr,
                                                 sizeof(TQ) == 2 ? ISC_F16 : ISC_F32, ldq, k, index_base, w.exact,
                                                 cw.part_code, os, oi, oc, gp, stream);
        if (st != ISC_OK) return st;
    }
    return isc_launch_status();
}

}

extern "C" int isc_cosine_topk_collapse_workspace_bytes(int dtype, int64_t N, int D, int Q, int k, int max_group_rows,
                                                        size_t* bytes) {
    ISC_REQUIRE(bytes);
    ISC_REQUIRE(max_group_rows >= 1);
    const int st = check_args(dtype, N, D, Q, k);
    if (st != ISC_OK) return st;
    const int ks = isc_ksteps(D, dtype == ISC_F16 ? 2 : 4);
    *bytes = carve_collapse(make_plan(N, Q, k, max_group_rows), ks, N, k, nullptr).bytes;
    return ISC_OK;
}

extern "C" int isc_cosine_topk_collapse(const void* bank, int dtype, int64_t N, int D, const void* queries, int q_dtype,
                                        int Q, int64_t ldq, int k, int64_t index_base, const float* norm_bound,
                                        float* out_scores, int64_t* out_indices, int32_t* status, void* workspace,
                                        size_t workspace_bytes, const uint32_t* row_mask, const int32_t* row_group,
                                        const int32_t* query_group, int max_group_rows, int32_t* out_codes,
                                        void* stream) {
    ISC_REQUIRE(bank && queries && out_scores && out_indices && out_codes && status && row_group);
    ISC_REQUIRE(q_dtype == ISC_F16 || q_dtype == ISC_F32);
    ISC_REQUIRE(max_group_rows >= 1);
    const int st = check_args(dtype, N, D, Q, k);
    if (st != ISC_OK) return st;
    ISC_REQUIRE(ldq >= D);
    if (!isc_aligned(row_group, 16) || !isc_aligned(query_group, 4) || !isc_aligned(row_mask, 4) ||
        !isc_aligned(out_codes, 4))
        return ISC_ERR_ALIGNMENT;
    if (!isc_aligned(bank, 16) || !isc_aligned(workspace, 256)) return ISC_ERR_ALIGNMENT;
    size_t need = 0;
    isc_cosine_topk_collapse_workspace_bytes(dtype, N, D, Q, k, max_group_rows, &need);
    if (!workspace || workspace_bytes < need) return ISC_ERR_WORKSPACE;
    const IscGroups g{row_mask, row_group, query_group, nullptr, Q};
    hipStream_t s = isc_stream(stream);
#define ISC_RUN_COLLAPSE(T_, TQ_)                                                                                      \
    return run_collapse<T_, TQ_>(bank, N, D, queries, Q, ldq, k, index_base, norm_bound, out_scores, out_indices,      \
                                 out_codes, status, workspace, s, g, max_group_rows)
    if (dtype == ISC_F16) {
        if (q_dtype == ISC_F16) ISC_RUN_COLLAPSE(_Float16, _Float16);
        ISC_RUN_COLLAPSE(_Float16, float);
    }
    if (q_dtype == ISC_F16) ISC_RUN_COLLAPSE(float, _Float16);
    ISC_RUN_COLLAPSE(float, float);
#undef ISC_RUN_COLLAPSE
}
```

### include/imagescry_hip.h

```cpp
#ifndef IMAGESCRY_HIP_H
#define IMAGESCRY_HIP_H

#include <stddef.h>
#include <stdint.h>

#ifdef __cplusplus
extern "C" {
#endif

#define ISC_ABI_VERSION 4

#define ISC_U8 0
#define ISC_F16 1
#define ISC_F32 2

#define ISC_OK 0
#define ISC_ERR_INVALID_ARG (-1)
#define ISC_ERR_UNSUPPORTED (-2)
#define ISC_ERR_WORKSPACE (-3)
#define ISC_ERR_LAUNCH (-4)
#define ISC_ERR_NO_DEVICE (-5)
#define ISC_ERR_ALIGNMENT (-6)

#define ISC_ACT_NONE 0
#define ISC_ACT_RELU 1
#define ISC_ACT_GELU 2
#define ISC_ACT_SILU 3
#define ISC_ACT_SIGMOID 4
#define ISC_ACT_RESIDUAL_AFTER 0x100

int isc_abi_version(void);
#define ISC_BUILD_ABLATION 1
int isc_build_flags(void);
const char* isc_strerror(int status);
int isc_device_info(int* num_cus, int* lds_bytes_per_cu, char* arch_name, int arch_name_len);

#define ISC_KERNEL_DOTS_FILTER 0
#define ISC_KERNEL_CONV 1
#define ISC_KERNEL_GEMM_F16 2
#define ISC_KERNEL_COUNT 3
int isc_timing_enable(int enable);
int isc_timing_read(int kernel_id, double* total_ms, int* launches);


int isc_channel_stats_workspace_bytes(int dtype, int B, int C, int H, int W, size_t* bytes);
int isc_channel_stats(const void* x, int dtype, int B, int C, int H, int W, float* mean, float* stdev,
                      void* workspace, size_t workspace_bytes, void* stream);

int isc_normalize_clip(const void* x, int dtype, int B, int C, int H, int W, const float* mean, const float* stdev,
                       int stat_batch, float eps, float lo, float hi, float* y, void* stream);

int isc_normalize_clip_nhwc4(const void* x, int dtype, int B, int C, int H, int W, const float* mean, const float* stdev,
                             int stat_batch, float eps, float lo, float hi, float* y, void* stream);

int isc_resize_bilinear(const void* x, int dtype, int planes, int H1, int W1, int H2, int W2, float* y, void* stream);

int isc_l2norm_channels(const float* x, int B, int E, int S, float eps, float* y, void* stream);

int isc_bank_packed_bytes(int dtype, int64_t N, int D, size_t* bytes);

int isc_bank_permutation(int64_t N, int64_t* mul, int64_t* mul_inv);

int isc_bank_pack(const void* rows, int in_dtype, int64_t n_rows, int D, int64_t ldx, int64_t first_row,
                  int64_t n_total, int normalize, float eps, void* packed, int dtype, float* norm_bound, void* stream);

int isc_bank_unpack(const void* packed, int dtype, int D, int64_t n_total, int64_t first_row, int64_t n_rows,
                    void* rows, int64_t ldy, void* stream);

int isc_bank_append(const void* rows, int in_dtype, int64_t n_rows, int D, int64_t ldx, int64_t first_row,
                    int64_t capacity, int normalize, float eps, void* packed, int dtype, float* norm_bound,
                    uint32_t* fill_mask, const int32_t* codes, int32_t* packed_codes, void* stream);

int isc_bank_repack(const void* src_packed, int64_t src_capacity, void* dst_packed, int64_t dst_capacity, int dtype, int D,
                    int64_t first_row, int64_t n_rows, const int32_t* src_codes, int32_t* dst_codes,
                    uint32_t* dst_fill_mask, void* stream);

int isc_row_mask_words(int64_t N, size_t* words);

int isc_row_mask_pack(const uint8_t* allow, int64_t N, uint32_t* packed_mask, int64_t* allowed_count, void* stream);

int isc_row_groups_pack(const int32_t* codes, int64_t N, int32_t* packed_codes, void* stream);


int isc_nchw_to_nhwc(const float* x, int B, int C, int H, int W, int Cpad, float* y, void* stream);

int isc_conv2d_nhwc(const float* x, int B, int H, int W, int Cin, const float* w, int Cout, int R, int S, int stride,
                    int pad, const float* bias, const float* residual, int act, float* out, void* stream);

int isc_conv2d_nhwc_dual(const float* x, int B, int H, int W, int Cin, const float* x2, int H2, int W2, int Cin2,
                         int stride2, const float* w, int Cout, const float* bias, const float* residual, int act,
                         float* out, void* stream);

int isc_conv2d_nhwc_gated(const float* x, int B, int H, int W, int Cin, const float* gate, const float* w, int Cout, int R,
                          int S, int stride, int pad, const float* bias, const float* residual, int act, float* out,
                          void* stream);

int isc_dwconv2d_nhwc(const float* x, int B, int H, int W, int C, const float* w, int R, int stride, int pad,
                      const float* bias, int act, float* y, void* stream);

int isc_dwconv2d_nhwc_pool(const float* x, int B, int H, int W, int C, const float* w, int R, int stride, int pad,
                           const float* bias, int act, const float* gate, float* y, float* pooled, void* stream);

int isc_se_gate(const float* pooled, int B, int C, const float* w1, int ld1, const float* b1, int S, const float* w2,
                int ld2, const float* b2, float* gate, void* stream);

int isc_linear_centered(const float* x, int64_t n, int F, const float* mean, const float* w, int K, const float* bias,
                        float* out, void* stream);

int isc_im2col_nchw(const float* x, int B, int C, int H, int W, int R, int S, int stride, int pad, int Kpad, float* y,
                    void* stream);

int isc_maxpool_nhwc(const float* x, int B, int H, int W, int C, int R, int stride, int pad, float* y, void* stream);

int isc_global_avgpool_nhwc(const float* x, int B, int H, int W, int C, float* y, void* stream);

int isc_pool_linear_l2norm(const float* x, int B, int H, int W, int C, const float* w, const float* bias, int E,
                           int normalize, float eps, float* out, void* stream);


#define ISC_GEMM_A_PACKED 1
#define ISC_GEMM_W_PACKED 2
#define ISC_GEMM_OUT_PACKED 4
#define ISC_GEMM_TILE_256 8
#define ISC_GEMM_TILE_128 16

int isc_gemm_f16(const void* a, int64_t M, int K, const void* w, int N, const float* bias, const float* residual,
                 int act, void* out, int out_dtype, int flags, void* stream);

int isc_layernorm(const float* x, int64_t rows, int D, int64_t ldx, const float* gamma, const float* beta, float eps,
                  void* y, int y_dtype, int64_t ldy, int y_packed, void* stream);

int isc_attention_f16(const void* qkv, int B, int T, int heads, int head_dim, void* out, int packed, void* stream);

int isc_patchify_f16(const float* x, int B, int C, int H, int W, int patch, void* patches, int packed, void* stream);

int isc_vit_assemble(const float* patch_embed, const float* cls_token, const float* pos_embed, int B, int T, int D,
                     float* tokens, void* stream);

int isc_vit_pos_resample(const float* pos_embed, int g, int h, int w, int D, float* out, void* stream);

int isc_vit_tokens_out(const float* tokens, int B, int T, int D, const float* gamma, const float* beta, float eps,
                       int normalize, float l2_eps, float* out, void* stream);


int isc_feature_sums_workspace_bytes(int64_t n, int F, size_t* bytes);
int isc_feature_sums(const float* x, int64_t n, int F, int64_t ldx, double* sums, void* workspace, size_t workspace_bytes,
                     void* stream);

int isc_center_transpose(const float* x, int64_t n, int F, int64_t ldx, const float* mean, float* xt, int Fpad,
                         int64_t ldn, void* stream);

int isc_gram_rows(const float* xt, int F, int64_t n, float* gram, void* stream);


#define ISC_TOPK_MAX_K 120
#define ISC_SEARCH_MAX_D 8192
#define ISC_SEARCH_MAX_Q (1 << 24)
#define ISC_SEARCH_PASS_QUERIES 1024
int isc_cosine_topk_workspace_bytes(int dtype, int64_t N, int D, int Q, int k, size_t* bytes);
int isc_cosine_topk(const void* bank, int dtype, int64_t N, int D, const void* queries, int q_dtype, int Q, int64_t ldq,
                    int k, int64_t index_base, const float* norm_bound, float* out_scores, int64_t* out_indices,
                    int32_t* status, void* workspace, size_t workspace_bytes, void* stream);

int isc_bank_shadow_bytes(int64_t N, int D, size_t* bytes);
int isc_bank_quantize(const void* packed, int64_t N, int D, void* shadow, size_t shadow_bytes, void* stream);
int isc_cosine_topk_uses_shadow(int dtype, int64_t N, int D, int Q, int k, int* uses);
int isc_cosine_topk_shadow(const void* bank, int dtype, int64_t N, int D, const void* queries, int q_dtype, int Q,
                           int64_t ldq, int k, int64_t index_base, const float* norm_bound, float* out_scores,
                           int64_t* out_indices, int32_t* status, void* workspace, size_t workspace_bytes,
                           const void* shadow, void* stream);

int isc_cosine_topk_masked(const void* bank, int dtype, int64_t N, int D, const void* queries, int q_dtype, int Q,
                           int64_t ldq, int k, int64_t index_base, const float* norm_bound, float* out_scores,
                           int64_t* out_indices, int32_t* status, void* workspace, size_t workspace_bytes,
                           const uint32_t* row_mask, void* stream);

int isc_cosine_topk_grouped(const void* bank, int dtype, int64_t N, int D, const void* queries, int q_dtype, int Q,
                            int64_t ldq, int k, int64_t index_base, const float* norm_bound, float* out_scores,
                            int64_t* out_indices, int32_t* status, void* workspace, size_t workspace_bytes,
                            const uint32_t* row_mask, const int32_t* row_group, const int32_t* query_group, void* stream);

int isc_cosine_topk_exhaustive_workspace_bytes(int dtype, int64_t N, int D, int Q, int k, size_t* bytes);
int isc_cosine_topk_exhaustive(const void* bank, int dtype, int64_t N, int D, const void* queries, int q_dtype, int Q,
                               int64_t ldq, int k, int64_t index_base, float* out_scores, int64_t* out_indices,
                               void* workspace, size_t workspace_bytes, void* stream);

int isc_cosine_topk_exhaustive_masked(const void* bank, int dtype, int64_t N, int D, const void* queries, int q_dtype,
                                      int Q, int64_t ldq, int k, int64_t index_base, float* out_scores,
                                      int64_t* out_indices, void* workspace, size_t workspace_bytes,
                                      const uint32_t* row_mask, void* stream);

int isc_cosine_topk_exhaustive_grouped(const void* bank, int dtype, int64_t N, int D, const void* queries, int q_dtype,
                                       int Q, int64_t ldq, int k, int64_t index_base, float* out_scores,
                                       int64_t* out_indices, void* workspace, size_t workspace_bytes,
                                       const uint32_t* row_mask, const int32_t* row_group, const int32_t* query_group,
                                       void* stream);

int isc_cosine_range_workspace_bytes(int dtype, int64_t N, int D, int Q, int64_t capacity, size_t* bytes);
int isc_cosine_range(const void* bank, int dtype, int64_t N, int D, const void* queries, int q_dtype, int Q, int64_t ldq,
                     const float* min_score, int64_t index_base, const float* norm_bound, int64_t capacity,
                     int64_t* offsets, float* scores, int64_t* indices, int64_t* needed, int32_t* status,
                     void* workspace, size_t workspace_bytes, void* stream);

int isc_cosine_range_masked(const void* bank, int dtype, int64_t N, int D, const void* queries, int q_dtype, int Q,
                            int64_t ldq, const float* min_score, int64_t index_base, const float* norm_bound,
                            int64_t capacity, int64_t* offsets, float* scores, int64_t* indices, int64_t* needed,
                            int32_t* status, void* workspace, size_t workspace_bytes, const uint32_t* row_mask,
                            void* stream);

int isc_cosine_range_grouped(const void* bank, int dtype, int64_t N, int D, const void* queries, int q_dtype, int Q,
                             int64_t ldq, const float* min_score, int64_t index_base, const float* norm_bound,
                             int64_t capacity, int64_t* offsets, float* scores, int64_t* indices, int64_t* needed,
                             int32_t* status, void* workspace, size_t workspace_bytes, const uint32_t* row_mask,
                             const int32_t* row_group, const int32_t* query_group, void* stream);

int isc_topk_merge(const float* scores, const int64_t* indices, int G, int Q, int kin, int kout, int64_t stride_g_scores,
                   int64_t stride_g_indices, float* out_scores, int64_t* out_indices, void* stream);

int isc_cosine_topk_collapse_workspace_bytes(int dtype, int64_t N, int D, int Q, int k, int max_group_rows,
                                             size_t* bytes);
int isc_cosine_topk_collapse(const void* bank, int dtype, int64_t N, int D, const void* queries, int q_dtype, int Q,
                             int64_t ldq, int k, int64_t index_base, const float* norm_bound, float* out_scores,
                             int64_t* out_indices, int32_t* status, void* workspace, size_t workspace_bytes,
                             const uint32_t* row_mask, const int32_t* row_group, const int32_t* query_group,
                             int max_group_rows, int32_t* out_codes, void* stream);

int isc_cosine_topk_exhaustive_collapse_workspace_bytes(int dtype, int64_t N, int D, int Q, int k, size_t* bytes);
int isc_cosine_topk_exhaustive_collapse(const void* bank, int dtype, int64_t N, int D, const void* queries, int q_dtype,
                                        int Q, int64_t ldq, int k, int64_t index_base, float* out_scores,
                                        int64_t* out_indices, void* workspace, size_t workspace_bytes,
                                        const uint32_t* row_mask, const int32_t* row_group, const int32_t* query_group,
                                        int32_t* out_codes, void* stream);

int isc_topk_merge_groups(const float* scores, const int64_t* indices, const int64_t* labels, int G, int Q, int kin,
                          int kout, int64_t stride_g_scores, int64_t stride_g_indices, int64_t stride_g_labels,
                          float* out_scores, int64_t* out_indices, int64_t* out_labels, void* stream);

#ifdef __cplusplus
}
#endif
#endif
```

Baseline: 119,200 queries/s.

## Extend int8 shadow filtering to intermediate levels with slack bands and exact rescoring

Runs the int8 shadow-bank filter on every non-sample level, not only the last one. Intermediate levels use a per-query slack derived from global shadow residual statistics, which narrows the candidate margin. Candidates that fall inside the uncertain band go straight to a per-query list and are rescored in fp16 by a new band-rescore kernel. That kernel also maintains a tau floor, which is passed to the final kernel. The aim is to cut fp16 bank reads at the earlier levels. The cost is extra rescoring, atomics, a stats kernel at quantize time, and more complex correctness bookkeeping.

```diff
diff --git a/imagescry_amd/_lib.py b/imagescry_amd/_lib.py
--- a/imagescry_amd/_lib.py
+++ b/imagescry_amd/_lib.py
@@ -146,6 +146,7 @@
     "isc_bank_shadow_bytes": (c_int, [c_int64, c_int, POINTER(c_size_t)]),
     "isc_bank_quantize": (c_int, [c_void_p, c_int64, c_int, c_void_p, c_size_t, c_void_p]),
     "isc_cosine_topk_uses_shadow": (c_int, [c_int, c_int64, c_int, c_int, c_int, POINTER(c_int)]),
+    "isc_cosine_topk_shadow_levels": (c_int, [c_int, c_int64, c_int, c_int, c_int, POINTER(c_int)]),
     "isc_cosine_topk_shadow": (
         c_int,
         [c_void_p, c_int, c_int64, c_int, c_void_p, c_int, c_int, c_int64, c_int, c_int64, c_void_p, c_void_p, c_void_p,
diff --git a/imagescry_amd/csrc/bank_layout.h b/imagescry_amd/csrc/bank_layout.h
--- a/imagescry_amd/csrc/bank_layout.h
+++ b/imagescry_amd/csrc/bank_layout.h
@@ -28,10 +28,15 @@
 __host__ __device__ inline size_t isc_shadow_data_bytes(int64_t n, int d) {
     return (size_t)((n + ISC_TILE_ROWS - 1) / ISC_TILE_ROWS) * isc_shadow_ksteps(d) * ISC_TILE_KSTEP_BYTES;
 }
-__host__ __device__ inline size_t isc_shadow_bytes(int64_t n, int d) {
+struct IscShadowStats {
+    float resid_max, resid_mean;
+    float norm_max, norm_mean;
+};
+__host__ __device__ inline size_t isc_shadow_stats_offset(int64_t n, int d) {
     const size_t rec = (size_t)((n + ISC_TILE_ROWS - 1) / ISC_TILE_ROWS) * sizeof(IscShadowRec);
     return isc_shadow_data_bytes(n, d) + (rec + 255) / 256 * 256;
 }
+__host__ __device__ inline size_t isc_shadow_bytes(int64_t n, int d) { return isc_shadow_stats_offset(n, d) + 256; }
 
 struct IscPerm {
     int64_t n;
diff --git a/imagescry_amd/csrc/bank_pack.hip b/imagescry_amd/csrc/bank_pack.hip
--- a/imagescry_amd/csrc/bank_pack.hip
+++ b/imagescry_amd/csrc/bank_pack.hip
@@ -227,6 +227,52 @@
         rec.resid = (float)sqrt(rmax) * (1.f + 1e-6f);
         rec.qnorm = bad ? INFINITY : (float)sqrt(qmax) * (1.f + 1e-6f);
         recs[tile] = rec;
+    }
+}
+
+__global__ __launch_bounds__(1024) void k_bank_shadow_stats(const IscShadowRec* __restrict__ recs, int64_t tiles,
+                                                           IscShadowStats* __restrict__ stats) {
+    __shared__ double sum_sh[2][1024];
+    __shared__ float max_sh[2][1024];
+    __shared__ long long cnt_sh[1024];
+    const int tid = threadIdx.x;
+    double se = 0.0, sn = 0.0;
+    float me = 0.f, mn = 0.f;
+    long long cnt = 0;
+    for (int64_t t = tid; t < tiles; t += 1024) {
+        const IscShadowRec r = recs[t];
+        const float e = r.resid / r.inv_scale, nn = (r.qnorm + r.resid) / r.inv_scale;
+        if (!(e <= 3.0e38f) || !(nn <= 3.0e38f)) continue;
+        se += (double)e;
+        sn += (double)nn;
+        me = fmaxf(me, e);
+        mn = fmaxf(mn, nn);
+        ++cnt;
+    }
+    sum_sh[0][tid] = se;
+    sum_sh[1][tid] = sn;
+    max_sh[0][tid] = me;
+    max_sh[1][tid] = mn;
+    cnt_sh[tid] = cnt;
+    __syncthreads();
+    for (int off = 512; off > 0; off >>= 1) {
+        if (tid < off) {
+            sum_sh[0][tid] += sum_sh[0][tid + off];
+            sum_sh[1][tid] += sum_sh[1][tid + off];
+            max_sh[0][tid] = fmaxf(max_sh[0][tid], max_sh[0][tid + off]);
+            max_sh[1][tid] = fmaxf(max_sh[1][tid], max_sh[1][tid + off]);
+            cnt_sh[tid] += cnt_sh[tid + off];
+        }
+        __syncthreads();
+    }
+    if (tid == 0) {
+        const double inv = cnt_sh[0] > 0 ? 1.0 / (double)cnt_sh[0] : 0.0;
+        IscShadowStats s;
+        s.resid_max = max_sh[0][0];
+        s.resid_mean = (float)(sum_sh[0][0] * inv);
+        s.norm_max = max_sh[1][0];
+        s.norm_mean = (float)(sum_sh[1][0] * inv);
+        *stats = s;
     }
 }
 
@@ -418,5 +464,8 @@
     hipLaunchKernelGGL(k_bank_quantize, dim3((unsigned)tiles), dim3(256), 0, isc_stream(stream),
                        static_cast<const unsigned char*>(packed), isc_ksteps(D, 2), isc_shadow_ksteps(D), out,
                        reinterpret_cast<IscShadowRec*>(out + isc_shadow_data_bytes(N, D)));
-    return isc_launch_status();
-}
+    hipLaunchKernelGGL(k_bank_shadow_stats, dim3(1), dim3(1024), 0, isc_stream(stream),
+                       reinterpret_cast<const IscShadowRec*>(out + isc_shadow_data_bytes(N, D)), tiles,
+                       reinterpret_cast<IscShadowStats*>(out + isc_shadow_stats_offset(N, D)));
+    return isc_launch_status();
+}
diff --git a/imagescry_amd/csrc/cosine_topk.hip b/imagescry_amd/csrc/cosine_topk.hip
--- a/imagescry_amd/csrc/cosine_topk.hip
+++ b/imagescry_amd/csrc/cosine_topk.hip
@@ -163,6 +163,7 @@
     IscExactWs exact;
     unsigned char* qpacked8;
     float4* qrec8;
+    float* tau_floor;
     size_t bytes;
 };
 
@@ -194,6 +195,7 @@
     const int ks8 = (ks + 1) / 2;
     w.qpacked8 = static_cast<unsigned char*>(take((size_t)p.qpad * ks8 * ISC_KSTEP_BYTES));
     w.qrec8 = static_cast<float4*>(take((size_t)p.qpad * sizeof(float4)));
+    w.tau_floor = static_cast<float*>(take((size_t)p.qpad * 4));
     w.bytes = off;
     return w;
 }
@@ -243,7 +245,8 @@
 template <typename TQ>
 __global__ __launch_bounds__(256) void k_prep_i8(const TQ* __restrict__ queries, int64_t ldq, int q, int d, int ks8,
                                                  int tnq, unsigned char* __restrict__ packed8,
-                                                 float4* __restrict__ qrec) {
+                                                 float4* __restrict__ qrec, const IscShadowStats* __restrict__ stats,
+                                                 float* __restrict__ tau_floor) {
     const int lane = threadIdx.x & 63;
     const int qrow = blockIdx.x * 4 + (threadIdx.x >> 6);
     const TQ* src = queries + (int64_t)qrow * ldq;
@@ -282,9 +285,18 @@
     }
     rs = isc_wave_sum(rs);
     qs = isc_wave_sum(qs);
-    if (lane == 0)
-        qrec[qrow] = make_float4(live ? c : __uint_as_float(0x7fc00000u), (float)sqrt(qs) * (1.f + 1e-6f),
-                                 (float)sqrt(rs) * (1.f + 1e-6f), 0.f);
+    if (lane == 0) {
+        const float qn = (float)sqrt(qs) * (1.f + 1e-6f), eq = (float)sqrt(rs) * (1.f + 1e-6f);
+        float sq = 0.f;
+        if (live) {
+            const IscShadowStats st = *stats;
+            const float e = fminf(st.resid_max, 4.f * st.resid_mean), nn = fminf(st.norm_max, 4.f * st.norm_mean);
+            sq = (float)((((double)qn * (double)e + (double)eq * (double)nn) / (double)c) * (1.0 + 1e-6));
+            if (!(sq >= 0.f && sq <= 3.0e38f)) sq = 0.f;
+        }
+        qrec[qrow] = make_float4(live ? c : __uint_as_float(0x7fc00000u), qn, eq, sq);
+        tau_floor[qrow] = -INFINITY;
+    }
 }
 
 template <typename T>
@@ -356,6 +368,7 @@
     const IscShadowRec* recs;
     const float4* qrec;
 };
+struct IscShadowSlackArgs : IscShadowArgs {};
 
 #define ISC_DS_READ(dst_, addr_, off_) \
     asm volatile("ds_read_b128 %0, %1 offset:%2" : "=v"(dst_) : "v"(addr_), "i"(off_))
@@ -407,6 +420,8 @@
                                                           int32_t* __restrict__ qflag, int32_t* __restrict__ status,
                                                           const int32_t* __restrict__ active, RowMask... row_mask) {
     constexpr bool I8 = std::is_same<T, signed char>::value;
+    constexpr bool SLACKED = (std::is_same<RowMask, IscShadowSlackArgs>::value || ...);
+    static_assert(!SLACKED || I8, "the slack belongs to the int8 test");
     typedef typename Mma<T>::Acc Acc;
     constexpr bool MASK = sizeof...(RowMask) > 0 && !I8;
     constexpr bool GROUP = isc_grouped<RowMask...>();
@@ -468,7 +483,7 @@
 #endif
         cnt[n] = 0;
     }
-    [[maybe_unused]] float qn8[4], eq8[4];
+    [[maybe_unused]] float qn8[4], eq8[4], sq8[4];
     if constexpr (I8) {
         const IscShadowArgs& sa = (row_mask, ...);
 #pragma unroll
@@ -477,6 +492,7 @@
             thr[n] *= qr.x;
             qn8[n] = qr.y;
             eq8[n] = qr.z;
+            if constexpr (SLACKED) sq8[n] = qr.w * qr.x;
         }
     }
 
@@ -987,11 +1003,20 @@
             if constexpr (GROUP && !DEFER) apply_codes(MBE_C{}, tile_codes);
             if constexpr (I8) {
                 int thr_i[4];
+                [[maybe_unused]] unsigned direct = 0u;
 #pragma unroll
                 for (int n = 0; n < 4; ++n) {
                     const float t = thr[n] * tile_ct;
                     const float mg = fmaf(qn8[n], tile_et, eq8[n] * (tile_nt + tile_et));
-                    const float lo = (t - mg) - (fabsf(t) + mg) * 9.5367431640625e-7f - 1e-30f;
+                    float lo;
+                    if constexpr (SLACKED) {
+                        const float sc = sq8[n] * tile_ct;
+                        const float left = fmaxf(mg - sc, 0.f);
+                        lo = (t - left) - (fabsf(t) + mg + sc) * 9.5367431640625e-7f - 1e-30f;
+                        if (left > 0.f) direct |= 1u << n;
+                    } else {
+                        lo = (t - mg) - (fabsf(t) + mg) * 9.5367431640625e-7f - 1e-30f;
+                    }
                     thr_i[n] = !(lo <= 2.0e9f) ? INT32_MAX : lo < -2.0e9f ? INT32_MIN : (int)floorf(lo);
                     if (!(tile_nt < INFINITY)) thr_i[n] = thr[n] < INFINITY ? INT32_MIN : INT32_MAX;
                 }
@@ -1021,9 +1046,21 @@
 #pragma unroll
                             for (int r = 0; r < 4; ++r) {
                                 if (acc[m][n][r] > thr_i[n]) {
-                                    const int pos = cnt[n]++;
-                                    if (pos < CAP)
-                                        my_ent[n * 16 * CAP + pos] = Cand{(float)acc[m][n][r], (int32_t)(trow0 + m * 16 + r)};
+                                    const Cand e{SLACKED ? (float)acc[m][n][r] / tile_ct : (float)acc[m][n][r],
+                                                 (int32_t)(trow0 + m * 16 + r)};
+                                    if (SLACKED && ((direct >> n) & 1u)) {
+                                        const int q = q0 + wn * 64 + n * 16 + frow;
+                                        const int pos = atomicAdd(&qcount[q], 1);
+                                        if (pos < QCAP) {
+                                            qlist[(size_t)q * QCAP + pos] = e;
+                                        } else {
+                                            atomicAdd(&status[0], 1);
+                                            qflag[q] = 1;
+                                        }
+                                    } else {
+                                        const int pos = cnt[n]++;
+                                        if (pos < CAP) my_ent[n * 16 * CAP + pos] = e;
+                                    }
                                 }
                             }
                         }
@@ -1393,6 +1430,51 @@
     }
 }
 
+__device__ __forceinline__ void rescore_load_query(const unsigned char* qrow_base, int ks, int tnq, float (&qv)[2][8]) {
+    const int lane = threadIdx.x & 63;
+#pragma unroll
+    for (int h = 0; h < 2; ++h) {
+        const int ch = lane + 64 * h;
+        uint4 raw = make_uint4(0u, 0u, 0u, 0u);
+        if (ch < ks * 8) raw = *reinterpret_cast<const uint4*>(qrow_base + (size_t)(ch >> 3) * tnq * ISC_KSTEP_BYTES + (ch & 7) * 16);
+        const _Float16* hv = reinterpret_cast<const _Float16*>(&raw);
+#pragma unroll
+        for (int j = 0; j < 8; ++j) qv[h][j] = (float)hv[j];
+    }
+}
+template <typename RowOf, typename Store>
+__device__ __forceinline__ void rescore_dots(const unsigned char* __restrict__ bank, int ks, const float (&qv)[2][8], int n,
+                                             int64_t nrows, RowOf row_of, Store store) {
+    const int lane = threadIdx.x & 63, wave = threadIdx.x >> 6;
+    constexpr int NW = SEL_THREADS / 64;
+    const int nch = ks * 8;
+    for (int c0 = wave; c0 < n; c0 += 4 * NW) {
+        float acc[4];
+#pragma unroll
+        for (int u = 0; u < 4; ++u) {
+            const int c = c0 + u * NW;
+            int row = c < n ? row_of(c) : 0;
+            if ((unsigned)row >= (unsigned)nrows) row = 0;
+            acc[u] = 0.f;
+#pragma unroll
+            for (int h = 0; h < 2; ++h) {
+                const int ch = lane + 64 * h;
+                if (ch < nch) {
+                    const uint4 raw = *reinterpret_cast<const uint4*>(bank + isc_packed_offset(row, ch >> 3, ks) + (ch & 7) * 16);
+                    const _Float16* hv = reinterpret_cast<const _Float16*>(&raw);
+#pragma unroll
+                    for (int j = 0; j < 8; ++j) acc[u] = fmaf((float)hv[j], qv[h][j], acc[u]);
+                }
+            }
+        }
+#pragma unroll
+        for (int u = 0; u < 4; ++u) {
+            const float tot = isc_wave_sum(acc[u]);
+            if (lane == 0 && c0 + u * NW < n) store(c0 + u * NW, tot);
+        }
+    }
+}
+
 __global__ __launch_bounds__(SEL_THREADS, 2) void k_rescore(const unsigned char* __restrict__ bank, int ks,
                                                             const unsigned char* __restrict__ qpacked, int tnq,
                                                             const float* __restrict__ tau, int32_t* __restrict__ qcount,
@@ -1400,48 +1482,13 @@
     __shared__ float score[QCAP];
     __shared__ int kept;
     const int q = blockIdx.x;
-    const int tid = threadIdx.x, lane = tid & 63, wave = tid >> 6;
-    constexpr int NW = SEL_THREADS / 64;
+    const int tid = threadIdx.x;
     const int n = min(qcount[q], QCAP);
     Cand* list = qlist + (size_t)q * QCAP;
-    const unsigned char* qrow_base = qpacked + ((size_t)(q / tnq) * ks * tnq + (q % tnq)) * ISC_KSTEP_BYTES;
-    const int nch = ks * 8;
     float qv[2][8];
-#pragma unroll
-    for (int h = 0; h < 2; ++h) {
-        const int ch = lane + 64 * h;
-        uint4 raw = make_uint4(0u, 0u, 0u, 0u);
-        if (ch < nch) raw = *reinterpret_cast<const uint4*>(qrow_base + (size_t)(ch >> 3) * tnq * ISC_KSTEP_BYTES + (ch & 7) * 16);
-        const _Float16* hv = reinterpret_cast<const _Float16*>(&raw);
-#pragma unroll
-        for (int j = 0; j < 8; ++j) qv[h][j] = (float)hv[j];
-    }
+    rescore_load_query(qpacked + ((size_t)(q / tnq) * ks * tnq + (q % tnq)) * ISC_KSTEP_BYTES, ks, tnq, qv);
     if (tid == 0) kept = 0;
-    for (int c0 = wave; c0 < n; c0 += 4 * NW) {
-        float acc[4];
-#pragma unroll
-        for (int u = 0; u < 4; ++u) {
-            const int c = c0 + u * NW;
-            int row = c < n ? list[c].row : 0;
-            if ((unsigned)row >= (unsigned)nrows) row = 0;
-            acc[u] = 0.f;
-#pragma unroll
-            for (int h = 0; h < 2; ++h) {
-                const int ch = lane + 64 * h;
-                if (ch < nch) {
-                    const uint4 raw = *reinterpret_cast<const uint4*>(bank + isc_packed_offset(row, ch >> 3, ks) + (ch & 7) * 16);
-                    const _Float16* hv = reinterpret_cast<const _Float16*>(&raw);
-#pragma unroll
-                    for (int j = 0; j < 8; ++j) acc[u] = fmaf((float)hv[j], qv[h][j], acc[u]);
-                }
-            }
-        }
-#pragma unroll
-        for (int u = 0; u < 4; ++u) {
-            const float tot = isc_wave_sum(acc[u]);
-            if (lane == 0 && c0 + u * NW < n) score[c0 + u * NW] = tot;
-        }
-    }
+    rescore_dots(bank, ks, qv, n, nrows, [&](int c) { return list[c].row; }, [&](int c, float dot) { score[c] = dot; });
     __syncthreads();
     const float t = tau[q];
     int rows[SEL_PER];
@@ -1453,6 +1500,111 @@
         const int i = tid + SEL_THREADS * j;
         if (i < n && score[i] > t) list[atomicAdd(&kept, 1)] = Cand{score[i], rows[j]};
     }
+    __syncthreads();
+    if (tid == 0) qcount[q] = kept;
+}
+
+__global__ __launch_bounds__(SEL_THREADS, 2) void k_rescore_band(const unsigned char* __restrict__ bank, int ks,
+                                                                 const unsigned char* __restrict__ qpacked, int tnq, int kp,
+                                                                 const float* __restrict__ tau, float* __restrict__ tau_floor,
+                                                                 const float4* __restrict__ qrec,
+                                                                 const IscShadowRec* __restrict__ recs,
+                                                                 int32_t* __restrict__ qcount, Cand* __restrict__ qlist,
+                                                                 int64_t nrows) {
+    __shared__ SelShared sh;
+    __shared__ float score[QCAP];
+    __shared__ unsigned short work[QCAP];
+    __shared__ int nwork, kept;
+    __shared__ float taup_sh;
+    const int q = blockIdx.x;
+    const int tid = threadIdx.x;
+    const int n = min(qcount[q], QCAP);
+    Cand* list = qlist + (size_t)q * QCAP;
+    const float4 qr = qrec[q];
+    if (tid == 0) {
+        const double f = (double)tau[q] + (double)qr.w;
+        float up = (float)f;
+        if ((double)up < f) up = nextafterf(up, INFINITY);
+        if (!(up == up)) up = INFINITY;
+        tau_floor[q] = fmaxf(tau_floor[q], up);
+        nwork = 0;
+        kept = 0;
+        taup_sh = -INFINITY;
+    }
+    if (n == 0) return;
+    float qv[2][8];
+    rescore_load_query(qpacked + ((size_t)(q / tnq) * ks * tnq + (q % tnq)) * ISC_KSTEP_BYTES, ks, tnq, qv);
+
+    unsigned long long key[SEL_PER + 1];
+    float mt[SEL_PER];
+#pragma unroll
+    for (int j = 0; j < SEL_PER; ++j) {
+        const int i = tid + SEL_THREADS * j;
+        key[j] = 0ull;
+        mt[j] = INFINITY;
+        if (i < n) {
+            const Cand e = list[i];
+            float p = -INFINITY;
+            if ((unsigned)e.row < (unsigned)nrows) {
+                const IscShadowRec rec = recs[e.row >> 8];
+                const float m = fmaf(qr.y, rec.resid, qr.z * (rec.qnorm + rec.resid)) / rec.inv_scale * (1.f + 1e-6f);
+                if (m <= 3.0e38f && e.s == e.s) {
+                    mt[j] = m;
+                    p = e.s;
+                }
+            }
+            key[j] = isc_make_key(p, e.row);
+        }
+    }
+    key[SEL_PER] = 0ull;
+    const int width = min(4 * kp, ISC_TOPK_MAX_K + 8);
+    const int na = wg_select_keys(sh, key, width);
+    const unsigned long long lim_a = na > 0 ? sh.topk[na - 1] : 0ull;
+    unsigned done = 0u;
+#pragma unroll
+    for (int j = 0; j < SEL_PER; ++j)
+        if (key[j] != 0ull && key[j] >= lim_a) {
+            work[atomicAdd(&nwork, 1)] = (unsigned short)(tid + SEL_THREADS * j);
+            done |= 1u << j;
+        }
+    __syncthreads();
+    const int n_a = nwork;
+    rescore_dots(bank, ks, qv, n_a, nrows, [&](int c) { return list[work[c]].row; },
+                 [&](int c, float dot) { score[work[c]] = dot; });
+    __syncthreads();
+    if (na >= kp && tid < n_a) {
+        const unsigned mine = isc_score_bits(score[work[tid]]);
+        int rank = 0;
+        for (int j = 0; j < n_a; ++j) {
+            const unsigned o = isc_score_bits(score[work[j]]);
+            rank += (o > mine || (o == mine && j < tid)) ? 1 : 0;
+        }
+        if (rank == kp - 1 && mine != 0u) taup_sh = score[work[tid]];
+    }
+    __syncthreads();
+    const float taup = taup_sh;
+    const float rhs = taup * qr.x;
+#pragma unroll
+    for (int j = 0; j < SEL_PER; ++j)
+        if (key[j] != 0ull && !((done >> j) & 1u)) {
+            const float p = isc_key_score(key[j]);
+            const float lhs = p + mt[j];
+            if (!(lhs + (fabsf(p) + mt[j] + fabsf(rhs)) * 9.5367431640625e-7f + 1e-30f < rhs)) {
+                work[atomicAdd(&nwork, 1)] = (unsigned short)(tid + SEL_THREADS * j);
+                done |= 1u << j;
+            }
+        }
+    __syncthreads();
+    const int n_b = nwork - n_a;
+    rescore_dots(bank, ks, qv, n_b, nrows, [&](int c) { return list[work[n_a + c]].row; },
+                 [&](int c, float dot) { score[work[n_a + c]] = dot; });
+    __syncthreads();
+#pragma unroll
+    for (int j = 0; j < SEL_PER; ++j)
+        if ((done >> j) & 1u) {
+            const float sc = score[tid + SEL_THREADS * j];
+            if (sc >= taup) list[atomicAdd(&kept, 1)] = Cand{sc, isc_key_row(key[j])};
+        }
     __syncthreads();
     if (tid == 0) qcount[q] = kept;
 }
@@ -1510,7 +1662,7 @@
     IscPerm pm, int64_t index_base, const float* __restrict__ norm_bound, const int32_t* __restrict__ qcount,
     const Cand* __restrict__ qlist, const float* __restrict__ carry_s, const int32_t* __restrict__ carry_r,
     const int32_t* __restrict__ carry_n, const int32_t* __restrict__ qflag, float* __restrict__ out_s,
-    int64_t* __restrict__ out_i, RedoLists rl, int32_t* __restrict__ status) {
+    int64_t* __restrict__ out_i, RedoLists rl, int32_t* __restrict__ status, const float* __restrict__ tau_floor) {
     __shared__ SelShared sh;
     __shared__ double exact_dot[ISC_TOPK_MAX_K + 8];
     __shared__ float fsc[ISC_TOPK_MAX_K + 8];
@@ -1585,7 +1737,8 @@
             if (nc < kp) {
                 if constexpr (!MASK) redo = true;
             } else {
-                const float t = isc_key_score(sh.topk[kp - 1]);
+                float t = isc_key_score(sh.topk[kp - 1]);
+                if (tau_floor && t == t) t = fmaxf(t, tau_floor[q]);
                 const float bound = (float)(((double)t + eps) / denom);
                 redo = !(bound < kth_sh);
             }
@@ -1834,6 +1987,7 @@
     const Level& l = p.levels[p.nlevels - 1];
     return (double)p.kp * (double)(l.r1 - l.r0) / (double)l.r0 * I8_INFLATION <= (double)p.budget;
 }
+int plan_i8_levels(const Plan& p, int d) { return plan_uses_i8(p, d) ? p.nlevels - 1 : 0; }
 
 template <typename T, typename TQ, typename... RowMask>
 int run(const void* bank, int64_t n, int d, const void* queries, int q_total, int64_t ldq, int k, int64_t index_base,
@@ -1864,41 +2018,55 @@
                            w.exact.redo_count, w.exact.done, w.r_count, w.tau2, w.qcount2, w.qflag2, status,
                            q0 == 0 ? 1 : 0);
         const int ks8 = isc_shadow_ksteps(d);
+        const unsigned char* sh = static_cast<const unsigned char*>(shadow);
+        const IscShadowRec* recs = use_i8 ? reinterpret_cast<const IscShadowRec*>(sh + isc_shadow_data_bytes(n, d)) : nullptr;
         if (use_i8)
             hipLaunchKernelGGL((k_prep_i8<TQ>), dim3(p.qpad / 4), dim3(256), 0, stream, qptr, ldq, q, d, ks8, p.tnq,
-                               w.qpacked8, w.qrec8);
+                               w.qpacked8, w.qrec8,
+                               reinterpret_cast<const IscShadowStats*>(sh + isc_shadow_stats_offset(n, d)), w.tau_floor);
         const FilterIO io{w.qpacked, w.tau, w.qcount, w.qflag, nullptr};
         for (int li = 0; li < p.nlevels; ++li) {
             const Level& l = p.levels[li];
-            if (use_i8 && li == p.nlevels - 1) {
-                const unsigned char* sh = static_cast<const unsigned char*>(shadow);
-                const IscShadowArgs sa{reinterpret_cast<const IscShadowRec*>(sh + isc_shadow_data_bytes(n, d)), w.qrec8};
+            const bool last = li == p.nlevels - 1;
+            if (use_i8 && !l.sample) {
+                const IscShadowArgs sa{recs, w.qrec8};
                 for_each_segment(l, p, [&](const Level& ls) {
                     isc_timing_begin(ISC_KERNEL_DOTS_FILTER, stream);
-                    hipLaunchKernelGGL((k_dots_filter<signed char, 256, 12, false, IscShadowArgs>),
-                                       dim3(ls.nchunks, p.qtiles), dim3(NTHREADS), 0, stream, sh, ls.r0, ls.r1,
-                                       ls.tiles_per_chunk, ls.ntiles, w.qpacked8, ks8, w.tau, p.qpad, w.seg_ent, w.qcount,
-                                       w.qlist, p.kp, p.nslots, w.qflag, status, (const int32_t*)nullptr, sa);
+                    if (last)
+                        hipLaunchKernelGGL((k_dots_filter<signed char, 256, 12, false, IscShadowArgs>),
+                                           dim3(ls.nchunks, p.qtiles), dim3(NTHREADS), 0, stream, sh, ls.r0, ls.r1,
+                                           ls.tiles_per_chunk, ls.ntiles, w.qpacked8, ks8, w.tau, p.qpad, w.seg_ent,
+                                           w.qcount, w.qlist, p.kp, p.nslots, w.qflag, status, (const int32_t*)nullptr, sa);
+                    else
+                        hipLaunchKernelGGL((k_dots_filter<signed char, 256, 12, false, IscShadowSlackArgs>),
+                                           dim3(ls.nchunks, p.qtiles), dim3(NTHREADS), 0, stream, sh, ls.r0, ls.r1,
+                                           ls.tiles_per_chunk, ls.ntiles, w.qpacked8, ks8, w.tau, p.qpad, w.seg_ent,
+                                           w.qcount, w.qlist, p.kp, p.nslots, w.qflag, status, (const int32_t*)nullptr,
+                                           IscShadowSlackArgs{sa});
                     isc_timing_end(ISC_KERNEL_DOTS_FILTER, stream);
                 });
-                hipLaunchKernelGGL(k_rescore, dim3(q), dim3(SEL_THREADS), 0, stream, bank_bytes, ksteps, w.qpacked, p.tnq,
-                                   w.tau, w.qcount, w.qlist, n);
-                continue;
-            }
-            for_each_segment(l, p, [&](const Level& ls) {
-                isc_timing_begin(ISC_KERNEL_DOTS_FILTER, stream);
-                if (p.tnq == 256)
-                    launch_filter<T, 256>(ls, p, w, io, bank_bytes, ksteps, status, stream,
-                                          pass_filter(rm, q0, q, nullptr)...);
-                else if (p.tnq == 128)
-                    launch_filter<T, 128>(ls, p, w, io, bank_bytes, ksteps, status, stream,
-                                          pass_filter(rm, q0, q, nullptr)...);
+                if (last)
+                    hipLaunchKernelGGL(k_rescore, dim3(q), dim3(SEL_THREADS), 0, stream, bank_bytes, ksteps, w.qpacked,
+                                       p.tnq, w.tau, w.qcount, w.qlist, n);
                 else
-                    launch_filter<T, 64>(ls, p, w, io, bank_bytes, ksteps, status, stream,
-                                         pass_filter(rm, q0, q, nullptr)...);
-                isc_timing_end(ISC_KERNEL_DOTS_FILTER, stream);
-            });
-            if (li + 1 < p.nlevels) {
+                    hipLaunchKernelGGL(k_rescore_band, dim3(q), dim3(SEL_THREADS), 0, stream, bank_bytes, ksteps, w.qpacked,
+                                       p.tnq, p.kp, w.tau, w.tau_floor, w.qrec8, recs, w.qcount, w.qlist, n);
+            } else {
+                for_each_segment(l, p, [&](const Level& ls) {
+                    isc_timing_begin(ISC_KERNEL_DOTS_FILTER, stream);
+                    if (p.tnq == 256)
+                        launch_filter<T, 256>(ls, p, w, io, bank_bytes, ksteps, status, stream,
+                                              pass_filter(rm, q0, q, nullptr)...);
+                    else if (p.tnq == 128)
+                        launch_filter<T, 128>(ls, p, w, io, bank_bytes, ksteps, status, stream,
+                                              pass_filter(rm, q0, q, nullptr)...);
+                    else
+                        launch_filter<T, 64>(ls, p, w, io, bank_bytes, ksteps, status, stream,
+                                             pass_filter(rm, q0, q, nullptr)...);
+                    isc_timing_end(ISC_KERNEL_DOTS_FILTER, stream);
+                });
+            }
+            if (!last) {
                 if (spec_all)
                     hipLaunchKernelGGL(k_select<SEL_PER>, dim3(q), dim3(SEL_THREADS), 0, stream, w.qcount, w.qlist, p.kp,
                                        w.tau, w.carry_s, w.carry_r, w.carry_n, w.qflag);
@@ -1911,11 +2079,11 @@
         if (spec_all)
             hipLaunchKernelGGL((k_final<T, SEL_PER, MASK>), dim3(q), dim3(SEL_THREADS), 0, stream, bank_bytes, ksteps, w.qpacked,
                                p.tnq, p.kp, k, pm, index_base, norm_bound, w.qcount, w.qlist, w.carry_s, w.carry_r,
-                               w.carry_n, w.qflag, os, oi, rl, status);
+                               w.carry_n, w.qflag, os, oi, rl, status, use_i8 ? w.tau_floor : nullptr);
         else
             hipLaunchKernelGGL((k_final<T, SEL_SPEC_MANY, MASK>), dim3(q), dim3(SEL_THREADS), 0, stream, bank_bytes, ksteps,
                                w.qpacked, p.tnq, p.kp, k, pm, index_base, norm_bound, w.qcount, w.qlist, w.carry_s,
-                               w.carry_r, w.carry_n, w.qflag, os, oi, rl, status);
+                               w.carry_r, w.carry_n, w.qflag, os, oi, rl, status, use_i8 ? w.tau_floor : nullptr);
         {
             const FilterIO rio{w.qpacked2, w.tau2, w.qcount2, w.qflag2, w.r_count};
             Level all;
@@ -2032,6 +2200,14 @@
     const int st = check_args(dtype, N, D, Q, k);
     if (st != ISC_OK) return st;
     *uses = dtype == ISC_F16 && plan_uses_i8(make_plan(N, Q, k), D) ? 1 : 0;
+    return ISC_OK;
+}
+
+extern "C" int isc_cosine_topk_shadow_levels(int dtype, int64_t N, int D, int Q, int k, int* n_int8_levels) {
+    ISC_REQUIRE(n_int8_levels);
+    const int st = check_args(dtype, N, D, Q, k);
+    if (st != ISC_OK) return st;
+    *n_int8_levels = dtype == ISC_F16 ? plan_i8_levels(make_plan(N, Q, k), D) : 0;
     return ISC_OK;
 }
 
diff --git a/include/imagescry_hip.h b/include/imagescry_hip.h
--- a/include/imagescry_hip.h
+++ b/include/imagescry_hip.h
@@ -165,6 +165,7 @@
 int isc_bank_shadow_bytes(int64_t N, int D, size_t* bytes);
 int isc_bank_quantize(const void* packed, int64_t N, int D, void* shadow, size_t shadow_bytes, void* stream);
 int isc_cosine_topk_uses_shadow(int dtype, int64_t N, int D, int Q, int k, int* uses);
+int isc_cosine_topk_shadow_levels(int dtype, int64_t N, int D, int Q, int k, int* n_int8_levels);
 int isc_cosine_topk_shadow(const void* bank, int dtype, int64_t N, int D, const void* queries, int q_dtype, int Q,
                            int64_t ldq, int k, int64_t index_base, const float* norm_bound, float* out_scores,
                            int64_t* out_indices, int32_t* status, void* workspace, size_t workspace_bytes,
```

After: 131,600 queries/s (median of 6 runs). 10.4% higher.
